# tvlearn/evo

Measured on AMD Instinct MI355X. Metric: E-step candidate-state evals/sec (NxS), full EM iteration, higher is better.
Workload: dtype f64; 1 GPU; ES3C D=256 H=512 S=200 N=100k f64 (north-star shape); algo=es3c, N_total=100000, N_rank0=100000, D=256, H=512, S=200, step=10 full EM iterations, world_size_rccl=1, ea=fit/randflip 10 parents x 1 child x 1 gen, states=p_init_Kn=1/H (init_states default), rng=device, mstep=device, parallelism=dp1

## Files before the change

evo_amd/csrc/evo_amd.hip:

```cpp
#include "../../include/evo_amd.h"

#include <dlfcn.h>
#include <math.h>
#include <stdarg.h>
#include <stdio.h>
#include <stdlib.h>
#include <string.h>

#include <chrono>
#include <memory>
#include <string>
#include <type_traits>
#include <vector>

#include "common.hpp"
#include "gemm_f64.hpp"
#include "kernels_bsc.hpp"
#include "kernels_common.hpp"
#include "kernels_evolve.hpp"
#include "kernels_mstep.hpp"
#include "kernels_sssc.hpp"
#include "kernels_sssc_quad.hpp"
#include "kernels_fused.hpp"
#include "kernels_patches.hpp"
#include "kernels_codes.hpp"
#include "kernels_init.hpp"
#include "kernels_generate.hpp"

static thread_local char g_err[512] = "";

static int fail(int code, const char *fmt, ...) {
  va_list ap;
  va_start(ap, fmt);
  vsnprintf(g_err, sizeof(g_err), fmt, ap);
  va_end(ap);
  return code;
}

#define HIP_TRY(expr)                                                                          \
  do {                                                                                         \
    hipError_t _e = (expr);                                                                    \
    if (_e != hipSuccess)                                                                      \
      return fail(EVOAMD_E_HIP, "%s failed: %s (%s:%d)", #expr, hipGetErrorString(_e), __FILE__, \
                  __LINE__);                                                                   \
  } while (0)

static const bool g_dbg_sync = getenv("EVOAMD_DEBUG_SYNC") != nullptr;
#define DBG_SYNC(c, what)                                                    \
  do {                                                                       \
    if (g_dbg_sync) {                                                        \
      fprintf(stderr, "[evoamd] %s ...", what);                              \
      fflush(stderr);                                                        \
      hipError_t _de = hipStreamSynchronize((c)->stream);                    \
      fprintf(stderr, " %s\n", hipGetErrorString(_de));                      \
      fflush(stderr);                                                        \
    }                                                                        \
  } while (0)

#define REQUIRE(cond, msg)                                   \
  do {                                                       \
    if (!(cond)) return fail(EVOAMD_E_INVALID, "%s", msg);   \
  } while (0)
#define REQUIRE_KN(c) \
  REQUIRE(!(c)->kn_lost, "K^n is not on the device: evoamd_init_states stopped at its round cap (upload or initialise K^n first)")

struct RcclId {
  char internal[128];
};
struct RcclApi {
  void *handle = nullptr;
  int (*GetUniqueId)(RcclId *) = nullptr;
  int (*CommInitRank)(void **, int, RcclId, int) = nullptr;
  int (*AllReduce)(const void *, void *, size_t, int, int, void *, hipStream_t) = nullptr;
  int (*CommDestroy)(void *) = nullptr;
  const char *(*GetErrorString)(int) = nullptr;
};
static RcclApi g_rccl;

static int rccl_load() {
  if (g_rccl.handle) return 0;
  const char *names[] = {"librccl.so.1", "librccl.so", "/opt/rocm/lib/librccl.so.1"};
  void *h = nullptr;
  for (const char *nm : names) {
    h = dlopen(nm, RTLD_NOW | RTLD_LOCAL);
    if (h) break;
  }
  if (!h) return fail(EVOAMD_E_RCCL, "cannot dlopen librccl: %s", dlerror());
  g_rccl.GetUniqueId = (int (*)(RcclId *))dlsym(h, "ncclGetUniqueId");
  g_rccl.CommInitRank = (int (*)(void **, int, RcclId, int))dlsym(h, "ncclCommInitRank");
  g_rccl.AllReduce =
      (int (*)(const void *, void *, size_t, int, int, void *, hipStream_t))dlsym(h, "ncclAllReduce");
  g_rccl.CommDestroy = (int (*)(void *))dlsym(h, "ncclCommDestroy");
  g_rccl.GetErrorString = (const char *(*)(int))dlsym(h, "ncclGetErrorString");
  if (!g_rccl.GetUniqueId || !g_rccl.CommInitRank || !g_rccl.AllReduce || !g_rccl.CommDestroy)
    return fail(EVOAMD_E_RCCL, "librccl is missing a required symbol");
  g_rccl.handle = h;
  return 0;
}
#define RCCL_TRY(expr)                                                                         \
  do {                                                                                         \
    int _r = (expr);                                                                           \
    if (_r != 0)                                                                               \
      return fail(EVOAMD_E_RCCL, "%s failed: %s", #expr,                                       \
                  g_rccl.GetErrorString ? g_rccl.GetErrorString(_r) : "?");                    \
  } while (0)

enum {
  KID_LPJ_RES = 0,
  KID_LPJ_CAND,
  KID_LPJ_OVF,
  KID_ROW_LSE,
  KID_VARY_KN,
  KID_STATS,
  KID_STATS_OVF,
  KID_GEMM,
  KID_EVOLVE,
  KID_MISC,
  KID_MSTEP,
  KID_LPJ_PASS,
  KID_STATS_PASS,
  KID_LPJ_K34,
  KID_LPJ_K58,
  KID_LPJ_K9P,
  KID_STATS_K34,
  KID_STATS_K58,
  KID_STATS_K9P,
  KID_ALLREDUCE,
  KID_ESTEP_FUSED,
  KID_PATCHES,
  KID_INIT_STATES,
  KID_COUNT
};

struct TimedSpan {
  hipEvent_t a, b;
  int kid;
};

struct evoamd_ctx {
  int device = 0;
  hipStream_t stream = nullptr;
  hipStream_t stream2 = nullptr;
  hipEvent_t ev_fork = nullptr, ev_join = nullptr;
  bool gemm_forked = false;
  hipStream_t stream_copy = nullptr;
  hipEvent_t ev_theta = nullptr, ev_theta_done = nullptr;
  hipEvent_t ev_mbox = nullptr, ev_bak = nullptr;
  int mbox_side = 1;
  int theta_copy_engine = 0;
  double rel_frac = -1.0;
  bool ar_gemm_pending = false;
  int overlap_gemm = 1;
  int early_fork = -1;
  int bg_unit = 0;
  int fold_clear = 1;
  bool acc_clean = false, clist_clean = false;
  bool wq_copy_valid = false;
  int stats_chunks = 1;
  int n_cu = 256;
  int stats_stage = 1;
  int stats_waves = 0;
  PairBins pbins = {};
  int bins_min = 256;
 int bins_scale = 3;
  int bins_scale_cur = 0;
  int bins_auto = 1;
  bool bins_dirty = false;
  int bins_nwg = 2048;
  int bsc_wave_opt = 1;
  int gemm_ws_opt = 1;
  double *gemm_ws = nullptr;
  size_t gemm_ws_n = 0;
  int pair_bins = 1;
  int gemm_streamk = 1;
  int sk_spare = -1;
  int sssc_prec32 = 0;
  int main_unstaged = 1;
  int sing_screen = 1;
  double *huge = nullptr;
  int *huge_ctl = nullptr;
  int huge_slots = 0, huge_kc = 0;
  int *sing_gen = nullptr;
  int theta_gen = 0;
  int gemm_grouped = 1;
  int gemm_per_xcd = 0;
  double *census = nullptr;
  i64 pre_n = 4;
  hipEvent_t ev_chunk[16] = {};
  bool configured = false, have_data = false, have_params = false, have_cand = false, B_valid = false;
  bool need_known = false;
  bool res_need[3] = {true, true, true};
  double res_cnt[3] = {0, 0, 0};
  bool cand_from_device = false;
  bool lists_clean = false;
  int pending_skip = 0;
  int pays_agreed = -1;
  int k8_mode = -1;
  bool bsc_direct = false;
  bool f32_opt = false, f32 = false;
  float *Yf = nullptr, *Ytf = nullptr, *Wf = nullptr, *Bf = nullptr, *Esf = nullptr;
  i64 ldYt = 0;
  double *Yt = nullptr;
  int b_tn_opt = 1;
  uint8_t *mask_infr = nullptr, *mask_x = nullptr;
  double *Yrec = nullptr;
  bool yrec_valid = false, rec_in_stats = false;
  double *yhat = nullptr, *tmpWt = nullptr;
  size_t yhat_n = 0;
  bool yhat_valid = false;
  bool stats_rows_valid = false;
  bool rec_resident = false, yrec_from_pass = false;
  uint8_t *keep_x = nullptr;
  bool keep_x_valid = false, rec_uses_keep = false;
  uint8_t *row_any = nullptr;
  int merge_select_fused = 0;
  unsigned long long gen = 0, prefetch_gen = ~0ull;
  bool prefetch_lpj = true;
  int spd_block = 0;
  bool use_digest = true;
  bool spd_inverse = true;
  long spd_fallbacks = 0;
  bool rows_fresh = false;
  int model = 0;
  i64 N = 0;
  int D = 0, H = 0, S = 0, S_perm = 0, Cmax = 0, HW = 0, L = 0;
  double *Y = nullptr, *yy = nullptr, *y2sum = nullptr;
  int ldY = 0;
  double *h_acc = nullptr, *h_par = nullptr;
  size_t h_par_n = 0;
  double *h_theta = nullptr;
  double *h_theta_dev = nullptr;
  bool h_theta_fresh = false;
  double *theta_bak = nullptr;
  size_t theta_bak_n = 0;
  bool theta_bak_valid = false;
  unsigned long long mbox_seq = 0;
  unsigned *mbox_counter = nullptr;
  int *h_err = nullptr;
  u64 *states = nullptr, *cand = nullptr;
  u64 *dig = nullptr, *cand_dig = nullptr;
  double *lpj = nullptr, *cand_lpj = nullptr;
  double *lpj_alt = nullptr;
  int *cand_counts = nullptr;
  u64 *cand_raw = nullptr, *dupold = nullptr;
  int *gen_start = nullptr;
  unsigned *flags = nullptr;
  double *rowmax = nullptr, *rowsum = nullptr, *partial = nullptr, *partial2 = nullptr, *diag = nullptr;
  i64 n_partial = 0;
  uint8_t *stage = nullptr;
  size_t stage_bytes = 0;
  double *W = nullptr, *Wt = nullptr, *G = nullptr, *Psi = nullptr, *Bm = nullptr, *mus = nullptr,
         *pilbar_v = nullptr;
  double2 *GP = nullptr;
  double4 *DG = nullptr;
  double4 *D1 = nullptr;
  PairEntry *PT = nullptr;
  double *pies = nullptr;
  double *dpar = nullptr;
  double *h_dpar = nullptr;
  double *colpart = nullptr;
  size_t colpart_n = 0;
  double *gjwork = nullptr;
  double *tmpA = nullptr, *tmpB = nullptr, *tmpC = nullptr;
  double ljc = 0;
  double *acc = nullptr;
  i64 acc_n = 0;
  double *acc_base = nullptr;
  i64 ovf_n = 0;
  double *Es = nullptr;
  int *list1 = nullptr, *list2 = nullptr, *list3 = nullptr, *list_n = nullptr, *err = nullptr;
  int *clist = nullptr, *clist_n = nullptr;
  size_t clist_words = 0;
  OvfRec *ovf_rec = nullptr;
  size_t ovf_rec_n = 0;
  unsigned long long kn_gen = 1, census_gen = 0;
  int census_opt = 1;
  int merge_small = 1;
  int stats_flat = 0;
  int fused_opt = 0;
  double *rowF = nullptr;
  int *rowcnt = nullptr, *defer = nullptr;
  double *fpart = nullptr;
  unsigned long long *fprof = nullptr;
  bool last_estep_fused = false;
  bool reduce_pending = false;
  long fused_calls = 0, unfused_calls = 0;
  int debug_poison_list = 0;
  int debug_fail_stats = 0;
  int census_skip = 0;
  size_t list_words = 0;
  double *tmp_y = nullptr, *tmp_lpj = nullptr;
  u64 *tmp_states = nullptr;
  size_t tmp_states_words = 0, tmp_lpj_n = 0;
  double *patch_img = nullptr, *patch_Y = nullptr;
  size_t patch_img_n = 0, patch_Y_n = 0;
  uint8_t *codes_buf = nullptr;
  size_t codes_bytes = 0;
  unsigned long long rows_kn_gen = 0;
  int codes_path = -1;
  int init_home = -1;
  u64 *init_scratch = nullptr;
  size_t init_scratch_words = 0;
  bool kn_lost = false;
  i64 kn_refill = 0;
  double *gen_par = nullptr, *gen_y = nullptr, *gen_z = nullptr, *gen_ymean = nullptr;
  u64 *gen_sin = nullptr, *gen_s = nullptr;
  size_t gen_par_n = 0, gen_y_n = 0, gen_z_n = 0, gen_ymean_n = 0, gen_sin_n = 0, gen_s_n = 0;
  i64 gen_N = 0;
  int gen_D = 0, gen_H = 0, gen_keep = -1;
  void *comm = nullptr;
  int rank = 0, world = 1;
  bool timing = false;
  unsigned timing_mask = 0xFFFFFFFFu;
  std::vector<TimedSpan> spans;
  std::vector<hipEvent_t> pool;
  double t_ms[KID_COUNT] = {0};
  i64 t_n[KID_COUNT] = {0};
};

struct SpanGuard {
  evoamd_ctx *c;
  int kid;
  hipStream_t stream;
  hipEvent_t a = nullptr, b = nullptr;
  SpanGuard(evoamd_ctx *ctx, int k, hipStream_t s = nullptr) : c(ctx), kid(k), stream(s ? s : ctx->stream) {
    if (!c->timing || !((c->timing_mask >> k) & 1u)) return;
    auto get = [&]() {
      hipEvent_t e;
      if (!c->pool.empty()) {
        e = c->pool.back();
        c->pool.pop_back();
      } else {
        (void)hipEventCreate(&e);
      }
      return e;
    };
    a = get();
    b = get();
    (void)hipEventRecord(a, stream);
  }
  ~SpanGuard() {
    if (!c->timing || !a) return;
    (void)hipEventRecord(b, stream);
    c->spans.push_back({a, b, kid});
  }
};

static int resolve_spans(evoamd_ctx *c) {
  for (auto &s : c->spans) {
    float ms = 0.f;
    HIP_TRY(hipEventSynchronize(s.b));
    HIP_TRY(hipEventElapsedTime(&ms, s.a, s.b));
    c->t_ms[s.kid] += ms;
    c->t_n[s.kid] += 1;
    c->pool.push_back(s.a);
    c->pool.push_back(s.b);
  }
  c->spans.clear();
  return 0;
}

template <typename T>
static int dev_alloc(T **p, size_t n) {
  if (*p) {
    (void)hipFree(*p);
    *p = nullptr;
  }
  if (n == 0) n = 1;
  HIP_TRY(hipMalloc((void **)p, n * sizeof(T)));
  return 0;
}
#define ALLOC(p, n)                 \
  do {                              \
    int _r = dev_alloc(&(p), (n));  \
    if (_r) return _r;              \
  } while (0)

static inline unsigned cdiv(i64 a, i64 b) { return (unsigned)((a + b - 1) / b); }
static inline size_t list_cap(i64 total) { return (size_t)(256 * (((total + 255) / 256 + LIST_SHARDS - 1) / LIST_SHARDS) + 1024); }

template <bool SQUARE>
static void launch_colsum(evoamd_ctx *c, const double *X, int ldx, i64 R, int Cn, double *out) {
  const i64 rpb = 256;
  dim3 grid(cdiv(Cn, 64), cdiv(R, rpb));
  colsum_f64<SQUARE><<<grid, 256, 0, c->stream>>>(X, ldx, R, Cn, rpb, out);
}


static int ensure_colpart(evoamd_ctx *c, size_t n) {
  if (n <= c->colpart_n) return 0;
  HIP_TRY(hipStreamSynchronize(c->stream));
  ALLOC(c->colpart, n);
  c->colpart_n = n;
  return 0;
}

static int ensure_lists(evoamd_ctx *c, i64 total) {
  const size_t need = list_cap(total) * LIST_SHARDS;
  if (need <= c->list_words) return 0;
  HIP_TRY(hipStreamSynchronize(c->stream));
  ALLOC(c->list1, need);
  ALLOC(c->list2, need);
  ALLOC(c->list3, need);
  c->list_words = need;
  return 0;
}

extern "C" int evoamd_abi_version(void) { return EVOAMD_ABI_VERSION; }
extern "C" const char *evoamd_last_error(void) { return g_err; }

extern "C" int evoamd_device_count(int *count) {
  REQUIRE(count, "count is NULL");
  int n = 0;
  hipError_t e = hipGetDeviceCount(&n);
  if (e != hipSuccess) {
    *count = 0;
    return fail(EVOAMD_E_NODEVICE, "hipGetDeviceCount: %s", hipGetErrorString(e));
  }
  *count = n;
  return 0;
}

extern "C" int evoamd_ctx_create(int device, evoamd_ctx **out) {
  REQUIRE(out, "out is NULL");
  int n = 0;
  if (hipGetDeviceCount(&n) != hipSuccess || n <= 0)
    return fail(EVOAMD_E_NODEVICE, "no HIP device visible (libevo_amd needs an MI355X / gfx950 GPU)");
  REQUIRE(device >= 0 && device < n, "device index out of range");
  HIP_TRY(hipSetDevice(device));
  hipDeviceProp_t prop;
  HIP_TRY(hipGetDeviceProperties(&prop, device));
  if (strncmp(prop.gcnArchName, "gfx950", 6) != 0)
    return fail(EVOAMD_E_NODEVICE, "device %d is %s; libevo_amd is built for gfx950 only", device,
                prop.gcnArchName);
  evoamd_ctx *c = new evoamd_ctx();
  c->device = device;
  c->n_cu = prop.multiProcessorCount > 0 ? prop.multiProcessorCount : 256;
  {
    int prio_lo = 0, prio_hi = 0;
    HIP_TRY(hipDeviceGetStreamPriorityRange(&prio_lo, &prio_hi));
    HIP_TRY(hipStreamCreateWithPriority(&c->stream, hipStreamNonBlocking, prio_hi));
    HIP_TRY(hipStreamCreateWithPriority(&c->stream2, hipStreamNonBlocking, prio_lo));
  }
  HIP_TRY(hipEventCreateWithFlags(&c->ev_fork, hipEventDisableTiming));
  HIP_TRY(hipEventCreateWithFlags(&c->ev_join, hipEventDisableTiming));
  HIP_TRY(hipStreamCreateWithFlags(&c->stream_copy, hipStreamNonBlocking));
  HIP_TRY(hipEventCreateWithFlags(&c->ev_theta, hipEventDisableTiming));
  HIP_TRY(hipEventCreateWithFlags(&c->ev_theta_done, hipEventDisableTiming));
  HIP_TRY(hipEventCreateWithFlags(&c->ev_mbox, hipEventDisableTiming));
  HIP_TRY(hipEventCreateWithFlags(&c->ev_bak, hipEventDisableTiming));
  for (int i = 0; i < 16; i++) HIP_TRY(hipEventCreateWithFlags(&c->ev_chunk[i], hipEventDisableTiming));

  HIP_TRY(hipFuncSetAttribute((const void *)sssc_stats_flat_kernel, hipFuncAttributeMaxDynamicSharedMemorySize, 150 * 1024));
  HIP_TRY(hipFuncSetAttribute((const void *)sssc_big_kernel<0>, hipFuncAttributeMaxDynamicSharedMemorySize,
                              136 * 1024));
  HIP_TRY(hipFuncSetAttribute((const void *)sssc_big_kernel<0, 0>, hipFuncAttributeMaxDynamicSharedMemorySize,
                              136 * 1024));
  HIP_TRY(hipFuncSetAttribute((const void *)sssc_big_kernel<0, 1>, hipFuncAttributeMaxDynamicSharedMemorySize,
                              136 * 1024));
  HIP_TRY(hipFuncSetAttribute((const void *)sssc_big_kernel<1>, hipFuncAttributeMaxDynamicSharedMemorySize,
                              136 * 1024));
  HIP_TRY(hipFuncSetAttribute((const void *)posterior_codes_kernel<CODES_LDS>, hipFuncAttributeMaxDynamicSharedMemorySize,
                              CODES_WAVES * CODES_LDS_H * (int)sizeof(double)));
  HIP_TRY(hipFuncSetAttribute((const void *)gemm_tn128_f64, hipFuncAttributeMaxDynamicSharedMemorySize,
                              (int)GEMM128_LDS_BYTES));
  HIP_TRY(hipFuncSetAttribute((const void *)gemm_tn128_rows_f64, hipFuncAttributeMaxDynamicSharedMemorySize,
                              (int)GEMM128_LDS_BYTES));
  HIP_TRY(hipFuncSetAttribute((const void *)gemm_tn128_sk_f64, hipFuncAttributeMaxDynamicSharedMemorySize,
                              (int)GEMM128_LDS_BYTES));
  HIP_TRY(hipFuncSetAttribute((const void *)gemm_tn128_sk_f32, hipFuncAttributeMaxDynamicSharedMemorySize,
                              (int)GEMM128_LDS_BYTES));
  HIP_TRY(hipFuncSetAttribute((const void *)gemm_tn128_store_f32, hipFuncAttributeMaxDynamicSharedMemorySize,
                              (int)GEMM128_LDS_BYTES));
  {
    const void *wk[] = {(const void *)sssc_stats_wave_kernel<0, 4>,  (const void *)sssc_stats_wave_kernel<1, 4>,
                        (const void *)sssc_stats_wave_kernel<2, 4>,  (const void *)sssc_stats_wave_kernel<4, 4>,
                        (const void *)sssc_stats_wave_kernel<8, 4>,  (const void *)sssc_stats_wave_kernel<16, 4>,
                        (const void *)sssc_stats_wave_kernel<0, 1>,  (const void *)sssc_stats_wave_kernel<0, 8>,
                        (const void *)sssc_stats_wave_kernel<0, 16>};
    for (const void *f : wk) HIP_TRY(hipFuncSetAttribute(f, hipFuncAttributeMaxDynamicSharedMemorySize, 150 * 1024));
    HIP_TRY(hipFuncSetAttribute((const void *)pair_bins_reduce_kernel, hipFuncAttributeMaxDynamicSharedMemorySize, 3 * PB_TILE * 8));
    HIP_TRY(hipFuncSetAttribute((const void *)sssc_small_kernel<4, 1, 2, 256>, hipFuncAttributeMaxDynamicSharedMemorySize, 120 * 1024));
    HIP_TRY(hipFuncSetAttribute((const void *)sssc_small_kernel<8, 1, 2, 256>, hipFuncAttributeMaxDynamicSharedMemorySize, 120 * 1024));
  }
  {
    const void *fk[] = {(const void *)sssc_estep_fused_kernel<1, false>,  (const void *)sssc_estep_fused_kernel<1, true>,
                        (const void *)sssc_estep_fused_kernel<2, false>,  (const void *)sssc_estep_fused_kernel<2, true>,
                        (const void *)sssc_estep_fused_kernel<4, false>,  (const void *)sssc_estep_fused_kernel<4, true>,
                        (const void *)sssc_estep_fused_kernel<8, false>,  (const void *)sssc_estep_fused_kernel<8, true>,
                        (const void *)sssc_estep_fused_kernel<16, false>, (const void *)sssc_estep_fused_kernel<16, true>};
    for (const void *fp : fk) HIP_TRY(hipFuncSetAttribute(fp, hipFuncAttributeMaxDynamicSharedMemorySize, 160 * 1024));
  }
  *out = c;
  return 0;
}

static void free_all(evoamd_ctx *c) {
  void *ptrs[] = {c->Y,      c->yy,     c->y2sum,   c->states,  c->cand,     c->lpj,       c->cand_lpj,
                  c->cand_counts, c->flags, c->rowmax, c->rowsum, c->partial, c->partial2, c->diag, c->stage,    c->W,
                  c->Wt,     c->G,      c->Psi,     c->Bm,      c->mus,      c->pilbar_v,  c->GP,      c->DG,    c->D1,    c->PT,   c->yhat,  c->tmpWt,  c->mask_infr,  c->mask_x,  c->Yrec,
                  c->pies,   c->tmpA,    c->tmpB,    c->tmpC,    c->gjwork,  c->colpart,
                  c->acc_base, c->Es,     c->list1,   c->list2,    c->list3,    c->list_n,    c->err,
                  c->tmp_y,  c->tmp_lpj, c->tmp_states, c->dig, c->cand_dig, c->lpj_alt, c->cand_raw, c->dupold, c->gen_start,
                  c->pbins.ent, c->pbins.part, c->pbins.gcnt, c->gemm_ws, c->Yt, c->Yf, c->Ytf, c->Wf, c->Bf, c->Esf,
                  c->clist, c->clist_n, c->ovf_rec, c->theta_bak, c->rowF, c->rowcnt, c->defer, c->fpart, c->huge, c->huge_ctl,
                  c->patch_img, c->patch_Y, c->keep_x, c->row_any, c->codes_buf, c->init_scratch,
                  c->gen_par, c->gen_y, c->gen_z, c->gen_ymean, c->gen_sin, c->gen_s};
  for (void *p : ptrs)
    if (p) (void)hipFree(p);
  if (c->h_acc) (void)hipHostFree(c->h_acc);
  if (c->h_par) (void)hipHostFree(c->h_par);
  if (c->h_theta) (void)hipHostFree(c->h_theta);
  c->h_theta = nullptr;
  if (c->h_err) (void)hipHostFree(c->h_err);
  if (c->h_dpar) (void)hipHostFree(c->h_dpar);
}

extern "C" void evoamd_ctx_destroy(evoamd_ctx *c) {
  if (!c) return;
  (void)hipSetDevice(c->device);
  (void)hipStreamSynchronize(c->stream);
  if (c->comm && g_rccl.CommDestroy) g_rccl.CommDestroy(c->comm);
  for (auto &s : c->spans) {
    (void)hipEventDestroy(s.a);
    (void)hipEventDestroy(s.b);
  }
  for (auto e : c->pool) (void)hipEventDestroy(e);
  free_all(c);
  (void)hipStreamDestroy(c->stream);
  if (c->stream2) (void)hipStreamDestroy(c->stream2);
  if (c->stream_copy) (void)hipStreamDestroy(c->stream_copy);
  if (c->ev_theta) (void)hipEventDestroy(c->ev_theta);
  if (c->ev_theta_done) (void)hipEventDestroy(c->ev_theta_done);
  if (c->ev_mbox) (void)hipEventDestroy(c->ev_mbox);
  if (c->ev_bak) (void)hipEventDestroy(c->ev_bak);
  if (c->ev_fork) (void)hipEventDestroy(c->ev_fork);
  if (c->ev_join) (void)hipEventDestroy(c->ev_join);
  for (int i = 0; i < 16; i++)
    if (c->ev_chunk[i]) (void)hipEventDestroy(c->ev_chunk[i]);

  delete c;
}

extern "C" int evoamd_set_option(evoamd_ctx *c, const char *name, int value) {
  REQUIRE(c && name, "bad arguments");
  c->gen++;
  if (strcmp(name, "sssc_k8") == 0) {
    c->k8_mode = value < 0 ? -1 : (value != 0);
    return 0;
  }
  if (strcmp(name, "ebsc_f32") == 0) {
    c->f32_opt = value != 0;
    return 0;
  }
  if (strcmp(name, "bsc_direct") == 0) {
    c->bsc_direct = value != 0;
    c->have_params = false;
    return 0;
  }
  if (strcmp(name, "reconstruct_in_stats") == 0) {
    c->rec_in_stats = value != 0;
    return 0;
  }
  if (strcmp(name, "codes_path") == 0) {
    if (value < -1 || value > CODES_GMEM) return fail(EVOAMD_E_INVALID, "codes_path: -1 (auto), 0 registers, 1 LDS, 2 global memory");
    c->codes_path = value;
    return 0;
  }
  if (strcmp(name, "merge_select_fused") == 0) {
    c->merge_select_fused = value != 0;
    return 0;
  }
  if (strcmp(name, "prefetch_lpj") == 0) {
    c->prefetch_lpj = value != 0;
    return 0;
  }
  if (strcmp(name, "inverse_block") == 0) {
    if (value != 0 && value != 16 && value != 32) return fail(EVOAMD_E_INVALID, "inverse_block: 0 (auto), 16 or 32");
    c->spd_block = value;
    return 0;
  }
  if (strcmp(name, "overlap_gemm") == 0) {
    c->overlap_gemm = value;
    return 0;
  }
  if (strcmp(name, "stats_stage") == 0) {
    c->stats_stage = value;
    return 0;
  }
  if (strcmp(name, "stats_waves") == 0) {
    c->stats_waves = value;
    return 0;
  }
  if (strcmp(name, "pair_bins") == 0) {
    c->pair_bins = value;
    return 0;
  }
  if (strcmp(name, "gemm_streamk") == 0) {
    c->gemm_streamk = value;
    return 0;
  }
  if (strcmp(name, "b_transposed") == 0) {
    c->b_tn_opt = value;
    return 0;
  }
  if (strcmp(name, "pair_bins_scale") == 0) {
    if (value < 1 || value > 64) return fail(EVOAMD_E_INVALID, "pair_bins_scale: 1 .. 64");
    c->bins_scale = value;
    return 0;
  }
  if (strcmp(name, "pair_bins_nwg") == 0) {
    if (value < 256 || value > 2048 || (value % 256) != 0) return fail(EVOAMD_E_INVALID, "pair_bins_nwg: 256 .. 2048, multiple of 256");
    c->bins_nwg = value;
    return 0;
  }
  if (strcmp(name, "pair_bins_auto") == 0) {
    c->bins_auto = value != 0;
    return 0;
  }
  if (strcmp(name, "pair_bins_min") == 0) {
    c->bins_min = value;
    return 0;
  }
  if (strcmp(name, "bsc_stats_wave") == 0) {
    c->bsc_wave_opt = value;
    return 0;
  }
  if (strcmp(name, "gemm_workspace") == 0) {
    c->gemm_ws_opt = value;
    return 0;
  }
  if (strcmp(name, "sssc_precision") == 0) {
    if (value != 64 && value != 32) return fail(EVOAMD_E_INVALID, "sssc_precision: 64 or 32");
    c->sssc_prec32 = value == 32;
    return 0;
  }
  if (strcmp(name, "lpj_main_unstaged") == 0) {
    c->main_unstaged = value != 0;
    return 0;
  }
  if (strcmp(name, "lpj_singular_screen") == 0) {
    if (value < 0 || value > 2) return fail(EVOAMD_E_INVALID, "lpj_singular_screen: 0 (never), 1 (automatic) or 2 (always)");
    c->sing_screen = (int)value;
    return 0;
  }
  if (strcmp(name, "gemm_grouped") == 0) {
    c->gemm_grouped = value != 0;
    return 0;
  }
  if (strcmp(name, "gemm_per_xcd") == 0) {
    c->gemm_per_xcd = value;
    return 0;
  }
  if (strcmp(name, "init_states_home") == 0) {
    if (value < -1 || value > 1) return fail(EVOAMD_E_INVALID, "init_states_home: -1 (auto), 0 LDS, 1 global memory");
    c->init_home = value;
    return 0;
  }
  if (strcmp(name, "background_unit") == 0) {
    c->bg_unit = value != 0;
    return 0;
  }
  if (strcmp(name, "fold_clear") == 0) {
    c->fold_clear = value != 0;
    return 0;
  }
  if (strcmp(name, "early_fork") == 0) {
    c->early_fork = value;
    return 0;
  }
  if (strcmp(name, "merge_small_levels") == 0) {
    c->merge_small = value != 0;
    return 0;
  }
  if (strcmp(name, "stats_flat") == 0) {
    c->stats_flat = value != 0;
    return 0;
  }
  if (strcmp(name, "theta_copy_engine") == 0) {
    c->theta_copy_engine = value != 0;
    return 0;
  }
  if (strcmp(name, "census_lists") == 0) {
    c->census_opt = value != 0;
    return 0;
  }
  if (strcmp(name, "sk_spare") == 0) {
    if (value < -1 || value > 32) return fail(EVOAMD_E_INVALID, "sk_spare: -1 (automatic) or 0 .. 32 workgroups per XCD");
    c->sk_spare = value;
    return 0;
  }
  if (strcmp(name, "stats_chunks") == 0) {
    if (value < 1 || value > 16) return fail(EVOAMD_E_INVALID, "stats_chunks: 1 .. 16");
    c->stats_chunks = value;
    return 0;
  }
  if (strcmp(name, "mailbox_side_stream") == 0) {
    c->mbox_side = value != 0;
    return 0;
  }
  if (strcmp(name, "fused_estep") == 0) {
    if (value < 0 || value > 2) return fail(EVOAMD_E_INVALID, "fused_estep: 0 (never), 1 (automatic) or 2 (whenever the shape allows it)");
    c->fused_opt = value;
    return 0;
  }
  if (strcmp(name, "debug_poison_list") == 0) {
    c->debug_poison_list = value != 0;
    return 0;
  }
  if (strcmp(name, "debug_fail_stats") == 0) {
    c->debug_fail_stats = value != 0;
    return 0;
  }
  if (strcmp(name, "state_digest") == 0) {
    c->use_digest = value != 0;
    return 0;
  }
  if (strcmp(name, "inverse_spd") == 0) {
    c->spd_inverse = value != 0;
    return 0;
  }
  return fail(EVOAMD_E_INVALID, "unknown option '%s'", name);
}

static int join_fork(evoamd_ctx *c);

extern "C" int evoamd_synchronize(evoamd_ctx *c) {
  REQUIRE(c, "ctx is NULL");
  int rj = join_fork(c);
  if (rj) return rj;
  HIP_TRY(hipStreamSynchronize(c->stream));
  return 0;
}

static i64 acc_len(const evoamd_ctx *c) {
  const i64 H = c->H, D = c->D;
  return (c->model == EVOAMD_MODEL_BSC) ? H * D + H * H + H + 1 + 8 : 2 * H + 4 * H * H + D * H + D + 8;
}
struct AccLayout {
  i64 Wp, Wq, pies, sigma;
  i64 xs, xss, xsz, xszsz, s_sz, sz_sz, sWp, y2;
  i64 tail;
};
static AccLayout acc_layout(const evoamd_ctx *c) {
  AccLayout a = {};
  const i64 H = c->H, D = c->D;
  if (c->model == EVOAMD_MODEL_BSC) {
    a.Wp = 0;
    a.Wq = H * D;
    a.pies = a.Wq + H * H;
    a.sigma = a.pies + H;
    a.tail = a.sigma + 1;
  } else {
    a.xs = 0;
    a.xss = H;
    a.xsz = a.xss + H * H;
    a.xszsz = a.xsz + H;
    a.sWp = a.xszsz + H * H;
    a.s_sz = a.sWp + D * H;
    a.sz_sz = a.s_sz + H * H;
    a.y2 = a.sz_sz + H * H;
    a.tail = a.y2 + D;
  }
  return a;
}

static int alloc_pair_bins(evoamd_ctx *c, int scale) {
  const i64 N = c->N;
  const int H = c->H, S = c->S;
  if (c->pbins.ent) (void)hipFree(c->pbins.ent);
  if (c->pbins.gcnt) (void)hipFree(c->pbins.gcnt);
  if (c->pbins.part) (void)hipFree(c->pbins.part);
  c->pbins = PairBins{};
  c->bins_scale_cur = 0;
  if (H >= 2 && H <= 1024) {
    PairBins pb = {};
    pb.rf = std::max(1, PB_TILE / (2 * H));
    const int nfold = (H - 1 + 1) / 2;
    pb.nb = (int)cdiv(nfold, pb.rf);
    pb.nwg = c->bins_nwg;
    pb.nsh = std::max((i64)N * S >= (i64)8 << 20 ? 8 : 4, std::min(PB_NSH_MAX, 256 / std::max(1, pb.nb)));
    pb.cap = (int)std::max<i64>(64, (i64)scale * cdiv((i64)N * S, (i64)pb.nb * pb.nwg));
    const size_t ne = (size_t)pb.nb * pb.nwg * pb.cap;
    const bool got = hipMalloc((void **)&pb.ent, ne * sizeof(double4)) == hipSuccess &&
                     hipMalloc((void **)&pb.part, (size_t)pb.nb * pb.nsh * 3 * 2 * pb.rf * H * sizeof(double)) == hipSuccess &&
                     hipMalloc((void **)&pb.gcnt, (size_t)pb.nb * pb.nwg * sizeof(int)) == hipSuccess;
    if (got) {
      HIP_TRY(hipMemsetAsync(pb.gcnt, 0, (size_t)pb.nb * pb.nwg * sizeof(int), c->stream));
      c->pbins = pb;
      c->bins_scale_cur = scale;
      c->bins_dirty = false;
    } else {
      (void)hipGetLastError();
      if (pb.ent) (void)hipFree(pb.ent);
      if (pb.part) (void)hipFree(pb.part);
      if (pb.gcnt) (void)hipFree(pb.gcnt);
    }
  }
  return 0;
}

static int ensure_bins_capacity(evoamd_ctx *c) {
  if (c->model != EVOAMD_MODEL_SSSC || !c->need_known || !c->pbins.ent || c->bins_auto == 0) return 0;
  const double NS = (double)c->N * c->S;
  const double n34 = c->res_cnt[0] - c->res_cnt[1], n58 = c->res_cnt[1] - c->res_cnt[2];
  const double entries = (NS - c->res_cnt[0]) + 6.0 * n34 + 28.0 * n58;
  int want = (int)std::ceil(3.0 * 1.25 * entries / NS);
  if (want > 64) want = 64;
  if (want <= c->bins_scale_cur) return 0;
  HIP_TRY(hipStreamSynchronize(c->stream));
  if (c->stream2) HIP_TRY(hipStreamSynchronize(c->stream2));
  const int before = c->bins_scale_cur;
  int r = alloc_pair_bins(c, want);
  if (r) return r;
  if (!c->pbins.ent) {
    r = alloc_pair_bins(c, before);
    if (r) return r;
    c->bins_auto = 0;
  }
  return 0;
}

extern "C" int evoamd_configure(evoamd_ctx *c, int model, int64_t N, int D, int H, int S, int S_perm,
                                int Cmax) {
  REQUIRE(c, "ctx is NULL");
  REQUIRE(model == EVOAMD_MODEL_BSC || model == EVOAMD_MODEL_SSSC, "unknown model");
  REQUIRE(N > 0 && D > 0 && H > 0 && S > 0, "N, D, H, S must be positive");
  REQUIRE(S_perm == 0 || S_perm == 1, "S_perm must be 0 or 1");
  REQUIRE(Cmax >= 1 && Cmax <= 64 * VK_MAX_C_PER_LANE, "Cmax must be in [1, 256]");
  REQUIRE(S <= 64 * VK_MAX_S_PER_LANE, "S must be <= 1024");
  REQUIRE((i64)N * (S > Cmax ? S : Cmax) < 2147483647LL, "N * max(S, Cmax) must fit in int32");
  HIP_TRY(hipSetDevice(c->device));
  c->model = model;
  c->N = N;
  c->D = D;
  c->H = H;
  c->S = S;
  c->S_perm = S_perm;
  c->Cmax = Cmax;
  c->HW = (H + 63) / 64;
  c->L = S + S_perm;
  const i64 HW = c->HW;
  c->ldY = (model == EVOAMD_MODEL_SSSC) ? D + 3 * H : D;
  ALLOC(c->Y, (size_t)N * c->ldY);
  ALLOC(c->yy, (size_t)N);
  ALLOC(c->y2sum, (size_t)D);
  ALLOC(c->states, (size_t)N * S * HW);
  ALLOC(c->cand, (size_t)N * Cmax * HW);
  if (H <= DIG_MAX_H) {
    ALLOC(c->dig, (size_t)N * S);
    ALLOC(c->cand_dig, (size_t)N * Cmax);
  } else {
    if (c->dig) (void)hipFree(c->dig);
    if (c->cand_dig) (void)hipFree(c->cand_dig);
    c->dig = c->cand_dig = nullptr;
  }
  ALLOC(c->lpj, (size_t)N * c->L);
  ALLOC(c->lpj_alt, (size_t)N * c->L);
  ALLOC(c->cand_lpj, (size_t)N * Cmax);
  ALLOC(c->cand_counts, (size_t)N);
  ALLOC(c->flags, (size_t)3 * N);
  ALLOC(c->rowmax, (size_t)N);
  ALLOC(c->rowsum, (size_t)N);
  c->n_partial = cdiv(N, 4);
  ALLOC(c->partial, (size_t)3 * c->n_partial);
  ALLOC(c->partial2, (size_t)c->n_partial);
  ALLOC(c->diag, (size_t)H);
  const int SC = S > Cmax ? S : Cmax;
  ALLOC(c->W, (size_t)D * H);
  ALLOC(c->tmpA, (size_t)H * H);
  ALLOC(c->tmpB, (size_t)H * H);
  ALLOC(c->tmpC, (size_t)H * H);
  ALLOC(c->gjwork, (size_t)2 * H * H + (size_t)132 * H + 1040 + 4 * GJS32 * GJS32);
  if (model == EVOAMD_MODEL_BSC) {
    ALLOC(c->Es, (model == EVOAMD_MODEL_BSC && c->f32_opt) ? 1 : (size_t)N * H);
  } else {
    if (c->Es) { (void)hipFree(c->Es); }
    c->Es = nullptr;
// ... 311 lines not shown
  REQUIRE(!(c->bg_unit && c->S_perm), "evoamd_init_states: no permanent all-zero state with the background unit (variational/utils.py:42-47)");
  REQUIRE(c->H - c->bg_unit >= 1, "evoamd_init_states: no latent varies");
  HIP_TRY(hipSetDevice(c->device));
  const int S = c->S, HW = c->HW;
  if (table_packed) {
    const int Hv = c->H - c->bg_unit;
    REQUIRE(Hv < 12 && S + c->S_perm == (1 << Hv),
            "evoamd_init_states: a state table means exact E-steps, S + S_perm == 2^Hv with Hv < 12 (variational/utils.py:55)");
  }
  if (table_packed) {
    const int PB = (c->H + 7) / 8;
    const size_t off = (((size_t)S * PB + 7) / 8) * 8;
    {
      int rs = ensure_stage(c, off + (size_t)S * HW * sizeof(u64));
      if (rs) return rs;
    }
    u64 *table = (u64 *)(c->stage + off);
    HIP_TRY(hipMemcpyAsync(c->stage, table_packed, (size_t)S * PB, hipMemcpyHostToDevice, c->stream));
    SpanGuard g(c, KID_INIT_STATES);
    words_from_packbits_kernel<<<cdiv((i64)S * HW, 256), 256, 0, c->stream>>>(c->stage, table, S, PB, HW, c->H);
    init_states_tile_kernel<<<cdiv(c->N * (i64)S, 256), 256, 0, c->stream>>>(table, c->states, c->dig, c->N, S, HW);
  } else {
    InitArgs a;
    a.states = c->states;
    a.dig = c->dig;
    a.scratch = nullptr;
    a.err = c->err + INIT_ERR_WORD;
    a.N = c->N;
    a.S = S;
    a.S_perm = c->S_perm;
    a.H = c->H;
    a.Hv = c->H - c->bg_unit;
    a.HW = HW;
    a.max_rounds = max_rounds;
    a.seed = seed;
    a.p0 = p_init > 0.0 ? p_init : 1.0 / (double)c->H;
    const size_t wave_words = 2 * (size_t)(HW + 1) * S;
    int W = 4;
    while (W > 1 && W * wave_words * sizeof(u64) > 150 * 1024) W >>= 1;
    const bool lds_fits = W * wave_words * sizeof(u64) <= 150 * 1024;
    REQUIRE(c->init_home != 0 || lds_fits, "init_states_home 0 (LDS): the round state of one wavefront does not fit");
    const bool lds_home = c->init_home < 0 ? lds_fits : c->init_home == 0;
    c->kn_lost = true;
    c->kn_refill = 0;
    c->gen++;
    c->kn_gen++;
    c->need_known = false;
    HIP_TRY(hipMemsetAsync(a.err, 0, sizeof(int), c->stream));
    if (lds_home) {
      const unsigned grid = (unsigned)std::min<i64>(cdiv(c->N, W), (i64)c->n_cu * 64);
      SpanGuard g(c, KID_INIT_STATES);
      init_states_kernel<true><<<grid, 64 * W, (size_t)W * wave_words * sizeof(u64), c->stream>>>(a);
    } else {
      W = 4;
      i64 grid = std::min<i64>(cdiv(c->N, W), (i64)c->n_cu * 2);
      while (grid > 1 && (size_t)grid * W * wave_words * sizeof(u64) > ((size_t)256 << 20)) grid >>= 1;
      const size_t need = (size_t)grid * W * wave_words;
      if (need > c->init_scratch_words) {
        HIP_TRY(hipStreamSynchronize(c->stream));
        ALLOC(c->init_scratch, need);
        c->init_scratch_words = need;
      }
      a.scratch = c->init_scratch;
      SpanGuard g(c, KID_INIT_STATES);
      init_states_kernel<false><<<(unsigned)grid, 64 * W, 0, c->stream>>>(a);
    }
    HIP_TRY(hipGetLastError());
    DBG_SYNC(c, "init_states");
    HIP_TRY(hipMemcpyAsync(c->h_err, a.err, sizeof(int), hipMemcpyDeviceToHost, c->stream));
    HIP_TRY(hipStreamSynchronize(c->stream));
    if (c->h_err[0] & INIT_ERR_CAP) {
      HIP_TRY(hipMemsetAsync(a.err, 0, sizeof(int), c->stream));
      return fail(EVOAMD_E_INVALID,
                  "evoamd_init_states: a datapoint holds fewer than S = %d distinct states after max_rounds = %d rounds (the "
                  "round cap); K^n is not initialised -- shapes with S close to 2^H belong to the host function",
                  S, max_rounds);
    }
    c->kn_lost = false;
    return 0;
  }
  HIP_TRY(hipGetLastError());
  HIP_TRY(hipStreamSynchronize(c->stream));
  c->gen++;
  c->kn_gen++;
  c->need_known = false;
  c->kn_lost = false;
  return 0;
}

extern "C" int evoamd_download_states_packed(evoamd_ctx *c, uint8_t *packed, int64_t n0, int64_t n) {
  REQUIRE(c && c->configured, "configure first");
  REQUIRE(packed && n0 >= 0 && n > 0 && n0 + n <= c->N, "bad row range");
  REQUIRE_KN(c);
  HIP_TRY(hipSetDevice(c->device));
  const int PB = (c->H + 7) / 8;
  const i64 ns = n * (i64)c->S;
  const size_t bytes = (size_t)ns * PB;
  {
    int rs = ensure_stage(c, bytes);
    if (rs) return rs;
  }
  packbits_from_words_kernel<<<cdiv(ns * PB, 256), 256, 0, c->stream>>>(c->states + (size_t)n0 * c->S * c->HW, c->stage, ns,
                                                                         PB, c->HW);
  HIP_TRY(hipGetLastError());
  HIP_TRY(hipMemcpyAsync(packed, c->stage, bytes, hipMemcpyDeviceToHost, c->stream));
  HIP_TRY(hipStreamSynchronize(c->stream));
  return 0;
}

extern "C" int evoamd_upload_lpj(evoamd_ctx *c, const double *lpj) {
  REQUIRE(c && c->configured, "configure first");
  HIP_TRY(hipSetDevice(c->device));
  HIP_TRY(hipMemcpyAsync(c->lpj, lpj, (size_t)c->N * c->L * sizeof(double), hipMemcpyHostToDevice, c->stream));
  HIP_TRY(hipStreamSynchronize(c->stream));
  c->rows_fresh = false;
  return 0;
}

extern "C" int evoamd_download_lpj(evoamd_ctx *c, double *lpj) {
  REQUIRE(c && c->configured, "configure first");
  HIP_TRY(hipSetDevice(c->device));
  HIP_TRY(hipMemcpyAsync(lpj, c->lpj, (size_t)c->N * c->L * sizeof(double), hipMemcpyDeviceToHost, c->stream));
  HIP_TRY(hipStreamSynchronize(c->stream));
  return 0;
}

static bool gemm_vec_ok(const double *p, int ld) { return (ld % 2) == 0 && ((uintptr_t)p % 16) == 0; }

static bool launch_gemm_nn_raw(evoamd_ctx *c, const double *A, int lda, const double *B, int ldb, double *C, int ldc,
                               i64 M, int Nc, int K, double *Ct = nullptr, int ldct = 0) {
  if (M <= 1024 && Nc <= 1024 && K <= 1024) {
    gemm_nn_small_kernel<<<dim3(cdiv(Nc, 16), cdiv(M, 16)), 256, 0, c->stream>>>(A, lda, B, ldb, C, ldc, (int)M, Nc, K, Ct, ldct);
    return Ct != nullptr;
  }
  const int gx = (int)cdiv(Nc, GEMM_BN), gy = (int)cdiv(M, GEMM_BM);
  const int rows_per_xcd = (gy + 7) / 8;
  const unsigned grid = (unsigned)(8 * rows_per_xcd * gx);
  if (gemm_vec_ok(A, lda) && gemm_vec_ok(B, ldb) && (K % 2) == 0 && (Nc % 2) == 0 && K >= 2 && Nc >= 2 && M >= 1)
    gemm_nn_f64<true><<<grid, 256, 0, c->stream>>>(A, lda, B, ldb, C, ldc, M, Nc, K, gx, gy, rows_per_xcd);
  else
    gemm_nn_f64<false><<<grid, 256, 0, c->stream>>>(A, lda, B, ldb, C, ldc, M, Nc, K, gx, gy, rows_per_xcd);
  return false;
}

struct GemmTnOpts {
  bool deterministic = false;
  int sym_row0 = -1;
  bool c_is_zero = false;
  bool accumulate = false;
  bool mirror = true;
  hipStream_t stream = nullptr;
  int spare = 0;
  double *diag = nullptr;
};

static bool gram_is_small(int M, i64 K) { return M <= 512 && K <= 4096; }

static double *streamk_workspace(evoamd_ctx *c, unsigned wpx, i64 n_real, int *segmax) {
  *segmax = (int)(n_real / wpx) + 2;
  const size_t need = (size_t)8 * wpx * (size_t)*segmax * GEMM_T * GEMM_T;
  if (need > c->gemm_ws_n) {
    if (c->gemm_ws) (void)hipFree(c->gemm_ws);
    c->gemm_ws = nullptr;
    c->gemm_ws_n = 0;
    if (hipMalloc((void **)&c->gemm_ws, need * sizeof(double)) != hipSuccess) {
      (void)hipGetLastError();
      c->gemm_ws = nullptr;
      return nullptr;
    }
    c->gemm_ws_n = need;
  }
  return c->gemm_ws;
}

static int launch_gemm_tn(evoamd_ctx *c, const double *A, int lda, const double *B, int ldb, double *C, int ldc,
                          int M, int Nc, i64 K, const GemmTnOpts &o = GemmTnOpts()) {
  const bool deterministic = o.deterministic, c_is_zero = o.c_is_zero, accumulate = o.accumulate, mirror = o.mirror;
  int sym_row0 = o.sym_row0;
  const hipStream_t stream = o.stream ? o.stream : c->stream;
  if (deterministic && A == B && lda == ldb && M == Nc && sym_row0 < 0 && gram_is_small(M, K)) {
    SpanGuard g(c, KID_GEMM, stream);
    const int nb16 = (int)cdiv(M, 16);
    gram_small_kernel<<<dim3(nb16, nb16), 256, 0, stream>>>(A, lda, (int)K, M, C, ldc, o.diag);
    HIP_TRY(hipGetLastError());
    return 0;
  }
  const bool vec = gemm_vec_ok(A, lda) && gemm_vec_ok(B, ldb) && (M % 2) == 0 && (Nc % 2) == 0 && M >= 2 && Nc >= 2;
  const bool big = vec && !deterministic && K >= 8192 && M >= 256 && Nc >= 256 &&
                   (sym_row0 < 0 || (sym_row0 % GEMM_T) == 0);
  const int T = big ? GEMM_T : GEMM_BM;
  if (sym_row0 >= 0 && (sym_row0 % T) != 0) sym_row0 = -1;
  const int gx = (int)cdiv(Nc, T), gy = (int)cdiv(M, T);
  const i64 tiles = (i64)gx * gy;
  i64 splits = 1;
  if (K >= 128 && !deterministic) {
    if (big) {
      i64 real = tiles;
      if (sym_row0 >= 0) {
        const i64 ts = cdiv(Nc, T);
        real -= ts * (ts - 1) / 2;
      }
      i64 per_xcd = 1;
      double best = 0.0;
      for (i64 pc = 1; pc <= 16; pc++) {
        if (pc > 1 && K / (8 * pc) < 512) break;
        const double eff = (double)(real * pc) / (64.0 * (double)cdiv(real * pc, 64));
        if (eff > best + 0.01) {
          best = eff;
          per_xcd = pc;
        }
      }
      if (real > 24 && K / 64 >= 384) per_xcd = 8;
      if (c->gemm_per_xcd > 0) per_xcd = c->gemm_per_xcd;
      splits = 8 * per_xcd;
    } else {
      splits = (512 + tiles - 1) / tiles;
    }
    const i64 maxs = (K + 63) / 64;
    if (splits > maxs) splits = maxs;
    if (splits > 1) splits = ((splits + 7) / 8) * 8;
  }
  if (accumulate && splits < 8) splits = 8;
  const int split = splits > 1;
  i64 kps = K;
  if (split) {
    kps = (K + splits - 1) / splits;
    kps = ((kps + GEMM_BK - 1) / GEMM_BK) * GEMM_BK;
    if (!c_is_zero && !accumulate) HIP_TRY(hipMemsetAsync(C, 0, (size_t)M * ldc * sizeof(double), stream));
  }
  const unsigned grid = (unsigned)(tiles * (split ? splits : 1));
  SpanGuard g(c, KID_GEMM, stream);
  if (big && split && c->gemm_streamk) {
    i64 real = tiles;
    if (sym_row0 >= 0) {
      const i64 ts = cdiv(Nc, T);
      real -= ts * (ts - 1) / 2;
    }
    const i64 Kx = ((cdiv(K, 8) + GEMM_BK - 1) / GEMM_BK) * GEMM_BK;
    const unsigned wpx = (unsigned)std::max(1, 2 * c->n_cu / 8 - o.spare);
    int segmax = 0;
    double *ws = c->gemm_ws_opt ? streamk_workspace(c, wpx, real, &segmax) : nullptr;
    const i64 J = (i64)8 * wpx / real;
    if (ws && c->gemm_grouped && J >= 2 && real * J * 100 >= (i64)8 * wpx * 93 && K / J >= 256) {
      const i64 Kc = ((cdiv(K, J) + 2 * GEMM_BK - 1) / (2 * GEMM_BK)) * (2 * GEMM_BK);
      gemm_tn128_gk<double><<<8 * wpx, 256, GEMM128_LDS_BYTES, stream>>>(A, lda, B, ldb, C, ldc, M, Nc, K, Kc, gx, gy,
                                                                            sym_row0, (int)real, (int)J, ws);
      gemm_gk_reduce_kernel<<<dim3((unsigned)real, GEMM_T * GEMM_T / 256), 256, 0, stream>>>(ws, C, ldc, M, Nc, gx, gy,
                                                                                               sym_row0, (int)real, (int)J);
    } else {
    gemm_tn128_sk_f64<<<8 * wpx, 256, GEMM128_LDS_BYTES, stream>>>(A, lda, B, ldb, C, ldc, M, Nc, K, Kx, gx, gy, sym_row0,
                                                                       (int)real, ws, segmax);
    if (ws)
      gemm_sk_reduce_kernel<<<dim3((unsigned)real, GEMM_T * GEMM_T / 256), 256, 0, stream>>>(
          ws, segmax, C, ldc, M, Nc, K, Kx, gx, gy, sym_row0, (int)real, (int)wpx);
    }
  } else if (big)
    gemm_tn128_f64<<<grid, 256, GEMM128_LDS_BYTES, stream>>>(A, lda, B, ldb, C, ldc, M, Nc, K, kps, gx, gy, split, sym_row0);
  else if (vec)
    gemm_tn_f64<true><<<grid, 256, 0, stream>>>(A, lda, B, ldb, C, ldc, M, Nc, K, kps, gx, gy, split, sym_row0);
  else
    gemm_tn_f64<false><<<grid, 256, 0, stream>>>(A, lda, B, ldb, C, ldc, M, Nc, K, kps, gx, gy, split, sym_row0);
  if (sym_row0 >= 0 && mirror)
    mirror_lower_kernel<<<cdiv((i64)Nc * Nc, 256), 256, 0, stream>>>(C + (size_t)sym_row0 * ldc, Nc, ldc, T);
  HIP_TRY(hipGetLastError());
  return 0;
}

static int launch_gemm_nn(evoamd_ctx *c, const double *A, int lda, const double *B, int ldb, double *C, int ldc,
                          i64 M, int Nc, int K) {
  SpanGuard g(c, KID_GEMM);
  launch_gemm_nn_raw(c, A, lda, B, ldb, C, ldc, M, Nc, K);
  HIP_TRY(hipGetLastError());
  return 0;
}

static int launch_B_f32(evoamd_ctx *c);

static int launch_B(evoamd_ctx *c) {
  if (c->f32) return launch_B_f32(c);
  if (!c->Yt) return launch_gemm_nn(c, c->Y, c->ldY, c->W, c->H, c->Bm, c->H, c->N, c->H, c->D);
  SpanGuard g(c, KID_GEMM);
  const int gx = (int)cdiv(c->H, GEMM_T), gy = (int)cdiv(c->N, GEMM_T);
  gemm_tn128_rows_f64<<<(unsigned)(8 * cdiv(gy, 8) * gx), 256, GEMM128_LDS_BYTES, c->stream>>>(
      c->Yt, (int)c->ldYt, c->W, c->H, c->Bm, c->H, (int)c->N, c->H, c->D, gx, gy);
  HIP_TRY(hipGetLastError());
  return 0;
}

static int derive_from_theta(evoamd_ctx *c, bool updated) {
  const int H = c->H, D = c->D;
  int r = 0;
  c->B_valid = false;
  if (c->model == EVOAMD_MODEL_BSC && c->bsc_direct) return 0;
  GemmTnOpts gram;
  gram.deterministic = true;
  if (c->model == EVOAMD_MODEL_SSSC) {
    if (!updated) {
      r = launch_gemm_tn(c, c->W, H, c->W, H, c->G, H, H, H, D, gram);
      if (r) return r;
      DBG_SYNC(c, "derive_from_theta: G = W^T W");
    }
    if (c->mask_infr) {
      if (!c->Wt) ALLOC(c->Wt, (size_t)H * D);
      transpose_kernel<<<cdiv((i64)H * D, 256), 256, 0, c->stream>>>(c->W, D, H, c->Wt);
    }
    sssc_tables_kernel<<<cdiv((i64)H * H, 256), 256, 0, c->stream>>>(c->G, c->Psi, c->mus, c->pilbar_v, c->dpar, H, c->D1,
                                                                     c->PT, c->GP, c->DG, c->sing_gen, ++c->theta_gen);
    DBG_SYNC(c, "derive_from_theta: tables");
  } else {
    const bool diag_rides = updated && gram_is_small(H, D);
    if (diag_rides) gram.diag = c->diag;
    r = launch_gemm_tn(c, c->W, H, c->W, H, c->G, H, H, H, D, gram);
    if (r) return r;
    if (!diag_rides) extract_diag_kernel<<<cdiv(H, 256), 256, 0, c->stream>>>(c->G, H, c->diag);
  }
  HIP_TRY(hipGetLastError());
  if (c->have_data) {
    r = launch_B(c);
    if (r) return r;
    c->B_valid = true;
  }
  return 0;
}

extern "C" int evoamd_set_params_bsc(evoamd_ctx *c, const double *W, double pi, double sigma, double *ljc) {
  REQUIRE(c && c->configured && c->model == EVOAMD_MODEL_BSC, "context is not configured for BSC");
  REQUIRE(W, "W is NULL");
  REQUIRE(!(c->f32 && c->bsc_direct), "the direct residual kernel is not available in the float32 mode");
  HIP_TRY(hipSetDevice(c->device));
  c->ljc = c->H * log(1.0 - pi) - (c->rel_frac >= 0.0 ? c->rel_frac : (double)c->D) / 2.0 * log(2 * M_PI * sigma * sigma);
  if (ljc) *ljc = c->ljc;
  HIP_TRY(hipStreamSynchronize(c->stream));
  memset(c->h_dpar, 0, DP_COUNT * sizeof(double));
  c->h_dpar[DP_PRE1] = -1.0 / 2.0 / sigma / sigma;
  c->h_dpar[DP_PILBAR] = log(pi / (1.0 - pi));
  c->h_dpar[DP_LJC] = c->ljc;
  c->h_dpar[DP_PI] = pi;
  c->h_dpar[DP_SIGMA] = sigma;
  HIP_TRY(hipMemcpyAsync(c->dpar, c->h_dpar, DP_COUNT * sizeof(double), hipMemcpyHostToDevice, c->stream));
  HIP_TRY(hipStreamSynchronize(c->stream));
  double *wt = c->h_par;
  for (int d = 0; d < c->D; d++)
    for (int h = 0; h < c->H; h++) wt[(size_t)h * c->D + d] = W[(size_t)d * c->H + h];
  HIP_TRY(hipMemcpyAsync(c->Wt, wt, (size_t)c->H * c->D * sizeof(double), hipMemcpyHostToDevice, c->stream));
  HIP_TRY(hipStreamSynchronize(c->stream));
  memcpy(wt, W, (size_t)c->D * c->H * sizeof(double));
  HIP_TRY(hipMemcpyAsync(c->W, wt, (size_t)c->D * c->H * sizeof(double), hipMemcpyHostToDevice, c->stream));
  int r = derive_from_theta(c, false);
  if (r) return r;
  c->have_params = true;
  c->gen++;
  c->h_theta_fresh = false;
  c->yhat_valid = c->stats_rows_valid = c->rec_resident = c->yrec_from_pass = false;
  return 0;
}

extern "C" int evoamd_set_params_sssc(evoamd_ctx *c, const double *W, const double *pies, const double *mus,
                                      const double *Psi, double sigma2, double *ljc) {
  REQUIRE(c && c->configured && c->model == EVOAMD_MODEL_SSSC, "context is not configured for SSSC");
  REQUIRE(W && pies && mus && Psi, "NULL parameter array");
  HIP_TRY(hipSetDevice(c->device));
  const int H = c->H, D = c->D;
  const long double s2 = (long double)sigma2;
  const double s2inv = c->sssc_prec32 ? (double)(float)(1.0L / s2) : (double)(1.0L / s2);
  double l = 0.0;
  std::vector<double> pb(H);
  {
    long double acc = 0.0L;
    for (int h = 0; h < H; h++) {
      acc += (long double)log(1.0 - pies[h]);
      pb[h] = log(pies[h] / (1.0 - pies[h]));
    }
    l = (double)acc;
  }
  if (c->rel_frac >= 0.0) {
    l += (-log(2 * M_PI) - log(sigma2)) * c->rel_frac / 2.0;
  } else {
    l -= D / 2.0 * log(2 * M_PI);
    if (c->sssc_prec32) {
      const float ld = (float)D * (float)logl(s2);
      l -= (double)(0.5f * ld);
    } else {
      l -= 0.5 * (D * (double)logl(s2));
    }
  }
  c->ljc = l;
  if (ljc) *ljc = l;
  HIP_TRY(hipStreamSynchronize(c->stream));
  {
    double *hw = c->h_par, *hpsi = hw + (size_t)D * H, *hmu = hpsi + (size_t)H * H, *hpb = hmu + H, *hpi = hpb + H;
    memcpy(hw, W, (size_t)D * H * sizeof(double));
    memcpy(hpsi, Psi, (size_t)H * H * sizeof(double));
    memcpy(hmu, mus, (size_t)H * sizeof(double));
    memcpy(hpb, pb.data(), (size_t)H * sizeof(double));
    memcpy(hpi, pies, (size_t)H * sizeof(double));
    memset(c->h_dpar, 0, DP_COUNT * sizeof(double));
    c->h_dpar[DP_S2INV] = s2inv;
    c->h_dpar[DP_SIGMA2] = sigma2;
    c->h_dpar[DP_LJC] = l;
    HIP_TRY(hipMemcpyAsync(c->dpar, c->h_dpar, DP_COUNT * sizeof(double), hipMemcpyHostToDevice, c->stream));
    HIP_TRY(hipMemcpyAsync(c->pies, hpi, (size_t)H * sizeof(double), hipMemcpyHostToDevice, c->stream));
    HIP_TRY(hipMemcpyAsync(c->W, hw, (size_t)D * H * sizeof(double), hipMemcpyHostToDevice, c->stream));
    HIP_TRY(hipMemcpyAsync(c->Psi, hpsi, (size_t)H * H * sizeof(double), hipMemcpyHostToDevice, c->stream));
    HIP_TRY(hipMemcpyAsync(c->mus, hmu, (size_t)H * sizeof(double), hipMemcpyHostToDevice, c->stream));
    HIP_TRY(hipMemcpyAsync(c->pilbar_v, hpb, (size_t)H * sizeof(double), hipMemcpyHostToDevice, c->stream));
  }
  int r = derive_from_theta(c, false);
  if (r) return r;
  c->have_params = true;
  c->gen++;
  c->h_theta_fresh = false;
  c->yhat_valid = c->stats_rows_valid = c->rec_resident = c->yrec_from_pass = false;
  return 0;
}

static int launch_gemm_tn_f32(evoamd_ctx *c, const float *A, int lda, const float *B, int ldb, double *C, int ldc, int M, int Nc,
                              i64 K, const GemmTnOpts &o = GemmTnOpts()) {
  const hipStream_t stream = o.stream ? o.stream : c->stream;
  SpanGuard g(c, KID_GEMM, stream);
  if (M >= 128 && Nc >= 128 && K >= 2048 && (M % 4) == 0 && (Nc % 4) == 0) {
    const int gx = (int)cdiv(Nc, GEMM_T), gy = (int)cdiv(M, GEMM_T);
    const i64 Kx = ((cdiv(K, 8) + GEMM_BK - 1) / GEMM_BK) * GEMM_BK;
    const unsigned wpx = (unsigned)std::max(1, 2 * c->n_cu / 8 - o.spare);
    int segmax = 0;
    double *ws = c->gemm_ws_opt ? streamk_workspace(c, wpx, (i64)gx * gy, &segmax) : nullptr;
    const i64 real = (i64)gx * gy, J = (i64)8 * wpx / real;
    if (ws && c->gemm_grouped && J >= 2 && real * J * 100 >= (i64)8 * wpx * 93 && K / J >= 256) {
      const i64 Kc = ((cdiv(K, J) + 2 * GEMM_BK - 1) / (2 * GEMM_BK)) * (2 * GEMM_BK);
      gemm_tn128_gk<float><<<8 * wpx, 256, GEMM128_LDS_BYTES, stream>>>(A, lda, B, ldb, C, ldc, M, Nc, K, Kc, gx, gy, -1,
                                                                           (int)real, (int)J, ws);
      gemm_gk_reduce_kernel<<<dim3((unsigned)real, GEMM_T * GEMM_T / 256), 256, 0, stream>>>(ws, C, ldc, M, Nc, gx, gy, -1,
                                                                                               (int)real, (int)J);
    } else {
      gemm_tn128_sk_f32<<<8 * wpx, 256, GEMM128_LDS_BYTES, stream>>>(A, lda, B, ldb, C, ldc, M, Nc, K, Kx, gx, gy, gx * gy,
                                                                         ws, segmax);
      if (ws)
        gemm_sk_reduce_kernel<<<dim3((unsigned)(gx * gy), GEMM_T * GEMM_T / 256), 256, 0, stream>>>(
            ws, segmax, C, ldc, M, Nc, K, Kx, gx, gy, -1, gx * gy, (int)wpx);
    }
  } else {
    gemm_tn_naive_f32<<<cdiv((i64)M * Nc, 256), 256, 0, stream>>>(A, lda, B, ldb, C, ldc, M, Nc, K);
  }
  HIP_TRY(hipGetLastError());
  return 0;
}

static int launch_B_f32(evoamd_ctx *c) {
  SpanGuard g(c, KID_GEMM);
  to_f32_kernel<<<cdiv((i64)c->D * c->H, 256), 256, 0, c->stream>>>(c->W, c->H, c->D, c->H, c->Wf, c->H);
  if (c->H >= 128 && c->N >= 128) {
    const int gx = (int)cdiv(c->H, GEMM_T), gy = (int)cdiv(c->N, GEMM_T);
    gemm_tn128_store_f32<<<(unsigned)gx * gy, 256, GEMM128_LDS_BYTES, c->stream>>>(c->Ytf, (int)c->ldYt, c->Wf, c->H, c->Bf,
                                                                                  c->H, (int)c->N, c->H, c->D, gx);
  } else {
    gemm_nn_naive_f32<<<cdiv(c->N * (i64)c->H, 256), 256, 0, c->stream>>>(c->Yf, c->D, c->Wf, c->H, c->Bf, c->H, c->N, c->H,
                                                                           c->D);
  }
  HIP_TRY(hipGetLastError());
  return 0;
}

static int ensure_B(evoamd_ctx *c) {
  if (c->B_valid || (c->model == EVOAMD_MODEL_BSC && c->bsc_direct)) return 0;
  int r = launch_B(c);
  if (r) return r;
  DBG_SYNC(c, "B = Y W");
  c->B_valid = true;
  return 0;
}

struct Batch {
  const u64 *states;
  const int *counts;
  const double *Y;
  const double *Bm;
  const double *yy;
  i64 N;
  int C, shared;
  double *out;
  int ldo, col0;
  unsigned *flags;
  int kid;
  int tag;
  const uint8_t *mask = nullptr;
};

static const u64 *dig_for(const evoamd_ctx *c, const u64 *states) {
  if (!c->use_digest) return nullptr;
  return states == c->states ? c->dig : states == c->cand ? c->cand_dig : nullptr;
}

static int launch_bsc_lpj(evoamd_ctx *c, const Batch &b) {
  if (!c->bsc_direct && b.tag != 2 && !b.mask) {
    const i64 total = b.N * (i64)b.C;
    unsigned grid = cdiv(total, 256);
    const int bf32 = (c->f32 && b.Bm == c->Bm) ? 1 : 0;
    const void *bmat = bf32 ? (const void *)c->Bf : (const void *)b.Bm;
    SpanGuard g(c, b.kid);
    const int rows_cap = 512 / b.C + 2;
    const size_t lds = (size_t)rows_cap * c->H * sizeof(double);
    const bool hw_ok = c->HW == 1 || c->HW == 2 || c->HW == 4 || c->HW == 8 || c->HW == 16;
    const u64 *dg = b.shared ? nullptr : dig_for(c, b.states);
    if (!b.shared && (hw_ok || dg) && (c->H % 2) == 0 && lds <= 40 * 1024) {
      const unsigned g2 = cdiv(total, 512);
#define GRAM2(TAG, HWT)                                                                                      \
  bsc_lpj_gram2_kernel<TAG, HWT><<<g2, 512, lds, c->stream>>>(b.states, b.counts, bmat, b.yy, c->G, b.N, b.C, c->H, \
                                                              c->HW, c->dpar, b.out, b.ldo, b.col0, b.flags, c->err, dg, bf32, c->diag)
#define GRAM2_HW(TAG)                    \
  switch (c->HW) {                       \
    case 1: GRAM2(TAG, 1); break;        \
    case 2: GRAM2(TAG, 2); break;        \
    case 4: GRAM2(TAG, 4); break;        \
    case 8: GRAM2(TAG, 8); break;        \
    default: GRAM2(TAG, 16); break;      \
  }
      if (b.tag == 0) {
        GRAM2_HW(0)
      } else {
        GRAM2_HW(1)
      }
#undef GRAM2_HW
#undef GRAM2
      HIP_TRY(hipGetLastError());
      return 0;
    }
#define GRAM_LAUNCH(TAG)                                                                                       \
  bsc_lpj_gram_kernel<TAG><<<grid, 256, 0, c->stream>>>(b.states, b.counts, bmat, b.yy, c->G, b.N, b.C, b.shared, \
                                                        c->H, c->HW, c->dpar, b.out, b.ldo, b.col0, b.flags, c->err, dg, bf32, c->diag)
    if (b.tag == 0)
      GRAM_LAUNCH(0);
    else
      GRAM_LAUNCH(1);
#undef GRAM_LAUNCH
    HIP_TRY(hipGetLastError());
    return 0;
  }
  const int nchunk = (b.C + BSC_CHUNK - 1) / BSC_CHUNK;
  const unsigned grid = cdiv(b.N * nchunk, 4);
  SpanGuard g(c, b.kid);
#define BSC_LAUNCH(R)                                                                                     \
  bsc_lpj_kernel<R><<<grid, 256, 0, c->stream>>>(b.Y, c->Wt, b.states, b.counts, b.N, b.C, b.C, b.shared, \
                                                  c->D, c->HW, c->dpar, b.out, b.ldo, b.col0, b.flags, c->err, b.mask)
  if (c->D <= 64)
    BSC_LAUNCH(1);
  else if (c->D <= 128)
    BSC_LAUNCH(2);
  else
    BSC_LAUNCH(4);
#undef BSC_LAUNCH
  HIP_TRY(hipGetLastError());
  return 0;
}

static SsscArgs sssc_args(evoamd_ctx *c, const Batch &b) {
  SsscArgs a = {};
  a.states = b.states;
  a.dig = b.shared ? nullptr : dig_for(c, b.states);
  a.counts = b.counts;
  a.Bm = b.Bm;
  a.yy = b.yy;
  a.GP = c->GP;
  a.DG = c->DG;
  a.D1 = c->D1;
  a.PT = c->PT;
  a.mus = c->mus;
  a.pil_bar = c->pilbar_v;
  a.s2inv = 0.0;
  a.dpar = c->dpar;
  a.N = b.N;
  a.C = b.C;
  a.shared = b.shared;
  a.H = c->H;
  a.HW = c->HW;
  a.lpj_out = b.out;
  a.ldo = b.ldo;
  a.col0 = b.col0;
  a.flags = b.flags;
  a.err = c->err;
  a.sing_gen = c->sing_gen;
  a.gen = c->theta_gen;
  a.screen = c->sing_screen;
  a.huge = c->huge;
  a.huge_ctl = c->huge_ctl;
  a.huge_slots = c->huge_slots;
  a.huge_kc = c->huge_kc;
  a.mask = b.mask;
  a.Wt = c->Wt;
  a.D = c->D;
  return a;
}

// ... 810 lines not shown
  HIP_TRY(hipGetLastError());
  DBG_SYNC(c, "fused E-step (reduce)");
  return 0;
}

extern "C" int evoamd_estep(evoamd_ctx *c, int n_parents, int n_children, uint64_t seed, int fit_parents, int Mprime, int *fused_out) {
  REQUIRE(c && c->configured && c->have_data && c->have_params, "configure, upload_data and set_params first");
  REQUIRE(n_parents >= 1 && n_parents <= c->S && n_parents <= 64, "n_parents must be in [1, min(S, 64)]");
  REQUIRE(n_children >= 1 && n_children <= EV_MAX_CHILDREN && n_children <= c->H, "n_children must be in [1, min(8, H)]");
  REQUIRE(n_parents * n_children <= c->Cmax, "n_parents * n_children exceeds the configured Cmax");
  REQUIRE(Mprime >= 1 && Mprime <= c->S, "Mprime must be in [1, S]");
  REQUIRE_KN(c);
  HIP_TRY(hipSetDevice(c->device));
  bool fused = c->fused_opt != 0 && fused_shape_ok(c, n_parents, n_children);
  if (fused && c->fused_opt == 1) fused = c->need_known && c->res_cnt[1] <= 0.25 * (double)c->N;
  if (fused_out) *fused_out = fused ? 1 : 0;
  if (!fused) {
    c->unfused_calls++;
    c->last_estep_fused = false;
    int r = evoamd_lpj_resident(c);
    if (r) return r;
    r = evoamd_evolve_randflip(c, n_parents, n_children, seed, fit_parents);
    if (r) return r;
    return evoamd_vary_kn(c, Mprime, nullptr);
  }
  c->fused_calls++;
  c->prefetch_gen = ~0ull;
  c->rows_fresh = false;
  int r = launch_estep_fused(c, n_parents, n_children, seed, fit_parents, Mprime);
  if (r) return r;
  c->gen++;
  c->kn_gen++;
  if (c->N * (i64)c->S < ((i64)4 << 20)) c->census_gen = c->kn_gen;
  c->rows_fresh = true;
  c->have_cand = false;
  c->cand_from_device = true;
  c->last_estep_fused = true;
  return 0;
}

extern "C" int evoamd_estep_counters(evoamd_ctx *c, int64_t out[4]) {
  REQUIRE(c && c->configured && out, "bad arguments");
  HIP_TRY(hipSetDevice(c->device));
  out[0] = c->fused_calls;
  out[1] = c->unfused_calls;
  out[2] = out[3] = 0;
  if (c->defer) {
    int h[2] = {0, 0};
    HIP_TRY(hipStreamSynchronize(c->stream));
    HIP_TRY(hipMemcpy(&h[0], c->defer + c->N, sizeof(int), hipMemcpyDeviceToHost));
    out[2] = h[0];
  }
  return 0;
}

extern "C" int evoamd_evolve_states(evoamd_ctx *c, int mutation, int fit_parents, int n_parents, int n_children,
                                    int n_generations, uint64_t seed, double sparseness, double bitflip_prob) {
  REQUIRE(c && c->configured && c->have_data && c->have_params, "configure, upload_data and set_params first");
  REQUIRE(mutation >= EV_RANDFLIP && mutation <= EV_CROSS_SPARSEFLIP, "unknown mutation operator");
  REQUIRE_KN(c);
  REQUIRE(n_parents >= 1 && n_parents <= c->S && n_parents <= 64, "n_parents must be in [1, min(S, 64)]");
  REQUIRE(n_generations >= 1, "n_generations must be positive");
  const bool crossing = mutation >= EV_CROSS;
  const int per_gen = crossing ? n_parents * (n_parents - 1) : n_parents * n_children;
  REQUIRE(crossing || (n_children >= 1 && n_children <= c->H), "n_children must be in [1, H]");
  REQUIRE(mutation != EV_RANDFLIP || n_children <= EV_MAX_CHILDREN, "randflip: n_children must be <= 8");
  REQUIRE((i64)per_gen * n_generations <= c->Cmax, "children per generation x generations exceeds the configured Cmax");
  REQUIRE(c->S <= EVG_MAX_S && c->Cmax <= EVG_MAX_C, "S <= 1024 and Cmax <= 256");
  const bool sparse = mutation == EV_SPARSEFLIP || mutation == EV_CROSS_SPARSEFLIP;
  REQUIRE(!sparse || bitflip_prob == bitflip_prob, "sparseflip needs bitflip_prob (eas.py:69)");
  REQUIRE(!crossing || c->H >= 2, "crossover needs H >= 2");
  HIP_TRY(hipSetDevice(c->device));
  if (!c->cand_raw) {
    ALLOC(c->cand_raw, (size_t)c->N * c->Cmax * c->HW);
    ALLOC(c->dupold, (size_t)c->N * EVG_FLAGW);
    ALLOC(c->gen_start, (size_t)c->N);
  }
  EvolveArgs a = {};
  a.states = c->states;
  a.dig = c->use_digest ? c->dig : nullptr;
  a.lpj = c->lpj;
  a.cand = c->cand;
  a.cand_dig = c->cand_dig;
  a.cand_lpj = c->cand_lpj;
  a.raw = c->cand_raw;
  a.counts = c->cand_counts;
  a.gen_start = c->gen_start;
  a.dupold = c->dupold;
  a.N = c->N;
  a.S = c->S;
  a.S_perm = c->S_perm;
  a.H = c->H - c->bg_unit;
  a.HW = c->HW;
  a.Cmax = c->Cmax;
  a.n_parents = n_parents;
  a.n_children = n_children;
  a.kind = mutation;
  a.fit_parents = fit_parents;
  a.seed = seed;
  a.sparseness = sparseness;
  a.p_bf = bitflip_prob;
  for (int g = 0; g < n_generations; g++) {
    a.gen = g;
    {
      SpanGuard sg(c, KID_EVOLVE);
      evolve_general_kernel<<<(unsigned)c->N, 64, 0, c->stream>>>(a);
      HIP_TRY(hipGetLastError());
      DBG_SYNC(c, "evolve (general)");
    }
    c->cand_from_device = false;
    int r = eval_candidates(c);
    if (r) return r;
  }
  c->have_cand = true;
  return 0;
}

extern "C" int evoamd_download_candidates(evoamd_ctx *c, uint8_t *cand_bool, int32_t *counts, double *lpj) {
  REQUIRE(c && c->configured && c->have_cand, "no resident candidate batch");
  REQUIRE(cand_bool && counts && lpj, "NULL output");
  HIP_TRY(hipSetDevice(c->device));
  const i64 ns = c->N * (i64)c->Cmax;
  int r = ensure_stage(c, (size_t)ns * c->H);
  if (r) return r;
  unpack_states_kernel<<<cdiv(ns * c->H, 256), 256, 0, c->stream>>>(c->cand, c->stage, ns, c->H, c->HW);
  HIP_TRY(hipGetLastError());
  HIP_TRY(hipMemcpyAsync(cand_bool, c->stage, (size_t)ns * c->H, hipMemcpyDeviceToHost, c->stream));
  HIP_TRY(hipMemcpyAsync(counts, c->cand_counts, (size_t)c->N * sizeof(int), hipMemcpyDeviceToHost, c->stream));
  HIP_TRY(hipMemcpyAsync(lpj, c->cand_lpj, (size_t)ns * sizeof(double), hipMemcpyDeviceToHost, c->stream));
  if (c->model == EVOAMD_MODEL_SSSC) return check_err(c);
  HIP_TRY(hipStreamSynchronize(c->stream));
  return 0;
}

extern "C" int64_t evoamd_acc_size(evoamd_ctx *c) { return (c && c->configured) ? c->acc_n : -1; }

static int row_lse(evoamd_ctx *c, const double *lpj, i64 N, int L, double *rowmax, double *rowsum, double *out_slot) {
  const unsigned nb = cdiv(N, 4);
  if ((i64)nb > c->n_partial) {
    ALLOC(c->partial, (size_t)3 * nb);
    ALLOC(c->partial2, (size_t)nb);
    c->n_partial = nb;
  }
  if (lpj != c->lpj) c->rows_fresh = false;
  SpanGuard g(c, KID_ROW_LSE);
  row_lse_kernel<<<nb, 256, 0, c->stream>>>(lpj, N, L, rowmax, rowsum, c->partial);
  reduce_partials_kernel<<<1, 256, 0, c->stream>>>(c->partial, nb, out_slot, 0);
  HIP_TRY(hipGetLastError());
  return 0;
}

static int compute_reconstruction(evoamd_ctx *c);

static int join_fork(evoamd_ctx *c) {
  if (c->gemm_forked) {
    HIP_TRY(hipStreamWaitEvent(c->stream, c->ev_join, 0));
    c->gemm_forked = false;
  }
  if (c->ar_gemm_pending) {
    c->ar_gemm_pending = false;
    const AccLayout a = acc_layout(c);
    SpanGuard g(c, KID_ALLREDUCE);
    RCCL_TRY(g_rccl.AllReduce(c->acc + a.sWp, c->acc + a.sWp, (size_t)(a.y2 - a.sWp),  8,  0,
                              c->comm, c->stream));
  }
  return 0;
}

static TailArgs make_tail_args(evoamd_ctx *c, const AccLayout &a, i64 N, bool census, int skipped) {
  TailArgs ta = {};
  ta.tail = c->acc + a.tail;
  ta.N = (double)N;
  ta.dpar = c->dpar;
  ta.flags = c->flags;
  ta.nflags3 = 3 * N;
  ta.nper = N;
  ta.err = c->err;
  ta.list_n = c->model == EVOAMD_MODEL_SSSC ? (census ? c->clist_n : c->list_n) : nullptr;
  ta.nshards = LIST_SHARDS;
  ta.skipped_mask = skipped;
  ta.census = c->census;
  ta.census_lists = census ? 1 : 0;
  ta.fly_n = (census && c->model == EVOAMD_MODEL_SSSC) ? c->list_n : nullptr;
  ta.fly_skip = c->pending_skip;
  return ta;
}

static double contraction_flops(const evoamd_ctx *c) {
  return c->model == EVOAMD_MODEL_SSSC ? 2.0 * (double)c->N * (c->D + 2.0 * c->H) * c->H : 2.0 * (double)c->N * c->D * c->H;
}

struct StatsPlan {
  AccLayout a;
  i64 N;
  int H, D;
  bool masked;
  LevelHints lv;
  bool gemm_timed;
  double gemm_flops;
  bool pays;
  bool early;
  bool fork_gemm;
  i64 rpb;
  int nblk;
  int nchunks;
  i64 rows_per_chunk;
  bool second_stream;
  int gemm_spare;
  int waves;
  bool census;
  bool bsc_wave;
};

struct StatsBlock {
  int ci;
  i64 n0, nc;
  int blk0, nblk_c;
};

struct StatsFlow {
  bool early_recorded = false;
  bool tail_done = false;
  bool served3 = false;
  int skipped = 0;
  int bsc_grid = 0;
  PairBins bsc_pb = {};
  PairBins pb = {};
};

struct Es3cPass {
  double *Es, *Ez, *Ed;
  SsscArgs sa = {};
  bool need[3] = {true, true, true};
  Es3cLists ls = {};
};

struct Es3cBlock {
  SsscArgs sc;
  i64 total;
  LevelHints lv;
  int flatG = 0;
  size_t flat_lds = 0;
  bool few4;
};

static bool stats_bins_pay(const evoamd_ctx *c) {
  return c->pbins.ent && (c->pair_bins == 2 || (c->pair_bins == 1 && c->N * (i64)c->S >= (i64)c->bins_min * 1024));
}

static int stats_per_cu(size_t lds_per_wg, int wave_lim) {
  int per_cu = (int)((160 * 1024) / lds_per_wg);
  if (per_cu > wave_lim) per_cu = wave_lim;
  if (per_cu > 8) per_cu = 8;
  if (per_cu < 1) per_cu = 1;
  return per_cu;
}

static int rows_written(evoamd_ctx *c, const StatsPlan &p, StatsFlow &fl) {
  if (p.second_stream && p.nchunks == 1 && p.early && !p.masked) {
    HIP_TRY(hipEventRecord(c->ev_chunk[0], c->stream));
    fl.early_recorded = true;
  }
  return 0;
}

static int reconstruct_rows(evoamd_ctx *c, const char *asked_msg = nullptr) {
  int r = compute_reconstruction(c);
  if (r) return r;
  if (asked_msg) REQUIRE(c->rec_in_stats, asked_msg);
  select_rec_kernel<<<cdiv(c->N, 4), 256, 0, c->stream>>>(c->Y, c->ldY, c->mask_x, c->mask_infr, c->yhat, c->N, c->D, c->Yrec);
  HIP_TRY(hipGetLastError());
  c->yrec_valid = c->yrec_from_pass = true;
  c->rec_in_stats = false;
  return 0;
}

static int stats_plan(evoamd_ctx *c, bool fork_gemm, StatsPlan &p) {
  p = StatsPlan{};
  p.a = acc_layout(c);
  p.N = c->N;
  p.H = c->H;
  p.D = c->D;
  p.masked = c->mask_infr != nullptr;
  p.lv.known_tag = c->cand_from_device ? 1 : 2;
  p.lv.one_bit = c->cand_from_device;
  p.gemm_timed = c->timing && (c->timing_mask & ((1u << KID_MSTEP) | (1u << KID_MISC) |
                                                 (1u << KID_STATS) | (1u << KID_STATS_OVF)));
  const double gemm_flops = p.gemm_flops = contraction_flops(c);
  bool pays = (c->model == EVOAMD_MODEL_SSSC && gemm_flops >= 8e9) || (c->model == EVOAMD_MODEL_BSC && !c->comm && gemm_flops >= 5e10);
  const bool early = p.early = c->early_fork == 1 || (c->early_fork < 0 && gemm_flops < 2e10);
  if (c->model == EVOAMD_MODEL_SSSC && !c->comm && early && gemm_flops >= 5e8 && !c->mask_infr) pays = true;
  if (c->model == EVOAMD_MODEL_BSC && !c->comm && early && gemm_flops >= 5e8 && !c->mask_infr && c->bsc_wave_opt &&
      dig_for(c, c->states) && cdiv(c->S, 64) <= 4 && (size_t)5 * c->H * sizeof(double) <= 150 * 1024 && !c->f32)
    pays = true;
  if (c->comm && c->model == EVOAMD_MODEL_SSSC) {
    if (c->pays_agreed < 0) {
      double v = pays ? 1.0 : 0.0;
      int ra = evoamd_comm_allreduce_host(c, &v, 1, 1);
      if (ra) return ra;
      c->pays_agreed = v > 0.0 ? 1 : 0;
    }
    pays = c->pays_agreed == 1;
  }
  p.pays = pays;
  p.fork_gemm = fork_gemm && (c->overlap_gemm == 2 || (c->overlap_gemm == 1 && pays)) &&
                (!c->comm || c->model == EVOAMD_MODEL_SSSC) && !p.gemm_timed && !c->mask_infr;
  p.rpb = ((std::max<i64>(256, cdiv(p.N, 128)) + 3) / 4) * 4;
  p.nblk = (int)cdiv(p.N, p.rpb);
  int nchunks = 1;
  if (!p.masked && !p.gemm_timed && c->overlap_gemm != 0 && c->stats_chunks > 1 && (gemm_flops >= 8e9 || c->overlap_gemm == 2))
    nchunks = std::min<int>(c->stats_chunks, p.nblk);
  p.waves = (c->stats_waves == 4 || c->stats_waves == 8 || c->stats_waves == 16)
                ? c->stats_waves
                : ((size_t)(4 * 2 + 3) * p.H * sizeof(double) <= 150 * 1024 ? 4 : 1);
  p.census = census_mode(c) && !p.masked && p.waves == 4;
  if (p.census) nchunks = 1;
  p.rows_per_chunk = (i64)cdiv(p.nblk, nchunks) * p.rpb;
  p.nchunks = nchunks = (int)cdiv(p.N, p.rows_per_chunk);
  p.second_stream = p.fork_gemm || nchunks > 1;
  {
    const double chain_us = c->H >= 256 ? 15.0 * cdiv(c->H, 32) : 8.5 * cdiv(c->H, 16);
    p.gemm_spare = !(p.fork_gemm && nchunks == 1) ? 0 : ((gemm_flops / 65e6 >= 3.0 * chain_us && c->H <= 512) ? 4 : 8);
  }
  const int SRb = (int)cdiv(c->S, 64);
  p.bsc_wave = c->model == EVOAMD_MODEL_BSC && c->bsc_wave_opt && dig_for(c, c->states) &&
               (SRb == 1 || SRb == 2 || SRb == 4 || SRb == 3) && nchunks == 1 && (size_t)5 * p.H * sizeof(double) <= 150 * 1024;
  return 0;
}

static int stats_bsc_wave(evoamd_ctx *c, const StatsPlan &p, const StatsBlock &blk, StatsFlow &fl) {
  const AccLayout &a = p.a;
  const i64 nc = blk.nc;
  const int H = p.H;
  const u64 *bdig = dig_for(c, c->states);
  const int SRb = (int)cdiv(c->S, 64);
  SpanGuard g(c, KID_STATS);
  const size_t ldsb = (size_t)5 * H * sizeof(double);
  const int per_cu = stats_per_cu(ldsb + 2048, 8);
  PairBins &bsc_pb = fl.bsc_pb;
  bsc_pb = PairBins{};
  if (stats_bins_pay(c)) bsc_pb = c->pbins;
  int sgrid = (int)std::min<i64>(cdiv(nc, 4), (i64)c->n_cu * per_cu * 2);
  if (sgrid > 2048) sgrid = 2048;
  if (bsc_pb.ent && sgrid > bsc_pb.nwg) sgrid = bsc_pb.nwg;
  PB_GRID_CHECK(bsc_pb, sgrid);
  if (bsc_pb.ent) c->bins_dirty = true;
  fl.bsc_grid = sgrid;
  void *EsP = c->f32 ? (void *)c->Esf : (void *)c->Es;
  double *csb = c->acc_base + 4;
#define BSC_WAVE(SR)                                                                                                      \
  bsc_stats_wave_kernel<SR><<<sgrid, 256, ldsb, c->stream>>>(c->states, c->lpj, c->rowmax, c->rowsum, c->yy, nc, c->S,     \
                                                            c->S_perm, H, c->HW, c->dpar, EsP, c->acc + a.Wq, c->partial2, \
                                                            bdig, c->f32 ? 1 : 0, bsc_pb, csb)
  if (SRb == 1) BSC_WAVE(1);
  else if (SRb == 2) BSC_WAVE(2);
  else BSC_WAVE(4);
#undef BSC_WAVE
  HIP_TRY(hipGetLastError());
  DBG_SYNC(c, "bsc stats (wave)");
  int r = rows_written(c, p, fl);
  if (r) return r;
  if (bsc_pb.ent) {
    pair_bins_reduce_kernel<<<bsc_pb.nb * bsc_pb.nsh, PB_RTHREADS, (size_t)3 * 2 * bsc_pb.rf * H * sizeof(double), c->stream>>>(
        bsc_pb, H, 0);
    HIP_TRY(hipGetLastError());
    c->bins_dirty = false;
  }
  return 0;
}

static int stats_bsc_classic(evoamd_ctx *c, const StatsPlan &p, const StatsBlock &blk) {
  const AccLayout &a = p.a;
  const i64 n0 = blk.n0, nc = blk.nc;
  const int H = p.H;
  {
    SpanGuard g(c, KID_STATS);
    with_hw(c->HW, [&](auto hw) {
      bsc_stats_kernel<decltype(hw)::value><<<cdiv(nc, 4), 256, (size_t)4 * H * sizeof(double), c->stream>>>(
          c->states + (size_t)n0 * c->S * c->HW, c->lpj + (size_t)n0 * c->L, c->rowmax + n0, c->rowsum + n0, c->yy + n0, nc,
          c->S, c->S_perm, H, c->HW, c->dpar,
          c->f32 ? (void *)(c->Esf + (size_t)n0 * H) : (void *)(c->Es + (size_t)n0 * H), c->acc + a.Wq, c->partial2 + n0 / 4,
          dig_for(c, c->states) ? dig_for(c, c->states) + (size_t)n0 * c->S : nullptr, c->f32 ? 1 : 0);
    });
    HIP_TRY(hipGetLastError());
    DBG_SYNC(c, "bsc stats");
  }
  {
    SpanGuard g(c, KID_MISC);
    if (c->f32)
      colsum_partial_f32_kernel<<<dim3(cdiv(H, 64), blk.nblk_c), 256, 0, c->stream>>>(c->Esf + (size_t)n0 * H, H, nc, H, p.rpb,
                                                                                      c->colpart + (size_t)blk.blk0 * H);
    else
      colsum_partial_kernel<<<dim3(cdiv(H, 64), blk.nblk_c), 256, 0, c->stream>>>(c->Es + (size_t)n0 * H, H, nc, H, p.rpb,
                                                                                  c->colpart + (size_t)blk.blk0 * H);
    HIP_TRY(hipGetLastError());
  }
  return 0;
}

static int stats_bsc_block(evoamd_ctx *c, const StatsPlan &p, const StatsBlock &blk, StatsFlow &fl, const double *&Ywp, int &ldwp) {
  int r = p.bsc_wave ? stats_bsc_wave(c, p, blk, fl) : stats_bsc_classic(c, p, blk);
  if (r) return r;
  if (p.masked) {
    if (c->rec_in_stats) {
      r = reconstruct_rows(c);
      if (r) return r;
    }
    REQUIRE(c->yrec_valid, "incomplete data: the M-step needs y_reconstructed (bsc.py:186); reconstruct or upload it");
    Ywp = c->Yrec;
    ldwp = p.D;
  }
  return 0;
}

static int stats_sssc_masked_block(evoamd_ctx *c, const StatsPlan &p, const Es3cPass &ep) {
  const i64 N = p.N;
  const int H = p.H;
  const i64 total = N * (i64)c->S;
  HIP_TRY(hipMemset2DAsync(ep.Es, (size_t)c->ldY * sizeof(double), 0, (size_t)3 * H * sizeof(double), (size_t)N, c->stream));
  {
    SpanGuard g(c, KID_STATS);
    sssc_big_kernel<1><<<(int)std::min<i64>(total, 65536), 64, big_lds(8), c->stream>>>(ep.sa, ep.ls.none_in, ep.ls.o3, 8);
    sssc_big_kernel<1><<<1024, 64, big_lds(SSSC_KCAP), c->stream>>>(ep.sa, ep.ls.i3, ep.ls.none_out, SSSC_KCAP);
    HIP_TRY(hipGetLastError());
  }
  SpanGuard g(c, KID_MISC);
  colsum_partial_kernel<<<dim3(cdiv(3 * H, 64), p.nblk), 256, 0, c->stream>>>(ep.Es, c->ldY, N, 3 * H, p.rpb, c->colpart);
  HIP_TRY(hipGetLastError());
  return 0;
}

static Es3cBlock sssc_block_setup(evoamd_ctx *c, const StatsPlan &p, const Es3cPass &ep, const StatsBlock &blk) {
  const SsscArgs &sa = ep.sa;
  const i64 n0 = blk.n0;
  const int H = p.H, D = p.D;
  Es3cBlock eb = {};
  SsscArgs &sc = eb.sc;
  sc = sa;
  sc.states = sa.states + (size_t)n0 * c->S * c->HW;
  if (sa.dig) sc.dig = sa.dig + (size_t)n0 * c->S;
  sc.Bm = sa.Bm + (size_t)n0 * H;
  sc.yy = sa.yy + n0;
  sc.lpj_in = sa.lpj_in + (size_t)n0 * sa.ldo;
  sc.rowmax = sa.rowmax + n0;
  sc.rowsum = sa.rowsum + n0;
  sc.Es = sa.Es + (size_t)n0 * sa.ldE;
  sc.Ez = sa.Ez + (size_t)n0 * sa.ldE;
  sc.Ed = sa.Ed + (size_t)n0 * sa.ldE;
  sc.N = blk.nc;
  eb.total = blk.nc * (i64)c->S;
  eb.lv = p.lv;
  eb.lv.scale = (double)blk.nc / (double)p.N;
  if (p.census && c->stats_flat && c->S <= FLAT_T && (H % 2) == 0 && (D % 2) == 0 && sc.Ez == sc.Es + H && c->stats_waves == 0) {
    int flatG = FLAT_T / c->S;
    const int gmax = (int)(((size_t)140 * 1024 / sizeof(double) - (size_t)7 * H) / ((size_t)4 * H + 4));
    if (flatG > gmax) flatG = gmax;
    if (flatG > 4 * FLAT_T / H) flatG = 4 * FLAT_T / H;
    if (flatG >= 1) eb.flat_lds = ((size_t)H * (4 * flatG + 7) + 4 * flatG) * sizeof(double);
    eb.flatG = flatG;
  }
  eb.few4 = p.census && eb.flatG < 1 && few_above4(c, eb.lv);
  return eb;
}

static int stats_sssc_census_quads(evoamd_ctx *c, const StatsPlan &p, const Es3cPass &ep, const Es3cBlock &eb, StatsFlow &fl) {
  const bool *need = ep.need;
  const PairBins &pb = fl.pb;
  int r = ensure_census(c);
  if (r) return r;
  if (need[0] || need[1]) {
    SpanGuard g(c, KID_STATS_OVF);
    const unsigned gcap = pb.ent ? (unsigned)std::min(2048, pb.nwg) : 2048u;
    const size_t dl = (size_t)p.H * sizeof(double);
    if (need[0]) {
      SpanGuard gl(c, KID_STATS_K34);
      const unsigned qg = quad_grid(c, eb.lv, 0, eb.total, gcap);
      PB_GRID_CHECK(pb, qg);
      sssc_quad_kernel<1, 1, 2><<<qg, 256, dl, c->stream>>>(eb.sc, ep.ls.cA, ep.ls.none_out, ep.ls.o3, pb, c->ovf_rec);
    }
// ... 62 lines not shown
  DBG_SYNC(c, "sssc stats main");
  return 0;
}

static int stats_sssc_census_levels(evoamd_ctx *c, const Es3cPass &ep, const Es3cBlock &eb) {
  const bool *need = ep.need;
  if (need[0] || need[1] || need[2]) {
    SpanGuard g(c, KID_STATS_OVF);
    SpanGuard gl(c, KID_STATS_K9P);
    const int served = census_wavefront_levels<1, 2>(c, eb.sc, ep.ls, need, eb.few4, eb.lv, eb.total);
    if (!(served & 2)) c->pending_skip |= 2;
    HIP_TRY(hipGetLastError());
    DBG_SYNC(c, "sssc stats wavefront level (census)");
  }
  return 0;
}

static int stats_sssc_chain_levels(evoamd_ctx *c, const StatsPlan &p, const Es3cPass &ep, const Es3cBlock &eb, StatsFlow &fl) {
  const bool *need = ep.need;
  const PairBins &pb = fl.pb;
  const SsscArgs &sc = eb.sc;
  const i64 total = eb.total;
  const LevelHints &lv = eb.lv;
  if (need[0] || need[1] || need[2]) {
    SpanGuard g(c, KID_STATS_OVF);
    const size_t cs_lds = sc.cs ? (size_t)3 * p.H * sizeof(double) : 0;
    bool merged23 = false;
    if (need[0]) {
      const unsigned g4 = pb_clamp(pb, level_grid(c, lv, 0, total, 1024, 256));
      PB_GRID_CHECK(pb, g4);
      sssc_small_kernel<4, 1, 2, 256><<<g4, 256, cs_lds, c->stream>>>(sc, ep.ls.i1, ep.ls.o2, pb, ep.ls.o3);
    }
    if (c->k8_mode == 1) {
      if (need[1]) {
        const unsigned g8 = pb_clamp(pb, level_grid(c, lv, 1, total, 256, 256));
        PB_GRID_CHECK(pb, g8);
        sssc_small_kernel<8, 1, 2, 256><<<g8, 256, cs_lds, c->stream>>>(sc, ep.ls.i2, ep.ls.o3, pb, ep.ls.o3);
      }
    } else if (need[1] && few_dense_states(c, lv)) {
      sssc_big_kernel<1><<<level_grid(c, lv, 1, total * 256, 1024, 1), 64, big_lds(SSSC_KCAP), c->stream>>>(
          sc, ep.ls.i2, ep.ls.none_out, SSSC_KCAP, ep.ls.i3);
      fl.served3 = true;
      merged23 = true;
    } else if (need[1]) {
      sssc_big_kernel<1><<<level_grid(c, lv, 1, total * 256, 4096, 1), 64, big_lds(8), c->stream>>>(sc, ep.ls.i2, ep.ls.o3, 8);
    }
    if ((need[2] || c->sing_screen) && !merged23) {
      sssc_big_kernel<1><<<level_grid(c, lv, 2, total * 256, 1024, 1), 64, big_lds(SSSC_KCAP), c->stream>>>(
          sc, ep.ls.i3, ep.ls.none_out, SSSC_KCAP);
      fl.served3 = true;
    }
    HIP_TRY(hipGetLastError());
    DBG_SYNC(c, "sssc stats overflow levels");
  }
  return 0;
}

static int stats_sssc_block(evoamd_ctx *c, const StatsPlan &p, const Es3cPass &ep, const StatsBlock &blk, StatsFlow &fl,
                            bool debug_fail) {
  PairBins &pb = fl.pb;
  const Es3cBlock eb = sssc_block_setup(c, p, ep, blk);
  int r;
  if (pb.ent) c->bins_dirty = true;
  if (blk.ci > 0) {
    census_lists_kernel<<<1, 256, 0, c->stream>>>(c->list_n, LIST_SHARDS, skip_mask(ep.need), c->err, c->census);
    HIP_TRY(hipGetLastError());
  }
  if (eb.flatG >= 1 && pb.ent) {
    const i64 per_bin = (i64)pb.nwg * pb.cap;
    pb.nwg = std::min(pb.nwg, c->n_cu);
    pb.cap = (int)std::min<i64>(per_bin / pb.nwg, 1 << 30);
  }
  if (p.census) {
    r = stats_sssc_census_quads(c, p, ep, eb, fl);
    if (r) return r;
  }
  r = stats_sssc_main(c, p, ep, eb, blk, fl);
  if (r) return r;
  if (debug_fail)
    return fail(EVOAMD_E_INVALID, "debug_fail_stats: statistics pass stopped after its main kernel");
  r = p.census ? stats_sssc_census_levels(c, ep, eb) : stats_sssc_chain_levels(c, p, ep, eb, fl);
  if (r) return r;
  r = rows_written(c, p, fl);
  if (r) return r;
  if (pb.ent) {
    SpanGuard g(c, KID_STATS);
    pair_bins_reduce_kernel<<<pb.nb * pb.nsh, PB_RTHREADS, (size_t)3 * 2 * pb.rf * p.H * sizeof(double), c->stream>>>(pb, p.H, blk.ci > 0);
    HIP_TRY(hipGetLastError());
    c->bins_dirty = false;
    DBG_SYNC(c, "pair bins reduce");
  }
  fl.skipped = skip_mask(ep.need) & ~(fl.served3 ? 4 : 0);
  return 0;
}

static int stats_finish(evoamd_ctx *c, const StatsPlan &p, const Es3cPass &ep, StatsFlow &fl) {
  const AccLayout &a = p.a;
  const i64 N = p.N;
  const int H = p.H, D = p.D;
  const bool masked = p.masked;
  SpanGuard g(c, KID_MISC);
  if (c->model == EVOAMD_MODEL_BSC) {
    TailArgs ta = {};
    if (p.nchunks == 1 && !masked && !c->reduce_pending) {
      ta = make_tail_args(c, a, N, false, fl.skipped);
      fl.tail_done = true;
    }
    double *wq_copy = (!c->comm && !masked && c->tmpA) ? c->tmpA : nullptr;
    c->wq_copy_valid = wq_copy != nullptr;
    const unsigned fgrid = cdiv((i64)H * H, 256) + (fl.tail_done ? 1 : 0);
    if (p.bsc_wave)
      bsc_finish_kernel<<<fgrid, 256, 0, c->stream>>>(c->acc + a.Wq, c->acc + a.pies, c->acc_base + 4, BSC_CS_SLICES, H,
                                                       c->partial2, fl.bsc_grid, c->acc + a.sigma, fl.bsc_pb, ta, wq_copy);
    else
      bsc_finish_kernel<<<fgrid, 256, 0, c->stream>>>(c->acc + a.Wq, c->acc + a.pies, c->colpart, p.nblk, H, c->partial2,
                                                       cdiv(N, 4), c->acc + a.sigma, PairBins{}, ta, wq_copy);
  } else {
    const SsscArgs &sa = ep.sa;
    const i64 nthr = (i64)H * H > D ? (i64)H * H : D;
    TailArgs ta = {};
    if (p.nchunks == 1 && !masked && !c->reduce_pending) {
      ta = make_tail_args(c, a, N, p.census, fl.skipped);
      fl.tail_done = true;
    }
    sssc_finish_kernel<<<cdiv(nthr, 256) + (fl.tail_done ? 1 : 0), 256, 0, c->stream>>>(
        c->acc + a.xss, c->acc + a.xszsz, c->acc + a.xs, c->acc + a.xsz, masked ? c->colpart : sa.cs,
        masked ? p.nblk : CS_SLICES, H, c->y2sum, c->acc + a.y2, D, sa.xss_o, sa.xszsz_o, masked ? nullptr : c->PT, fl.pb, ta);
  }
  HIP_TRY(hipGetLastError());
  DBG_SYNC(c, "colsum + finish");
  return 0;
}

static int stats_contract_block(evoamd_ctx *c, const StatsPlan &p, const Es3cPass &ep, const StatsBlock &blk, const StatsFlow &fl,
                                const double *Ywp, int ldwp) {
  const AccLayout &a = p.a;
  const i64 n0 = blk.n0, nc = blk.nc;
  const int H = p.H, D = p.D, ci = blk.ci;
  GemmTnOpts o;
  if (p.second_stream) {
    if (!fl.early_recorded) HIP_TRY(hipEventRecord(c->ev_chunk[ci], c->stream));
    HIP_TRY(hipStreamWaitEvent(c->stream2, c->ev_chunk[ci], 0));
    o.stream = c->stream2;
    o.spare = c->sk_spare >= 0 ? c->sk_spare : p.gemm_spare;
  }
  o.c_is_zero = true;
  o.accumulate = p.nchunks > 1;
  o.mirror = ci == p.nchunks - 1;
  if (c->model == EVOAMD_MODEL_BSC && c->f32)
    return launch_gemm_tn_f32(c, c->Esf + (size_t)n0 * H, H, c->Yf + (size_t)n0 * D, D, c->acc + a.Wp, D, H, D, nc, o);
  if (c->model == EVOAMD_MODEL_BSC)
    return launch_gemm_tn(c, c->Es + (size_t)n0 * H, H, Ywp + (size_t)n0 * ldwp, ldwp, c->acc + a.Wp, D, H, D, nc, o);
  o.sym_row0 = ((D + H) % GEMM_BM) == 0 ? D + H : -1;
  return launch_gemm_tn(c, c->Y + (size_t)n0 * c->ldY, c->ldY, ep.Ez + (size_t)n0 * c->ldY, c->ldY, c->acc + a.sWp, H,
                        D + 2 * H, H, nc, o);
}

static int stats_sssc_masked_products(evoamd_ctx *c, const StatsPlan &p, const Es3cPass &ep) {
  const AccLayout &a = p.a;
  const int H = p.H, D = p.D;
  int r = reconstruct_rows(c, "ES3C on incomplete data needs do_reconstruction in every step (sssc.py:630-633)");
  if (r) return r;
  GemmTnOpts o;
  o.c_is_zero = true;
  o.sym_row0 = (H % GEMM_BM) == 0 ? H : -1;
  r = launch_gemm_tn(c, ep.Es, c->ldY, ep.Ez, c->ldY, c->acc + a.sWp + (size_t)D * H, H, 2 * H, H, p.N, o);
  if (r) return r;
  o.sym_row0 = -1;
  return launch_gemm_tn(c, c->Yrec, D, ep.Ez, c->ldY, c->acc + a.sWp, H, D, H, p.N, o);
}

static int stats_epilogue(evoamd_ctx *c, const StatsPlan &p, const StatsFlow &fl) {
  const AccLayout &a = p.a;
  const i64 N = p.N;
  if (p.second_stream) {
    HIP_TRY(hipEventRecord(c->ev_join, c->stream2));
    if (p.fork_gemm)
      c->gemm_forked = true;
    else
      HIP_TRY(hipStreamWaitEvent(c->stream, c->ev_join, 0));
  }
  {
    int rfr = flush_reduce(c);
    if (rfr) return rfr;
  }
  {
    SpanGuard g(c, KID_MISC);
    if (!fl.tail_done) tail_kernel<<<1, 256, 0, c->stream>>>(make_tail_args(c, a, N, p.census, fl.skipped));
    HIP_TRY(hipGetLastError());
    DBG_SYNC(c, "stats contraction + tail");
    c->lists_clean = c->model == EVOAMD_MODEL_SSSC;
    if (c->lists_clean) c->pending_skip = 0;
    if (c->model == EVOAMD_MODEL_SSSC && c->mask_infr) {
      masked_sqsum_kernel<<<256, 256, 0, c->stream>>>(c->yhat, c->mask_infr, N * (i64)p.D, c->acc + a.tail + 7);
      HIP_TRY(hipGetLastError());
    }
  }
  if (c->comm && c->gemm_forked) {
    SpanGuard g(c, KID_ALLREDUCE);
    RCCL_TRY(g_rccl.AllReduce(c->acc, c->acc, (size_t)a.sWp,  8,  0, c->comm, c->stream));
    RCCL_TRY(g_rccl.AllReduce(c->acc + a.y2, c->acc + a.y2, (size_t)(c->acc_n - a.y2), 8, 0, c->comm, c->stream));
    c->ar_gemm_pending = true;
  } else if (c->comm) {
    SpanGuard g(c, KID_ALLREDUCE);
    RCCL_TRY(g_rccl.AllReduce(c->acc, c->acc, (size_t)c->acc_n,  8,  0, c->comm, c->stream));
  }
  return 0;
}

static int stats_sssc_pass(evoamd_ctx *c, const StatsPlan &p, Es3cPass &ep) {
  const AccLayout &a = p.a;
  const i64 N = p.N;
  const int H = p.H, D = p.D;
  ep.Es = c->model == EVOAMD_MODEL_SSSC ? c->Y + D : c->Es;
  ep.Ez = c->Y + D + H;
  ep.Ed = c->Y + D + 2 * H;
  if (c->model != EVOAMD_MODEL_SSSC) return 0;
  SsscArgs &sa = ep.sa;
  Batch b = {c->states, nullptr, c->Y, c->Bm, c->yy, N, c->S, 0, nullptr, c->L, c->S_perm, c->flags, KID_STATS, 0};
  b.mask = c->mask_infr;
  sa = sssc_args(c, b);
  sa.lpj_in = c->lpj;
  sa.rowmax = c->rowmax;
  sa.rowsum = c->rowsum;
  sa.Es = ep.Es;
  sa.Ez = ep.Ez;
  sa.Ed = ep.Ed;
  sa.ldE = c->ldY;
  sa.xss = c->acc + a.xss;
  sa.xszsz = c->acc + a.xszsz;
  sa.xss_o = c->acc_base + c->pre_n;
  sa.xszsz_o = c->acc_base + c->pre_n + (size_t)H * H;
  if (!p.masked) sa.cs = c->acc_base + 4;
  ep.ls = es3c_lists(c, (int)list_cap(N * (i64)c->S));
  levels_for(c, p.lv, ep.need);
  return zero_lists(c);
}

static int stats_compute(evoamd_ctx *c, bool fork_gemm = false) {
  REQUIRE(c && c->configured && c->have_data && c->have_params, "configure, upload_data and set_params first");
  REQUIRE_KN(c);
  StatsPlan p;
  int r = stats_plan(c, fork_gemm, p);
  if (r) return r;
  r = join_fork(c);
  if (r) return r;
  HIP_TRY(hipSetDevice(c->device));
  r = ensure_bins_capacity(c);
  if (r) return r;
  if (c->bins_dirty && c->pbins.gcnt)
    HIP_TRY(hipMemsetAsync(c->pbins.gcnt, 0, (size_t)c->pbins.nb * c->pbins.nwg * sizeof(int), c->stream));
  c->bins_dirty = false;
  const bool debug_fail = c->debug_fail_stats != 0;
  c->debug_fail_stats = 0;
  if (!c->acc_clean)
    HIP_TRY(hipMemsetAsync(c->acc_base, 0, (size_t)(c->ovf_n + c->acc_n) * sizeof(double), c->stream));
  c->acc_clean = false;
  c->yhat_valid = c->stats_rows_valid = c->rec_resident = c->yrec_from_pass = false;
  r = ensure_B(c);
  if (r) return r;
  if (!c->rows_fresh) {
    r = row_lse(c, c->lpj, p.N, c->L, c->rowmax, c->rowsum, c->dpar + DP_FS);
    if (r) return r;
  }
  StatsFlow fl;
  std::unique_ptr<SpanGuard> pass(new SpanGuard(c, KID_STATS_PASS));
  r = ensure_colpart(c, (size_t)p.nblk * (c->model == EVOAMD_MODEL_BSC ? p.H : 3 * p.H));
  if (r) return r;
  Es3cPass ep;
  r = stats_sssc_pass(c, p, ep);
  if (r) return r;
  const double *Ywp = c->Y;
  int ldwp = c->ldY;
  if (c->model == EVOAMD_MODEL_SSSC && !p.masked && stats_bins_pay(c)) fl.pb = c->pbins;
  for (int ci = 0; ci < p.nchunks; ci++) {
    const i64 n0 = (i64)ci * p.rows_per_chunk;
    const i64 nc = std::min<i64>(p.rows_per_chunk, p.N - n0);
    const StatsBlock blk = {ci, n0, nc, (int)(n0 / p.rpb), (int)cdiv(nc, p.rpb)};
    if (c->model == EVOAMD_MODEL_BSC)
      r = stats_bsc_block(c, p, blk, fl, Ywp, ldwp);
    else if (p.masked)
      r = stats_sssc_masked_block(c, p, ep);
    else
      r = stats_sssc_block(c, p, ep, blk, fl, debug_fail);
    if (r) return r;
    if (ci == p.nchunks - 1) {
      r = stats_finish(c, p, ep, fl);
      if (r) return r;
      pass.reset();
    }
    if (c->model == EVOAMD_MODEL_SSSC && p.masked) continue;
    r = stats_contract_block(c, p, ep, blk, fl, Ywp, ldwp);
    if (r) return r;
  }
  if (c->model == EVOAMD_MODEL_SSSC && p.masked) {
    r = stats_sssc_masked_products(c, p, ep);
    if (r) return r;
  }
  r = stats_epilogue(c, p, fl);
  if (r) return r;
  c->stats_rows_valid = true;
  c->rows_kn_gen = c->kn_gen;
  return 0;
}

static void note_levels(evoamd_ctx *c, const double *dpar_host) {
  if (c->model != EVOAMD_MODEL_SSSC) return;
  for (int j = 0; j < 3; j++) {
    c->res_cnt[j] = dpar_host[DP_NGT2 + j];
    c->res_need[j] = c->res_cnt[j] > 0.0;
  }
  c->need_known = true;
}

extern "C" int evoamd_stats(evoamd_ctx *c, double *acc_out) {
  REQUIRE(acc_out, "acc_out is NULL");
  int r = stats_compute(c);
  if (r) return r;
  HIP_TRY(hipMemcpyAsync(c->h_acc, c->acc, ((size_t)c->acc_n + DP_COUNT) * sizeof(double), hipMemcpyDeviceToHost,
                         c->stream));
  r = check_err(c);
  if (c->sssc_prec32 && c->model == EVOAMD_MODEL_SSSC) {
    const AccLayout a = acc_layout(c);
    for (i64 i = 0; i < a.sWp; i++) c->h_acc[i] = (double)(float)c->h_acc[i];
    for (i64 i = a.s_sz; i < a.y2; i++) c->h_acc[i] = (double)(float)c->h_acc[i];
  }
  memcpy(acc_out, c->h_acc, (size_t)c->acc_n * sizeof(double));
  if (!r) note_levels(c, c->h_acc + c->acc_n);
  return r;
}

static int launch_inverse_pivoted(evoamd_ctx *c, double *A, double *B, int n) {
  if (n <= GJR_N) {
    gj_inverse_reg_kernel<<<B ? 2 : 1, MS_T, 0, c->stream>>>(A, B, n, c->dpar + DP_STATUS);
    HIP_TRY(hipGetLastError());
    return 0;
  }
  double *mats[2] = {A, B};
  const dim3 ugrid(cdiv(n, 64), cdiv(n, 64));
  if (n <= 1024) {
    const int nmat = B ? 2 : 1;
    GjMats gm;
    gm.a[0] = A;
    gm.a[1] = B ? B : A;
    gm.w[0] = c->gjwork;
    gm.w[1] = c->gjwork + (size_t)n * n;
    double *Dp = c->gjwork + (size_t)2 * n * n;
    double *Pn = Dp + (size_t)64 * n;
    int *ipiv = (int *)(Pn + (size_t)64 * n);
    int *perm = ipiv + 2 * n;
    const int rpt = n <= 256 ? 1 : 2;
    const int pthreads = cdiv(cdiv(n, rpt), 64) * 64;
    const dim3 ug(cdiv(n, 64), cdiv(n, 64), nmat);
    int flip = 0;
    for (int p0 = 0; p0 < n; p0 += 16, flip ^= 1) {
      const int pf = flip | (p0 ? 0 : 4);
      if (rpt == 1)
        gjp_panel_kernel<16, 1><<<nmat, pthreads, 0, c->stream>>>(gm, n, p0, pf, ipiv, perm, Pn, Dp, c->dpar + DP_STATUS);
      else
        gjp_panel_kernel<16, 2><<<nmat, pthreads, 0, c->stream>>>(gm, n, p0, pf, ipiv, perm, Pn, Dp, c->dpar + DP_STATUS);
      gjp_update_kernel<16><<<ug, 256, 0, c->stream>>>(gm, n, p0, flip, ipiv, Dp, Pn);
    }
    gjp_unscramble_kernel<<<dim3(n, nmat), 256, 0, c->stream>>>(gm, n, flip, perm);
    HIP_TRY(hipGetLastError());
    return 0;
  }
  for (int m = 0; m < 2; m++) {
    if (!mats[m]) continue;
    for (int p = 0; p < n; p++) {
      gj_pivot_kernel<<<1, MS_T, 0, c->stream>>>(mats[m], n, p, c->gjwork, c->dpar + DP_STATUS);
      gj_update_kernel<<<ugrid, 256, 0, c->stream>>>(mats[m], n, p, c->gjwork);
    }
    gj_unscramble_kernel<<<n, 256, (size_t)n * (sizeof(double) + sizeof(int)), c->stream>>>(mats[m], n, c->gjwork);
    HIP_TRY(hipGetLastError());
  }
  return 0;
}

static int launch_inverse_spd(evoamd_ctx *c, double *A, double *B, int n) {
  const int nmat = B ? 2 : 1;
  GjMats gm;
  gm.a[0] = A;
  gm.a[1] = B ? B : A;
  gm.w[0] = c->gjwork;
  gm.w[1] = c->gjwork + (size_t)n * n;
  double *Pinv = c->gjwork + (size_t)2 * n * n + (size_t)130 * n + 8;
  double *d0 = Pinv + 2 * 2 * GJS_B * GJS_B;
  if (n <= GJR_MAXN && c->spd_block == 0) {
    gjs_resident_kernel<<<nmat, 1024, 0, c->stream>>>(gm, n, c->dpar + DP_STATUS);
    HIP_TRY(hipGetLastError());
    return 0;
  }
  if (n >= GJS32 && (c->spd_block == 32 || (c->spd_block == 0 && n >= 256))) {
    double *Pinv32 = c->gjwork + (size_t)2 * n * n + (size_t)132 * n + 1040;
    gjs32_first_kernel<<<nmat, 64, 0, c->stream>>>(gm, n, Pinv32, d0, c->dpar + DP_STATUS);
    const dim3 grid32(cdiv(n, 64), cdiv(n, 64), nmat);
    int flip32 = 0;
    for (int p0 = 0; p0 < n; p0 += GJS32, flip32 ^= 1)
      gjs32_step_kernel<<<grid32, 256, 0, c->stream>>>(gm, n, p0, flip32, Pinv32, d0, c->dpar + DP_STATUS);
    HIP_TRY(hipGetLastError());
    if (flip32) {
      for (int k = 0; k < nmat; k++)
        HIP_TRY(hipMemcpyAsync(gm.a[k], gm.w[k], (size_t)n * n * sizeof(double), hipMemcpyDeviceToDevice, c->stream));
    }
    return 0;
  }
  gjs_first_kernel<<<nmat, 64, 0, c->stream>>>(gm, n, Pinv, d0, c->dpar + DP_STATUS);
  const dim3 grid(cdiv(n, 64), cdiv(n, 64), nmat);
  int flip = 0;
  for (int p0 = 0; p0 < n; p0 += GJS_B, flip ^= 1)
    gjs_step_kernel<<<grid, 256, 0, c->stream>>>(gm, n, p0, flip, Pinv, d0, c->dpar + DP_STATUS);
  HIP_TRY(hipGetLastError());
  if (flip) {
    for (int k = 0; k < nmat; k++)
      HIP_TRY(hipMemcpyAsync(gm.a[k], gm.w[k], (size_t)n * n * sizeof(double), hipMemcpyDeviceToDevice, c->stream));
  }
  return 0;
}

static int launch_inverse(evoamd_ctx *c, double *A, double *B, int n, bool force_pivot = false) {
  if (c->spd_inverse && !force_pivot) return launch_inverse_spd(c, A, B, n);
  return launch_inverse_pivoted(c, A, B, n);
}

enum : int {
  MSTEP_LEARN_BITS = L_W | L_PIES | L_MUS | L_SIGMA2 | L_PSI,
  MSTEP_WANT_REC = 32,
  MSTEP_THETA_HOME = 64,
};

enum BackupRoute {
  BACKUP_NONE,
  BACKUP_IN_UPDATE,
  BACKUP_SIDE_KERNEL,
};

enum PublishRoute {
  PUBLISH_FOLDED,
  PUBLISH_MAIN,
  PUBLISH_SIDE,
  PUBLISH_COPY_ENGINE,
};

struct MstepPlan {
  int learn;
  bool want_rec;
  bool theta_home;
  bool force_pivot;
  BackupRoute backup;
  PublishRoute publish;
  bool theta_in_mailbox;
};

static bool backup_rides_in_update(const evoamd_ctx *c) {
  return c->model == EVOAMD_MODEL_SSSC && c->D <= 8 * c->H;
}

static MstepPlan mstep_plan(const evoamd_ctx *c, int learn_mask, bool spd_retry) {
  MstepPlan p = {};
  p.learn = learn_mask & MSTEP_LEARN_BITS;
  p.want_rec = (learn_mask & MSTEP_WANT_REC) != 0;
  p.theta_home = (learn_mask & MSTEP_THETA_HOME) != 0;
  p.force_pivot = spd_retry;
  p.backup = BACKUP_NONE;
  if (p.learn && p.theta_home && !spd_retry) p.backup = backup_rides_in_update(c) ? BACKUP_IN_UPDATE : BACKUP_SIDE_KERNEL;
  const bool theta_out = p.learn && !p.theta_home;
  if (theta_out && c->theta_copy_engine) {
    p.publish = PUBLISH_COPY_ENGINE;
    return p;
  }
  p.theta_in_mailbox = theta_out;
  if (c->mbox_side && contraction_flops(c) >= (theta_out ? 8e10 : 8e9))
    p.publish = PUBLISH_SIDE;
  else
    p.publish = (p.learn && p.theta_home && !spd_retry) ? PUBLISH_FOLDED : PUBLISH_MAIN;
  return p;
}

static int theta_update_sssc(evoamd_ctx *c, const MstepPlan &p, unsigned long long fold_seq) {
  const AccLayout a = acc_layout(c);
  const int H = c->H, D = c->D, learn = p.learn;
  const i64 HH = (i64)H * H;
  const double *Nptr = c->acc + a.tail + 3;
  double *bak = p.backup == BACKUP_IN_UPDATE ? c->theta_bak : nullptr;
  int r = 0;
  if (c->sssc_prec32)
    round_f32_kernel<<<cdiv(a.sWp, 256), 256, 0, c->stream>>>(c->acc, a.sWp);
  sssc_mstep_prepare_kernel<<<cdiv(HH, 256), 256, 0, c->stream>>>(c->acc + a.xs, c->acc + a.xsz, c->acc + a.xss,
                                                                  c->acc + a.xszsz, Nptr, H, learn,
                                                                  c->pies, c->mus, c->tmpA, c->tmpC, c->tmpB, bak, c->W,
                                                                  c->Psi, c->dpar, D, c->bg_unit);
  if ((learn & L_W) && (learn & L_PSI))
    r = launch_inverse(c, c->tmpA, c->tmpB, H, p.force_pivot);
  else if (learn & L_W)
    r = launch_inverse(c, c->tmpA, nullptr, H, p.force_pivot);
  else if (learn & L_PSI)
    r = launch_inverse(c, c->tmpB, nullptr, H, p.force_pivot);
  if (r) return r;
  r = join_fork(c);
  if (r) return r;
  if (c->sssc_prec32) round_f32_kernel<<<cdiv(a.y2 - a.s_sz, 256), 256, 0, c->stream>>>(c->acc + a.s_sz, a.y2 - a.s_sz);
  if (learn & L_W)
    launch_gemm_nn_raw(c, c->acc + a.sWp, H, c->tmpA, H, c->W, H, D, H, H);
  const bool masked = c->mask_infr != nullptr;
  const bool psi_with_trace = (learn & L_PSI) && (learn & L_SIGMA2) && !masked;
  if ((learn & L_PSI) && !psi_with_trace)
    sssc_psi_finish_kernel<<<cdiv(HH, 256), 256, 0, c->stream>>>(c->tmpC, c->tmpB, c->acc + a.s_sz, c->mus, H, c->Psi);
  else if (!(learn & L_PSI))
    psi_floor_kernel<<<cdiv(H, 256), 256, 0, c->stream>>>(c->Psi, H);
  HIP_TRY(hipGetLastError());
  GemmTnOpts gram;
  gram.deterministic = true;
  r = launch_gemm_tn(c, c->W, H, c->W, H, c->G, H, H, H, D, gram);
  if (r) return r;
  const int n_part = (int)std::min<i64>(1024, cdiv(HH, 1024));
  r = ensure_colpart(c, (size_t)n_part);
  if (r) return r;
  if (psi_with_trace)
    sssc_trace_partial_kernel<<<n_part, 256, 0, c->stream>>>(c->acc + a.sz_sz, c->G, H, cdiv(HH, n_part), c->colpart, c->tmpC,
                                                             c->tmpB, c->acc + a.s_sz, c->mus, c->Psi);
  else if ((learn & L_SIGMA2) && !masked)
    sssc_trace_partial_kernel<<<n_part, 256, 0, c->stream>>>(c->acc + a.sz_sz, c->G, H, cdiv(HH, n_part), c->colpart);
  sssc_sigma_precompute_kernel<<<1, MS_T, 0, c->stream>>>(c->acc + a.y2, D, c->colpart, masked ? 0 : n_part, H, Nptr, learn,
                                                          c->pies, c->pilbar_v, c->dpar, masked ? c->rel_frac : -1.0,
                                                          c->acc + a.tail + 7, c->sssc_prec32,
                                                          fold_seq ? c->h_theta_dev : nullptr, c->acc + a.tail, c->err, fold_seq);
  HIP_TRY(hipGetLastError());
  return 0;
}

static int theta_update_bsc(evoamd_ctx *c, const MstepPlan &p, unsigned long long fold_seq) {
  const AccLayout a = acc_layout(c);
  const int H = c->H, D = c->D, learn = p.learn;
  int r = 0;
  if (learn & L_W) {
    if (!c->wq_copy_valid || p.force_pivot)
      HIP_TRY(hipMemcpyAsync(c->tmpA, c->acc + a.Wq, (size_t)H * H * sizeof(double), hipMemcpyDeviceToDevice, c->stream));
    c->wq_copy_valid = false;
    r = launch_inverse(c, c->tmpA, nullptr, H, p.force_pivot);
    if (r) return r;
    r = join_fork(c);
    if (r) return r;
    if (!launch_gemm_nn_raw(c, c->tmpA, H, c->acc + a.Wp, D, c->Wt, D, H, D, H, c->W, H))
      transpose_kernel<<<cdiv((i64)H * D, 256), 256, 0, c->stream>>>(c->Wt, H, D, c->W);
  }
  bsc_scalars_kernel<<<1, MS_T, 0, c->stream>>>(c->acc + a.pies, c->acc + a.sigma, H, D, c->acc + a.tail + 3, learn, c->dpar,
                                                c->mask_infr ? c->rel_frac : -1.0, fold_seq ? c->h_theta_dev : nullptr,
                                                c->acc + a.tail, c->err, fold_seq, c->bg_unit);
  HIP_TRY(hipGetLastError());
  return 0;
}

static int theta_update(evoamd_ctx *c, const MstepPlan &p, unsigned long long fold_seq) {
  c->gen++;
  SpanGuard g(c, KID_MSTEP);
  int r = c->model == EVOAMD_MODEL_SSSC ? theta_update_sssc(c, p, fold_seq) : theta_update_bsc(c, p, fold_seq);
  if (r) return r;
  c->B_valid = false;
  return 0;
}

static int compute_reconstruction(evoamd_ctx *c) {
  REQUIRE(!c->f32, "reconstruction is not available in the float32 mode");
  const size_t need = (size_t)c->N * c->D;
  if (need > c->yhat_n) {
    ALLOC(c->yhat, need);
    c->yhat_n = need;
  }
  const double *Wt = c->Wt;
  const double *E = c->Es;
  int lde = c->H;
  if (c->model == EVOAMD_MODEL_SSSC) {
    if (!c->tmpWt) ALLOC(c->tmpWt, (size_t)c->H * c->D);
    transpose_kernel<<<cdiv((i64)c->H * c->D, 256), 256, 0, c->stream>>>(c->W, c->D, c->H, c->tmpWt);
    Wt = c->tmpWt;
    E = c->Y + c->D + c->H;
    lde = c->ldY;
  }
  SpanGuard g(c, KID_GEMM);
  launch_gemm_nn_raw(c, E, lde, Wt, c->D, c->yhat, c->D, c->N, c->D, c->H);
  HIP_TRY(hipGetLastError());
  c->yhat_valid = true;
  return 0;
}

extern "C" int evoamd_reconstruct(evoamd_ctx *c, double *y_hat) {
  REQUIRE(c && c->configured && c->have_data && c->have_params && y_hat, "bad arguments");
  HIP_TRY(hipSetDevice(c->device));
  if (!c->yhat_valid) {
    REQUIRE(c->stats_rows_valid, "evoamd_reconstruct: call evoamd_stats first (and before setting new parameters)");
    int r = compute_reconstruction(c);
    if (r) return r;
  }
  HIP_TRY(hipMemcpyAsync(y_hat, c->yhat, (size_t)c->N * c->D * sizeof(double), hipMemcpyDeviceToHost, c->stream));
  HIP_TRY(hipStreamSynchronize(c->stream));
  return 0;
}

struct MailboxTicket {
  unsigned long long seq;
  hipStream_t stream;
};

static int mailbox_publish(evoamd_ctx *c, const MstepPlan &p, unsigned long long fold_seq, MailboxTicket &t) {
  t.stream = c->stream;
  if (p.publish == PUBLISH_FOLDED) {
    t.seq = fold_seq;
    return 0;
  }
  const AccLayout a = acc_layout(c);
  const size_t DH = (size_t)c->D * c->H, HH = (size_t)c->H * c->H, H = c->H;
  const bool sssc = c->model == EVOAMD_MODEL_SSSC;
  if (p.publish == PUBLISH_COPY_ENGINE) {
    double *dst = c->h_theta + MAILBOX_HDR;
    HIP_TRY(hipEventRecord(c->ev_theta, c->stream));
    HIP_TRY(hipStreamWaitEvent(c->stream_copy, c->ev_theta, 0));
    HIP_TRY(hipMemcpyAsync(dst, c->W, DH * sizeof(double), hipMemcpyDeviceToHost, c->stream_copy));
    if (sssc) {
      HIP_TRY(hipMemcpyAsync(dst + DH, c->Psi, HH * sizeof(double), hipMemcpyDeviceToHost, c->stream_copy));
      HIP_TRY(hipMemcpyAsync(dst + DH + HH, c->mus, H * sizeof(double), hipMemcpyDeviceToHost, c->stream_copy));
      HIP_TRY(hipMemcpyAsync(dst + DH + HH + H, c->pies, H * sizeof(double), hipMemcpyDeviceToHost, c->stream_copy));
    }
    HIP_TRY(hipEventRecord(c->ev_theta_done, c->stream_copy));
  }
  MailboxSegs segs = {};
  if (p.theta_in_mailbox) {
    segs.src[0] = c->W;
    segs.n[0] = (long long)DH;
    if (sssc) {
      segs.src[1] = c->Psi;
      segs.n[1] = (long long)HH;
      segs.src[2] = c->mus;
      segs.n[2] = (long long)H;
      segs.src[3] = c->pies;
      segs.n[3] = (long long)H;
    }
  }
  t.seq = ++c->mbox_seq;
  const long long total = MAILBOX_HDR + (p.theta_in_mailbox ? (long long)(DH + HH + 2 * H) : 0);
  const int grid = (int)std::min<long long>(64, cdiv(total, 256 * 8));
  if (p.publish == PUBLISH_SIDE) {
    HIP_TRY(hipEventRecord(c->ev_mbox, c->stream));
    HIP_TRY(hipStreamWaitEvent(c->stream_copy, c->ev_mbox, 0));
    t.stream = c->stream_copy;
  }
  mailbox_kernel<<<grid < 1 ? 1 : grid, 256, 0, t.stream>>>(c->h_theta_dev, c->acc + a.tail, c->err, segs, c->mbox_counter, t.seq);
  HIP_TRY(hipGetLastError());
  return 0;
}

static void prefetch_next_pass(evoamd_ctx *c) {
  if (!c->prefetch_lpj || c->mask_infr || c->last_estep_fused) return;
  c->prefetch_gen = ~0ull;
  const int rp = lpj_resident_launch(c, c->lpj_alt, batch_hints(c, 0, true));
  if (rp == 0) c->prefetch_gen = c->gen;
}

static int mailbox_poll(evoamd_ctx *c, const MstepPlan &p, const MailboxTicket &t) {
  volatile unsigned long long *flag = (volatile unsigned long long *)c->h_theta;
  const auto t0 = std::chrono::steady_clock::now();
  unsigned spins = 0;
  while (*flag != t.seq) {
    __builtin_ia32_pause();
    if ((++spins & 0xFFFu) == 0 &&
        std::chrono::duration<double>(std::chrono::steady_clock::now() - t0).count() > 0.02) {
      HIP_TRY(hipStreamSynchronize(t.stream));
      if (*flag != t.seq) return fail(EVOAMD_E_HIP, "mailbox kernel finished without publishing its sequence number");
    }
  }
  __atomic_thread_fence(__ATOMIC_ACQUIRE);
  if (p.publish == PUBLISH_COPY_ENGINE) HIP_TRY(hipEventSynchronize(c->ev_theta_done));
  return 0;
}

static int mailbox_errors(evoamd_ctx *c) {
  const int *e = (const int *)(c->h_theta + 1);
  if (e[0]) {
    HIP_TRY(hipMemsetAsync(c->err, 0, sizeof(int), c->stream));
    if (e[0] & 4) return fail(EVOAMD_E_INVALID, "internal: an ES3C overflow level was skipped although its list was not empty");
    if (e[0] & EVO_ERR_LIST_FULL) return fail(EVOAMD_E_INVALID, "internal: an ES3C overflow list was full, states were dropped");
    if (e[0] & EVO_ERR_BAD_ENTRY) return fail(EVOAMD_E_INVALID, "internal: an ES3C list entry or latent index read back from LDS was out of range");
    if (e[0] & 1) return fail(EVOAMD_E_KLIMIT, "ES3C: a state has more than %d active latents", SSSC_KCAP);
    return fail(EVOAMD_E_SINGULAR, "ES3C: exactly singular k x k system (the reference takes pinv here)");
  }
  return 0;
}

static CopySegs theta_segs(evoamd_ctx *c) {
  CopySegs s = {};
  s.ptr[0] = c->W;
  s.n[0] = (long long)c->D * c->H;
  if (c->model == EVOAMD_MODEL_SSSC) {
    s.ptr[1] = c->Psi;
    s.n[1] = (long long)c->H * c->H;
    s.ptr[2] = c->mus;
    s.n[2] = c->H;
    s.ptr[3] = c->pies;
    s.n[3] = c->H;
  }
  s.ptr[4] = c->dpar;
  s.n[4] = DP_COUNT;
  return s;
}

static int mstep_backup(evoamd_ctx *c, const MstepPlan &p) {
  if (p.backup == BACKUP_NONE) return 0;
  const CopySegs s = theta_segs(c);
  size_t n = 0;
  for (int k = 0; k < 5; k++) n += (size_t)s.n[k];
  if (n > c->theta_bak_n) {
    ALLOC(c->theta_bak, n);
    c->theta_bak_n = n;
  }
  if (p.backup == BACKUP_IN_UPDATE) return 0;
  theta_backup_kernel<<<(unsigned)std::min<size_t>(256, cdiv((i64)n, 256 * 8)), 256, 0, c->stream_copy>>>(c->theta_bak, s, 0);
  HIP_TRY(hipGetLastError());
  HIP_TRY(hipEventRecord(c->ev_bak, c->stream_copy));
  c->theta_bak_valid = true;
  return 0;
}

extern "C" int evoamd_restore_theta_backup(evoamd_ctx *c) {
  REQUIRE(c && c->configured, "configure first");
  REQUIRE(c->theta_bak && c->theta_bak_valid, "no parameter backup (evoamd_mstep_device keeps one when Theta stays on the device)");
  HIP_TRY(hipSetDevice(c->device));
  int r = join_fork(c);
  if (r) return r;
  HIP_TRY(hipStreamSynchronize(c->stream_copy));
  theta_backup_kernel<<<256, 256, 0, c->stream>>>(c->theta_bak, theta_segs(c), 1);
  HIP_TRY(hipGetLastError());
  HIP_TRY(hipStreamSynchronize(c->stream));
  c->gen++;
  c->h_theta_fresh = false;
  c->B_valid = false;
  c->have_params = true;
  c->prefetch_gen = ~0ull;
  return 0;
}

static int mstep_attempt(evoamd_ctx *c, const MstepPlan &p) {
  unsigned long long fold_seq = 0;
  int r;
  if (p.learn) {
    if (p.publish == PUBLISH_FOLDED) fold_seq = ++c->mbox_seq;
    r = theta_update(c, p, fold_seq);
    if (r) return r;
    if (p.backup == BACKUP_IN_UPDATE) c->theta_bak_valid = true;
    c->stats_rows_valid = false;
  }
  r = join_fork(c);
  if (r) return r;
  MailboxTicket t;
  r = mailbox_publish(c, p, fold_seq, t);
  if (r) return r;
  if (p.learn) {
    SpanGuard g(c, KID_MSTEP);
    r = derive_from_theta(c, true);
    if (r) return r;
  }
  prefetch_next_pass(c);
  return mailbox_poll(c, p, t);
}

static int mstep_deliver(evoamd_ctx *c, const MstepPlan &p, double *tail_out, double *dpar_out) {
  const double *h = c->h_theta + 8;
  memcpy(tail_out, h, 8 * sizeof(double));
  memcpy(dpar_out, h + 8, DP_COUNT * sizeof(double));
  memcpy(c->h_dpar, h + 8, DP_COUNT * sizeof(double));
  int r = mailbox_errors(c);
  if (r) return r;
  note_levels(c, c->h_dpar);
  c->h_theta_fresh = p.learn != 0 && !p.theta_home && c->h_dpar[DP_STATUS] == 0.0;
  if (c->h_dpar[DP_STATUS] == 0.0) return 0;
  dpar_out[DP_STATUS] = c->h_dpar[DP_STATUS];
  HIP_TRY(hipMemsetAsync(c->dpar + DP_STATUS, 0, sizeof(double), c->stream));
  c->prefetch_gen = ~0ull;
  c->have_params = false;
  HIP_TRY(hipMemsetAsync(c->flags, 0, (size_t)3 * c->N * sizeof(unsigned), c->stream));
  HIP_TRY(hipMemsetAsync(c->err, 0, 2 * sizeof(int), c->stream));
  return fail(EVOAMD_E_SINGULAR, "device Theta update: %s",
              c->h_dpar[DP_STATUS] == 1.0 ? "singular H x H system (the reference falls back to pinv / lstsq here)"
                                          : "non-finite sigma / pi");
}

extern "C" int evoamd_mstep_device(evoamd_ctx *c, int learn_mask, double *tail_out, double *dpar_out) {
  REQUIRE(tail_out && dpar_out, "NULL output");
  REQUIRE(!(c && c->mask_infr && c->rel_frac < 0.0), "incomplete data: evoamd_set_reliable_fraction first (bsc.py:113-118)");
  const MstepPlan p = mstep_plan(c, learn_mask, false);
  c->theta_bak_valid = false;
  int r = mstep_backup(c, p);
  if (r) return r;
  r = stats_compute(c, true);
  if (r) return r;
  c->h_theta_fresh = false;
  if (p.want_rec && !c->yhat_valid) {
    r = compute_reconstruction(c);
    if (r) return r;
  }
  if (p.backup == BACKUP_SIDE_KERNEL) HIP_TRY(hipStreamWaitEvent(c->stream, c->ev_bak, 0));
  r = mstep_attempt(c, p);
  if (r) return r;
  if (p.learn && c->h_theta[8 + 8 + DP_STATUS] == 3.0) {
    c->spd_fallbacks++;
    HIP_TRY(hipMemsetAsync(c->dpar + DP_STATUS, 0, sizeof(double), c->stream));
    HIP_TRY(hipMemcpyAsync(c->dpar + DP_LJC, c->dpar + DP_LJC_PREV, sizeof(double), hipMemcpyDeviceToDevice, c->stream));
    r = mstep_attempt(c, mstep_plan(c, learn_mask, true));
    if (r) return r;
  }
  return mstep_deliver(c, p, tail_out, dpar_out);
}

extern "C" int evoamd_gemm_tn(evoamd_ctx *c, const double *A, const double *B, double *C, int64_t K, int M, int Nc,
                              int sym_row0) {
  REQUIRE(c && A && B && C && K > 0 && M > 0 && Nc > 0, "bad arguments");
  REQUIRE(sym_row0 < 0 || (sym_row0 + Nc == M), "sym_row0: the symmetric block must be the last Nc rows of C");
  HIP_TRY(hipSetDevice(c->device));
  double *dA = nullptr, *dB = nullptr, *dC = nullptr;
  hipError_t e = hipMalloc((void **)&dA, (size_t)K * M * sizeof(double));
  if (e == hipSuccess) e = hipMalloc((void **)&dB, (size_t)K * Nc * sizeof(double));
  if (e == hipSuccess) e = hipMalloc((void **)&dC, (size_t)M * Nc * sizeof(double));
  int r = 0;
  if (e == hipSuccess) e = hipMemcpyAsync(dA, A, (size_t)K * M * sizeof(double), hipMemcpyHostToDevice, c->stream);
  if (e == hipSuccess) e = hipMemcpyAsync(dB, B, (size_t)K * Nc * sizeof(double), hipMemcpyHostToDevice, c->stream);
  GemmTnOpts o;
  o.sym_row0 = sym_row0;
  if (e == hipSuccess) r = launch_gemm_tn(c, dA, M, dB, Nc, dC, Nc, M, Nc, K, o);
  if (e == hipSuccess && !r) e = hipMemcpyAsync(C, dC, (size_t)M * Nc * sizeof(double), hipMemcpyDeviceToHost, c->stream);
  if (e == hipSuccess) e = hipStreamSynchronize(c->stream);
  (void)hipFree(dA);
  (void)hipFree(dB);
  (void)hipFree(dC);
  if (e != hipSuccess) return fail(EVOAMD_E_HIP, "evoamd_gemm_tn: %s", hipGetErrorString(e));
  return r;
}

extern "C" int evoamd_inverse(evoamd_ctx *c, double *A, double *B, int n, double *timing_ms) {
  REQUIRE(c && c->configured, "configure first");
  REQUIRE(A && n == c->H, "A must be H x H of the configured context");
  HIP_TRY(hipSetDevice(c->device));
  const size_t bytes = (size_t)n * n * sizeof(double);
  hipEvent_t e0, e1;
  HIP_TRY(hipEventCreate(&e0));
  HIP_TRY(hipEventCreate(&e1));
  double st = 0.0;
  int r = 0;
  for (int attempt = 0; attempt < 2; attempt++) {
    HIP_TRY(hipMemcpyAsync(c->tmpA, A, bytes, hipMemcpyHostToDevice, c->stream));
    if (B) HIP_TRY(hipMemcpyAsync(c->tmpB, B, bytes, hipMemcpyHostToDevice, c->stream));
    HIP_TRY(hipMemsetAsync(c->dpar + DP_STATUS, 0, sizeof(double), c->stream));
    HIP_TRY(hipEventRecord(e0, c->stream));
    r = launch_inverse(c, c->tmpA, B ? c->tmpB : nullptr, n, attempt == 1);
    HIP_TRY(hipEventRecord(e1, c->stream));
    if (r) break;
    HIP_TRY(hipMemcpyAsync(c->h_dpar + DP_COUNT, c->dpar + DP_STATUS, sizeof(double), hipMemcpyDeviceToHost, c->stream));
    HIP_TRY(hipMemsetAsync(c->dpar + DP_STATUS, 0, sizeof(double), c->stream));
    HIP_TRY(hipStreamSynchronize(c->stream));
    st = c->h_dpar[DP_COUNT];
    if (st != 3.0) break;
    c->spd_fallbacks++;
  }
  float ms = 0.f;
  if (!r) {
    HIP_TRY(hipEventElapsedTime(&ms, e0, e1));
    if (st == 0.0) {
      HIP_TRY(hipMemcpyAsync(A, c->tmpA, bytes, hipMemcpyDeviceToHost, c->stream));
      if (B) HIP_TRY(hipMemcpyAsync(B, c->tmpB, bytes, hipMemcpyDeviceToHost, c->stream));
      HIP_TRY(hipStreamSynchronize(c->stream));
    }
  }
  (void)hipEventDestroy(e0);
  (void)hipEventDestroy(e1);
  if (timing_ms) *timing_ms = ms;
  if (r) return r;
  if (st != 0.0) return fail(EVOAMD_E_SINGULAR, "evoamd_inverse: singular %d x %d system", n, n);
  return 0;
}

extern "C" int evoamd_get_params_bsc(evoamd_ctx *c, double *W, double *pi, double *sigma) {
  REQUIRE(c && c->configured && c->model == EVOAMD_MODEL_BSC && c->have_params, "no BSC parameters on the device");
  REQUIRE(W && pi && sigma, "NULL output");
  if (c->h_theta_fresh) {
    memcpy(W, c->h_theta + MAILBOX_HDR, (size_t)c->D * c->H * sizeof(double));
    *pi = c->h_dpar[DP_PI];
    *sigma = c->h_dpar[DP_SIGMA];
    return 0;
  }
  HIP_TRY(hipSetDevice(c->device));
  HIP_TRY(hipStreamSynchronize(c->stream));
  HIP_TRY(hipMemcpyAsync(c->h_par, c->W, (size_t)c->D * c->H * sizeof(double), hipMemcpyDeviceToHost, c->stream));
  HIP_TRY(hipMemcpyAsync(c->h_dpar, c->dpar, DP_COUNT * sizeof(double), hipMemcpyDeviceToHost, c->stream));
  HIP_TRY(hipStreamSynchronize(c->stream));
  memcpy(W, c->h_par, (size_t)c->D * c->H * sizeof(double));
  *pi = c->h_dpar[DP_PI];
  *sigma = c->h_dpar[DP_SIGMA];
  return 0;
}

extern "C" int evoamd_get_params_sssc(evoamd_ctx *c, double *W, double *pies, double *mus, double *Psi, double *sigma2) {
  REQUIRE(c && c->configured && c->model == EVOAMD_MODEL_SSSC && c->have_params, "no SSSC parameters on the device");
  REQUIRE(W && pies && mus && Psi && sigma2, "NULL output");
  if (c->h_theta_fresh) {
    const size_t DH = (size_t)c->D * c->H, HH = (size_t)c->H * c->H, H = c->H;
    const double *th = c->h_theta + MAILBOX_HDR;
    memcpy(W, th, DH * sizeof(double));
    memcpy(Psi, th + DH, HH * sizeof(double));
    memcpy(mus, th + DH + HH, H * sizeof(double));
    memcpy(pies, th + DH + HH + H, H * sizeof(double));
    *sigma2 = c->h_dpar[DP_SIGMA2];
    return 0;
  }
  HIP_TRY(hipSetDevice(c->device));
  HIP_TRY(hipStreamSynchronize(c->stream));
  const size_t DH = (size_t)c->D * c->H, HH = (size_t)c->H * c->H, H = c->H;
  double *hw = c->h_par, *hpsi = hw + DH, *hmu = hpsi + HH, *hpi = hmu + 2 * H;
  HIP_TRY(hipMemcpyAsync(hw, c->W, DH * sizeof(double), hipMemcpyDeviceToHost, c->stream));
  HIP_TRY(hipMemcpyAsync(hpsi, c->Psi, HH * sizeof(double), hipMemcpyDeviceToHost, c->stream));
  HIP_TRY(hipMemcpyAsync(hmu, c->mus, H * sizeof(double), hipMemcpyDeviceToHost, c->stream));
  HIP_TRY(hipMemcpyAsync(hpi, c->pies, H * sizeof(double), hipMemcpyDeviceToHost, c->stream));
  HIP_TRY(hipMemcpyAsync(c->h_dpar, c->dpar, DP_COUNT * sizeof(double), hipMemcpyDeviceToHost, c->stream));
  HIP_TRY(hipStreamSynchronize(c->stream));
  memcpy(W, hw, DH * sizeof(double));
  memcpy(Psi, hpsi, HH * sizeof(double));
  memcpy(mus, hmu, H * sizeof(double));
  memcpy(pies, hpi, H * sizeof(double));
  *sigma2 = c->h_dpar[DP_SIGMA2];
  return 0;
}

extern "C" int evoamd_free_energy(evoamd_ctx *c, const double *lpj, int64_t N, int C, double *Fs_out) {
  REQUIRE(c && lpj && Fs_out && N > 0 && C > 0, "bad arguments");
  HIP_TRY(hipSetDevice(c->device));
  double *d = nullptr;
  HIP_TRY(hipMalloc((void **)&d, ((size_t)N * C + 1) * sizeof(double)));
  hipError_t e = hipMemcpyAsync(d, lpj, (size_t)N * C * sizeof(double), hipMemcpyHostToDevice, c->stream);
  int r = 0;
  if (e != hipSuccess) r = fail(EVOAMD_E_HIP, "free_energy upload: %s", hipGetErrorString(e));
  if (!r) r = row_lse(c, d, N, C, nullptr, nullptr, d + (size_t)N * C);
  if (!r) {
    e = hipMemcpyAsync(Fs_out, d + (size_t)N * C, sizeof(double), hipMemcpyDeviceToHost, c->stream);
    if (e == hipSuccess) e = hipStreamSynchronize(c->stream);
    if (e != hipSuccess) r = fail(EVOAMD_E_HIP, "free_energy copy back: %s", hipGetErrorString(e));
  }
  (void)hipFree(d);
  return r;
}

static int ensure_patch_scratch(evoamd_ctx *c, size_t img_n, size_t y_n) {
  if (img_n > c->patch_img_n) {
    ALLOC(c->patch_img, img_n);
    c->patch_img_n = img_n;
  }
  if (y_n > c->patch_Y_n) {
    ALLOC(c->patch_Y, y_n);
    c->patch_Y_n = y_n;
  }
  return 0;
}

extern "C" int evoamd_patches_extract(evoamd_ctx *c, const double *img, int H, int W, int C, int ph, int pw, int shift,
// ... 441 lines not shown
```

evo_amd/csrc/gemm_f64.hpp:

```cpp
#pragma once
#include "common.hpp"

typedef double v4f64 __attribute__((ext_vector_type(4)));

#define GEMM_BM 64
#define GEMM_BN 64
#define GEMM_BK 16
#define GEMM_LDS 80

template <bool VEC>
__global__ __launch_bounds__(256, 3) void gemm_tn_f64(const double *__restrict__ A, int lda,
                                                   const double *__restrict__ B, int ldb,
                                                   double *__restrict__ C, int ldc, int M, int Nc,
                                                   i64 K, i64 k_per_split, int gx, int gy, int split, int sym_row0) {
  __shared__ double As[2][GEMM_BK][GEMM_LDS];
  __shared__ double Bs[2][GEMM_BK][GEMM_LDS];
  const int tiles = gx * gy;
  const int xcd = blockIdx.x & 7, jj = blockIdx.x >> 3;
  const int zc = split ? xcd + 8 * (jj / tiles) : 0;
  const int tile = split ? jj % tiles : (int)blockIdx.x;
  const int m0 = (tile / gx) * GEMM_BM, n0 = (tile % gx) * GEMM_BN;
  if (sym_row0 >= 0 && m0 >= sym_row0 && m0 - sym_row0 > n0) return;
  const i64 kbeg = (i64)zc * k_per_split;
  const i64 kend = (kbeg + k_per_split < K) ? kbeg + k_per_split : K;
// ... 215 lines not shown
    const int kl = kk * 4 + (lane >> 4);
#pragma unroll
    for (int i = 0; i < 4; i++) a[i] = As[buf][kl][wm * 64 + i * 16 + (lane & 15)];
#pragma unroll
    for (int j = 0; j < 4; j++) b[j] = Bs[buf][kl][wn * 64 + j * 16 + (lane & 15)];
  };
  auto compute = [&](int buf) {
    T a[2][4], b[2][4];
    frags(buf, 0, a[0], b[0]);
#pragma unroll
    for (int kk = 0; kk < GEMM_BK / 4; kk++) {
      if (kk + 1 < GEMM_BK / 4) frags(buf, kk + 1, a[(kk + 1) & 1], b[(kk + 1) & 1]);
#pragma unroll
      for (int i = 0; i < 4; i++)
#pragma unroll
        for (int j = 0; j < 4; j++) acc[i][j] = MM::mma(a[kk & 1][i], b[kk & 1][j], acc[i][j]);
    }
  };
  i64 nslab = (kend > kbeg) ? (kend - kbeg + GEMM_BK - 1) / GEMM_BK : 0;
  nslab = (nslab + 1) & ~(i64)1;
  if (nslab > 0) {
    fetch(ra, rb, kbeg);
    stash(ra, rb, 0, kbeg);
    fetch(ra, rb, kbeg + GEMM_BK);
  }
  __syncthreads();
  i64 s0 = 0;
  if (m0 + GEMM_T <= M && n0 + GEMM_T <= Nc) {
    constexpr int RPP = 256 / PPR;
    const int pr = t / PPR, pc = (t % PPR) * EPP;
    const T *pa = A + (kbeg + 2 * GEMM_BK + pr) * (i64)lda + m0 + pc;
    const T *pb = B + (kbeg + 2 * GEMM_BK + pr) * (i64)ldb + n0 + pc;
    const i64 stepA = (i64)RPP * lda, stepB = (i64)RPP * ldb, slabA = (i64)GEMM_BK * lda, slabB = (i64)GEMM_BK * ldb;
    for (; kbeg + (s0 + 4) * GEMM_BK <= kend; s0 += 2) {
#pragma unroll
      for (int j = 0; j < 2; j++) {
        compute(j);
#pragma unroll
        for (int i = 0; i < NP; i++) {
          *(piece_t *)&As[j ^ 1][pr + RPP * i][pc] = ra[i];
          *(piece_t *)&Bs[j ^ 1][pr + RPP * i][pc] = rb[i];
        }
#pragma unroll
        for (int i = 0; i < NP; i++) {
          ra[i] = *(const piece_t *)(pa + i * stepA);
          rb[i] = *(const piece_t *)(pb + i * stepB);
        }
        pa += slabA;
        pb += slabB;
        __syncthreads();
      }
    }
    if (s0 + 2 == nslab && kbeg + nslab * GEMM_BK == kend) {
      compute(0);
#pragma unroll
      for (int i = 0; i < NP; i++) {
        *(piece_t *)&As[1][pr + RPP * i][pc] = ra[i];
        *(piece_t *)&Bs[1][pr + RPP * i][pc] = rb[i];
      }
      __syncthreads();
      compute(1);
      s0 = nslab;
    }
  }
  for (; s0 < nslab; s0 += 2) {
#pragma unroll
    for (int j = 0; j < 2; j++) {
      const i64 sl = s0 + j;
      compute(j);
      stash(ra, rb, j ^ 1, kbeg + (sl + 1) * GEMM_BK);
      fetch(ra, rb, kbeg + (sl + 2) * GEMM_BK);
      __syncthreads();
    }
  }
#pragma unroll
  for (int i = 0; i < 4; i++)
#pragma unroll
    for (int j = 0; j < 4; j++)
#pragma unroll
      for (int r = 0; r < 4; r++) {
        const int row = m0 + wm * 64 + i * 16 + MM::row(lane, r);
        const int col = n0 + wn * 64 + j * 16 + (lane & 15);
        if (slab) {
          slab[(row - m0) * GEMM_T + (col - n0)] = (TO)acc[i][j][r];
        } else if (row < M && col < Nc) {
          if (atomic)
            unsafeAtomicAdd((double *)&C[(i64)row * ldc + col], (double)acc[i][j][r]);
          else
            C[(i64)row * ldc + col] = (TO)acc[i][j][r];
        }
      }
}

__global__ __launch_bounds__(256) __attribute__((amdgpu_waves_per_eu(2, 2))) void gemm_tn128_f64(const double *__restrict__ A, int lda,
                                                      const double *__restrict__ B, int ldb,
                                                      double *__restrict__ C, int ldc, int M, int Nc, i64 K,
                                                      i64 k_per_split, int gx, int gy, int split, int sym_row0) {
  extern __shared__ double lds128[];
  double(*As)[GEMM_BK][GEMM_LDS2] = (double(*)[GEMM_BK][GEMM_LDS2])lds128;
  double(*Bs)[GEMM_BK][GEMM_LDS2] = (double(*)[GEMM_BK][GEMM_LDS2])(lds128 + 2 * GEMM_BK * GEMM_LDS2);
  const int tiles = gx * gy;
  const int xcd = blockIdx.x & 7, jj = blockIdx.x >> 3;
  const int zc = split ? xcd + 8 * (jj / tiles) : 0;
  const int tile = split ? jj % tiles : (int)blockIdx.x;
  const int m0 = (tile / gx) * GEMM_T, n0 = (tile % gx) * GEMM_T;
  if (sym_row0 >= 0 && m0 >= sym_row0 && m0 - sym_row0 > n0) return;
  const i64 kbeg = (i64)zc * k_per_split;
  const i64 kend = (kbeg + k_per_split < K) ? kbeg + k_per_split : K;
  gemm_tn128_segment(A, lda, B, ldb, C, ldc, M, Nc, m0, n0, kbeg, kend, split != 0, As, Bs);
}

__global__ __launch_bounds__(256) __attribute__((amdgpu_waves_per_eu(2, 2))) void gemm_tn128_sk_f64(
    const double *__restrict__ A, int lda, const double *__restrict__ B, int ldb, double *__restrict__ C, int ldc, int M,
    int Nc, i64 K, i64 Kx, int gx, int gy, int sym_row0, int n_real, double *__restrict__ ws, int segmax) {
  extern __shared__ double lds128[];
  double(*As)[GEMM_BK][GEMM_LDS2] = (double(*)[GEMM_BK][GEMM_LDS2])lds128;
  double(*Bs)[GEMM_BK][GEMM_LDS2] = (double(*)[GEMM_BK][GEMM_LDS2])(lds128 + 2 * GEMM_BK * GEMM_LDS2);
  const int xcd = blockIdx.x & 7, w = blockIdx.x >> 3, wpx = gridDim.x >> 3;
  const i64 kx0 = (i64)xcd * Kx;
  const i64 kx1 = (kx0 + Kx < K) ? kx0 + Kx : K;
  if (kx1 <= kx0) return;
  const i64 slabs = (kx1 - kx0 + GEMM_BK - 1) / GEMM_BK;
  const i64 U = (i64)n_real * slabs;
  i64 u = U * w / wpx;
  const i64 u1 = U * (w + 1) / wpx;
  int seg = 0;
  while (u < u1) {
    const int rt = (int)(u / slabs);
    const i64 sb = u - (i64)rt * slabs;
    i64 se = sb + (u1 - u);
    if (se > slabs) se = slabs;
    int tile = 0, seen = -1;
    for (int tt = 0; tt < gx * gy; tt++) {
      const int tm = (tt / gx) * GEMM_T, tn = (tt % gx) * GEMM_T;
      if (sym_row0 >= 0 && tm >= sym_row0 && tm - sym_row0 > tn) continue;
      if (++seen == rt) {
        tile = tt;
        break;
      }
    }
    const int m0 = (tile / gx) * GEMM_T, n0 = (tile % gx) * GEMM_T;
    const i64 kbeg = kx0 + sb * GEMM_BK;
    i64 kend = kx0 + se * GEMM_BK;
    if (kend > kx1) kend = kx1;
    double *slab = (ws && seg < segmax) ? ws + ((size_t)blockIdx.x * segmax + seg) * (GEMM_T * GEMM_T) : nullptr;
    gemm_tn128_segment(A, lda, B, ldb, C, ldc, M, Nc, m0, n0, kbeg, kend, true, As, Bs, slab);
    u += se - sb;
    seg++;
  }
}

__global__ __launch_bounds__(256) void gemm_sk_reduce_kernel(const double *__restrict__ ws, int segmax,
                                                             double *__restrict__ C, int ldc, int M, int Nc, i64 K, i64 Kx,
                                                             int gx, int gy, int sym_row0, int n_real, int wpx) {
  constexpr int MAXW = 72;
  __shared__ int slab_of[8][MAXW];
  __shared__ int slab_n[8];
  __shared__ int tile_sh;
  const int rt = blockIdx.x;
  const int e = blockIdx.y * 256 + threadIdx.x;
  if (threadIdx.x < 8) {
    const int xcd = threadIdx.x;
    int q = 0;
    const i64 kx0 = (i64)xcd * Kx;
    const i64 kx1 = (kx0 + Kx < K) ? kx0 + Kx : K;
    if (kx1 > kx0) {
      const i64 slabs = (kx1 - kx0 + GEMM_BK - 1) / GEMM_BK;
      const i64 U = (i64)n_real * slabs;
      const i64 a = (i64)rt * slabs, b = a + slabs;
      i64 w = a * wpx / U;
      while (w > 0 && U * w / wpx > a) w--;
      while (w < wpx && U * (w + 1) / wpx <= a) w++;
      for (; w < wpx && q < MAXW; w++) {
        const i64 u0 = U * w / wpx, u1 = U * (w + 1) / wpx;
        if (u0 >= b) break;
        if (u1 <= u0) continue;
        const int seg = rt - (int)(u0 / slabs);
        if (seg < segmax) slab_of[xcd][q++] = (int)((xcd + 8 * w) * segmax + seg);
      }
    }
    slab_n[xcd] = q;
  } else if (threadIdx.x == 64) {
    int tile = 0, seen = -1;
    for (int tt = 0; tt < gx * gy; tt++) {
      const int tm = (tt / gx) * GEMM_T, tn = (tt % gx) * GEMM_T;
      if (sym_row0 >= 0 && tm >= sym_row0 && tm - sym_row0 > tn) continue;
      if (++seen == rt) {
        tile = tt;
        break;
      }
    }
    tile_sh = tile;
  }
  __syncthreads();
  const int tile = tile_sh;
  const int row = (tile / gx) * GEMM_T + e / GEMM_T, col = (tile % gx) * GEMM_T + e % GEMM_T;
  double sum = 0.0;
  for (int xcd = 0; xcd < 8; xcd++)
    for (int q = 0; q < slab_n[xcd]; q++) sum += ws[(size_t)slab_of[xcd][q] * (GEMM_T * GEMM_T) + e];
  if (row < M && col < Nc) C[(i64)row * ldc + col] += sum;
}

template <typename T>
__global__ __launch_bounds__(256) __attribute__((amdgpu_waves_per_eu(2, 2))) void gemm_tn128_gk(
    const T *__restrict__ A, int lda, const T *__restrict__ B, int ldb, double *__restrict__ C, int ldc, int M, int Nc,
    i64 K, i64 Kc, int gx, int gy, int sym_row0, int n_real, int J, double *__restrict__ ws) {
  extern __shared__ double lds128[];
  T(*As)[GEMM_BK][GEMM_LDS2] = (T(*)[GEMM_BK][GEMM_LDS2])lds128;
  T(*Bs)[GEMM_BK][GEMM_LDS2] = (T(*)[GEMM_BK][GEMM_LDS2])((T *)lds128 + 2 * GEMM_BK * GEMM_LDS2);
  const int xcd = blockIdx.x & 7, l = blockIdx.x >> 3, wpx = gridDim.x >> 3;
  const int g = xcd * wpx + l;
  if (g >= n_real * J) return;
  const int j = g / n_real, rt = g - j * n_real;
  int tile = 0, seen = -1;
  for (int tt = 0; tt < gx * gy; tt++) {
    const int tm = (tt / gx) * GEMM_T, tn = (tt % gx) * GEMM_T;
    if (sym_row0 >= 0 && tm >= sym_row0 && tm - sym_row0 > tn) continue;
    if (++seen == rt) {
      tile = tt;
      break;
    }
  }
  const int m0 = (tile / gx) * GEMM_T, n0 = (tile % gx) * GEMM_T;
  const i64 kbeg = (i64)j * Kc;
  const i64 kend = (kbeg + Kc < K) ? kbeg + Kc : K;
  gemm_tn128_segment<T, double>(A, lda, B, ldb, C, ldc, M, Nc, m0, n0, kbeg, kend, true, As, Bs,
                                ws + (size_t)g * (GEMM_T * GEMM_T));
}

__global__ __launch_bounds__(256) void gemm_gk_reduce_kernel(const double *__restrict__ ws, double *__restrict__ C, int ldc,
                                                             int M, int Nc, int gx, int gy, int sym_row0, int n_real, int J) {
  __shared__ int tile_sh;
  const int rt = blockIdx.x;
  const int e = blockIdx.y * 256 + threadIdx.x;
  if (threadIdx.x == 0) {
    int tile = 0, seen = -1;
    for (int tt = 0; tt < gx * gy; tt++) {
      const int tm = (tt / gx) * GEMM_T, tn = (tt % gx) * GEMM_T;
      if (sym_row0 >= 0 && tm >= sym_row0 && tm - sym_row0 > tn) continue;
      if (++seen == rt) {
        tile = tt;
        break;
      }
    }
    tile_sh = tile;
  }
  __syncthreads();
  const int tile = tile_sh;
  const int row = (tile / gx) * GEMM_T + e / GEMM_T, col = (tile % gx) * GEMM_T + e % GEMM_T;
  double sum = 0.0;
  for (int j = 0; j < J; j++) sum += ws[((size_t)j * n_real + rt) * (GEMM_T * GEMM_T) + e];
  if (row < M && col < Nc) C[(i64)row * ldc + col] += sum;
}

__global__ __launch_bounds__(256) __attribute__((amdgpu_waves_per_eu(2, 2))) void gemm_tn128_rows_f64(
    const double *__restrict__ A, int lda, const double *__restrict__ B, int ldb, double *__restrict__ C, int ldc, int M,
    int Nc, i64 K, int gx, int gy) {
  extern __shared__ double lds128[];
  double(*As)[GEMM_BK][GEMM_LDS2] = (double(*)[GEMM_BK][GEMM_LDS2])lds128;
  double(*Bs)[GEMM_BK][GEMM_LDS2] = (double(*)[GEMM_BK][GEMM_LDS2])(lds128 + 2 * GEMM_BK * GEMM_LDS2);
  const int xcd = blockIdx.x & 7, j = blockIdx.x >> 3;
  const int ty = xcd + 8 * (j / gx), tx = j % gx;
  if (ty >= gy) return;
  gemm_tn128_segment(A, lda, B, ldb, C, ldc, M, Nc, ty * GEMM_T, tx * GEMM_T, 0, K, false, As, Bs);
}

__global__ __launch_bounds__(256) __attribute__((amdgpu_waves_per_eu(2, 2))) void gemm_tn128_sk_f32(
    const float *__restrict__ A, int lda, const float *__restrict__ B, int ldb, double *__restrict__ C, int ldc, int M,
    int Nc, i64 K, i64 Kx, int gx, int gy, int n_real, double *__restrict__ ws, int segmax) {
  extern __shared__ double lds128[];
  float(*As)[GEMM_BK][GEMM_LDS2] = (float(*)[GEMM_BK][GEMM_LDS2])lds128;
  float(*Bs)[GEMM_BK][GEMM_LDS2] = (float(*)[GEMM_BK][GEMM_LDS2])((float *)lds128 + 2 * GEMM_BK * GEMM_LDS2);
  const int xcd = blockIdx.x & 7, w = blockIdx.x >> 3, wpx = gridDim.x >> 3;
  const i64 kx0 = (i64)xcd * Kx;
  const i64 kx1 = (kx0 + Kx < K) ? kx0 + Kx : K;
  if (kx1 <= kx0) return;
  const i64 slabs = (kx1 - kx0 + GEMM_BK - 1) / GEMM_BK;
  const i64 U = (i64)n_real * slabs;
  i64 u = U * w / wpx;
  const i64 u1 = U * (w + 1) / wpx;
  int seg = 0;
  while (u < u1) {
    const int tile = (int)(u / slabs);
    const i64 sb = u - (i64)tile * slabs;
    i64 se = sb + (u1 - u);
    if (se > slabs) se = slabs;
    const int m0 = (tile / gx) * GEMM_T, n0 = (tile % gx) * GEMM_T;
    const i64 kbeg = kx0 + sb * GEMM_BK;
    i64 kend = kx0 + se * GEMM_BK;
    if (kend > kx1) kend = kx1;
    double *slab = (ws && seg < segmax) ? ws + ((size_t)blockIdx.x * segmax + seg) * (GEMM_T * GEMM_T) : nullptr;
    gemm_tn128_segment<float, double>(A, lda, B, ldb, C, ldc, M, Nc, m0, n0, kbeg, kend, true, As, Bs, slab);
    u += se - sb;
    seg++;
  }
}

__global__ __launch_bounds__(256) __attribute__((amdgpu_waves_per_eu(2, 2))) void gemm_tn128_store_f32(
    const float *__restrict__ A, int lda, const float *__restrict__ B, int ldb, float *__restrict__ C, int ldc, int M,
    int Nc, i64 K, int gx) {
  extern __shared__ double lds128[];
  float(*As)[GEMM_BK][GEMM_LDS2] = (float(*)[GEMM_BK][GEMM_LDS2])lds128;
  float(*Bs)[GEMM_BK][GEMM_LDS2] = (float(*)[GEMM_BK][GEMM_LDS2])((float *)lds128 + 2 * GEMM_BK * GEMM_LDS2);
  const int tile = blockIdx.x;
  const int m0 = (tile / gx) * GEMM_T, n0 = (tile % gx) * GEMM_T;
  gemm_tn128_segment<float, float>(A, lda, B, ldb, C, ldc, M, Nc, m0, n0, 0, K, false, As, Bs);
}

template <bool VEC>
__global__ __launch_bounds__(256, 4) void gemm_nn_f64(const double *__restrict__ A, int lda,
                                                   const double *__restrict__ B, int ldb,
                                                   double *__restrict__ C, int ldc, i64 M, int Nc,
                                                   int K, int gx, int gy, int rows_per_xcd) {
  __shared__ double As[2][GEMM_BK][GEMM_LDS];
  __shared__ double Bs[2][GEMM_BK][GEMM_LDS];
  const int xcd = blockIdx.x & 7, jj = blockIdx.x >> 3;
  const i64 ry = (i64)xcd * rows_per_xcd + jj / gx;
  if (jj / gx >= rows_per_xcd || ry >= gy) return;
  const i64 m0 = ry * GEMM_BM;
  const int n0 = (jj % gx) * GEMM_BN;
  const int t = threadIdx.x, lane = t & 63, wave = t >> 6;
  const int wm = wave >> 1, wn = wave & 1;
  v4f64 acc[2][2];
#pragma unroll
  for (int i = 0; i < 2; i++)
#pragma unroll
    for (int j = 0; j < 2; j++) acc[i][j] = (v4f64){0.0, 0.0, 0.0, 0.0};
  const int am = t >> 2, ak = (t & 3) * 4;
  const int br = t >> 4, bc = (t & 15) * 4;
  double ra[2][4], rb[2][4];
  auto fetch = [&](double(&qa)[4], double(&qb)[4], int k0) {
    const i64 m = m0 + am;
    if (VEC) {
#pragma unroll
      for (int i = 0; i < 2; i++) {
        const int k = k0 + ak + 2 * i;
        const i64 mc = m < M ? m : M - 1;
        const double2 va = *(const double2 *)(A + mc * lda + (k < K ? k : K - 2));
        qa[2 * i] = va.x;
        qa[2 * i + 1] = va.y;
        const int p = t + 256 * i, kb = k0 + (p >> 5), cc = (p & 31) * 2, nb = n0 + cc;
        const double2 vb = *(const double2 *)(B + (i64)(kb < K ? kb : K - 1) * ldb + (nb < Nc ? nb : Nc - 2));
        qb[2 * i] = vb.x;
        qb[2 * i + 1] = vb.y;
      }
    } else {
      const int kb = k0 + br;
#pragma unroll
      for (int q = 0; q < 4; q++) {
        const int k = k0 + ak + q, n = n0 + bc + q;
        qa[q] = (m < M && k < K) ? A[m * lda + k] : 0.0;
        qb[q] = (kb < K && n < Nc) ? B[(i64)kb * ldb + n] : 0.0;
      }
    }
  };
  auto stash = [&](const double(&qa)[4], const double(&qb)[4], int buf, int k0) {
    if (VEC) {
      const bool min = m0 + am < M;
#pragma unroll
      for (int q = 0; q < 4; q++) As[buf][ak + q][am] = (min && k0 + ak + (q & ~1) < K) ? qa[q] : 0.0;
#pragma unroll
      for (int i = 0; i < 2; i++) {
        const int p = t + 256 * i, r = p >> 5, cc = (p & 31) * 2;
        const bool inb = k0 + r < K && n0 + cc < Nc;
        *(double2 *)&Bs[buf][r][cc] = inb ? make_double2(qb[2 * i], qb[2 * i + 1]) : make_double2(0.0, 0.0);
      }
    } else {
#pragma unroll
      for (int q = 0; q < 4; q++) As[buf][ak + q][am] = qa[q];
#pragma unroll
      for (int q = 0; q < 4; q++) Bs[buf][br][bc + q] = qb[q];
    }
  };
  auto compute = [&](int buf) {
#pragma unroll
    for (int kk = 0; kk < GEMM_BK / 4; kk++) {
      const int kl = kk * 4 + (lane >> 4);
      double a[2], b[2];
#pragma unroll
      for (int i = 0; i < 2; i++) a[i] = As[buf][kl][wm * 32 + i * 16 + (lane & 15)];
#pragma unroll
      for (int j = 0; j < 2; j++) b[j] = Bs[buf][kl][wn * 32 + j * 16 + (lane & 15)];
#pragma unroll
      for (int i = 0; i < 2; i++)
#pragma unroll
        for (int j = 0; j < 2; j++)
// ... 237 lines not shown
```

Baseline: 5.083 billion state evals/s.

## Run M-step tail and Gram derivation on side stream beside B; split deferred GEMM reduce

Adds a DerivePlan that, for large SSSC problems, moves the post-W M-step tail (psi finish, Gram GEMM, trace, sigma, mailbox, tables) onto the secondary stream so it runs concurrently with launch_B on the main stream, joined by an event. It also defers the stream-K/grouped-K reduce of the sufficient-statistics GEMM: only the tiles feeding the W' rows are reduced before the W update, and the remaining tiles are reduced on the side stream. The reduce kernels gain a tile offset to allow partial launches. The cost is added cross-stream event bookkeeping and risk of ordering bugs around pending reduces.

```diff
diff --git a/evo_amd/csrc/evo_amd.hip b/evo_amd/csrc/evo_amd.hip
--- a/evo_amd/csrc/evo_amd.hip
+++ b/evo_amd/csrc/evo_amd.hip
@@ -152,6 +152,17 @@
   bool ar_gemm_pending = false;
   int overlap_gemm = 1;
   int early_fork = -1;
+  int tail_beside_b = -1;
+  hipEvent_t ev_w = nullptr, ev_tail = nullptr;
+  struct PendingReduce {
+    bool active = false;
+    bool grouped = false;
+    const double *ws = nullptr;
+    double *C = nullptr;
+    int ldc = 0, M = 0, Nc = 0, gx = 0, gy = 0, sym_row0 = -1, n_real = 0, J = 0, segmax = 0, wpx = 0, T = 0;
+    i64 K = 0, Kx = 0;
+    bool mirror = false;
+  } pend;
   int bg_unit = 0;
   int fold_clear = 1;
   bool acc_clean = false, clist_clean = false;
@@ -448,6 +459,8 @@
   HIP_TRY(hipEventCreateWithFlags(&c->ev_theta, hipEventDisableTiming));
   HIP_TRY(hipEventCreateWithFlags(&c->ev_theta_done, hipEventDisableTiming));
   HIP_TRY(hipEventCreateWithFlags(&c->ev_mbox, hipEventDisableTiming));
+  HIP_TRY(hipEventCreateWithFlags(&c->ev_w, hipEventDisableTiming));
+  HIP_TRY(hipEventCreateWithFlags(&c->ev_tail, hipEventDisableTiming));
   HIP_TRY(hipEventCreateWithFlags(&c->ev_bak, hipEventDisableTiming));
   for (int i = 0; i < 16; i++) HIP_TRY(hipEventCreateWithFlags(&c->ev_chunk[i], hipEventDisableTiming));
 
@@ -533,6 +546,8 @@
   if (c->ev_theta) (void)hipEventDestroy(c->ev_theta);
   if (c->ev_theta_done) (void)hipEventDestroy(c->ev_theta_done);
   if (c->ev_mbox) (void)hipEventDestroy(c->ev_mbox);
+  if (c->ev_w) (void)hipEventDestroy(c->ev_w);
+  if (c->ev_tail) (void)hipEventDestroy(c->ev_tail);
   if (c->ev_bak) (void)hipEventDestroy(c->ev_bak);
   if (c->ev_fork) (void)hipEventDestroy(c->ev_fork);
   if (c->ev_join) (void)hipEventDestroy(c->ev_join);
@@ -669,6 +684,11 @@
     c->early_fork = value;
     return 0;
   }
+  if (strcmp(name, "tail_beside_b") == 0) {
+    if (value < -1 || value > 1) return fail(EVOAMD_E_INVALID, "tail_beside_b: -1 (automatic), 0 (serial order) or 1");
+    c->tail_beside_b = value;
+    return 0;
+  }
   if (strcmp(name, "merge_small_levels") == 0) {
     c->merge_small = value != 0;
     return 0;
@@ -723,7 +743,7 @@
   return fail(EVOAMD_E_INVALID, "unknown option '%s'", name);
 }
 
-static int join_fork(evoamd_ctx *c);
+static int join_fork(evoamd_ctx *c, bool keep_reduce = false);
 
 extern "C" int evoamd_synchronize(evoamd_ctx *c) {
   REQUIRE(c, "ctx is NULL");
@@ -1341,6 +1361,7 @@
   hipStream_t stream = nullptr;
   int spare = 0;
   double *diag = nullptr;
+  bool defer_reduce = false;
 };
 
 static bool gram_is_small(int M, i64 K) { return M <= 512 && K <= 4096; }
@@ -1360,6 +1381,23 @@
     c->gemm_ws_n = need;
   }
   return c->gemm_ws;
+}
+
+static int reduce_tiles(const evoamd_ctx::PendingReduce &pr, int first, int last, hipStream_t stream) {
+  if (last > first) {
+    const dim3 grid((unsigned)(last - first), GEMM_T * GEMM_T / 256);
+    if (pr.grouped)
+      gemm_gk_reduce_kernel<<<grid, 256, 0, stream>>>(pr.ws, pr.C, pr.ldc, pr.M, pr.Nc, pr.gx, pr.gy, pr.sym_row0, pr.n_real,
+                                                      pr.J, first);
+    else
+      gemm_sk_reduce_kernel<<<grid, 256, 0, stream>>>(pr.ws, pr.segmax, pr.C, pr.ldc, pr.M, pr.Nc, pr.K, pr.Kx, pr.gx, pr.gy,
+                                                      pr.sym_row0, pr.n_real, pr.wpx, first);
+  }
+  if (pr.mirror && last == pr.n_real)
+    mirror_lower_kernel<<<cdiv((i64)pr.Nc * pr.Nc, 256), 256, 0, stream>>>(pr.C + (size_t)pr.sym_row0 * pr.ldc, pr.Nc, pr.ldc,
+                                                                         pr.T);
+  HIP_TRY(hipGetLastError());
+  return 0;
 }
 
 static int launch_gemm_tn(evoamd_ctx *c, const double *A, int lda, const double *B, int ldb, double *C, int ldc,
@@ -1427,6 +1465,7 @@
     }
     const i64 Kx = ((cdiv(K, 8) + GEMM_BK - 1) / GEMM_BK) * GEMM_BK;
     const unsigned wpx = (unsigned)std::max(1, 2 * c->n_cu / 8 - o.spare);
+    evoamd_ctx::PendingReduce pr;
     int segmax = 0;
     double *ws = c->gemm_ws_opt ? streamk_workspace(c, wpx, real, &segmax) : nullptr;
     const i64 J = (i64)8 * wpx / real;
@@ -1434,14 +1473,26 @@
       const i64 Kc = ((cdiv(K, J) + 2 * GEMM_BK - 1) / (2 * GEMM_BK)) * (2 * GEMM_BK);
       gemm_tn128_gk<double><<<8 * wpx, 256, GEMM128_LDS_BYTES, stream>>>(A, lda, B, ldb, C, ldc, M, Nc, K, Kc, gx, gy,
                                                                             sym_row0, (int)real, (int)J, ws);
-      gemm_gk_reduce_kernel<<<dim3((unsigned)real, GEMM_T * GEMM_T / 256), 256, 0, stream>>>(ws, C, ldc, M, Nc, gx, gy,
-                                                                                               sym_row0, (int)real, (int)J);
+      pr.grouped = true;
+      pr.J = (int)J;
     } else {
     gemm_tn128_sk_f64<<<8 * wpx, 256, GEMM128_LDS_BYTES, stream>>>(A, lda, B, ldb, C, ldc, M, Nc, K, Kx, gx, gy, sym_row0,
                                                                        (int)real, ws, segmax);
-    if (ws)
-      gemm_sk_reduce_kernel<<<dim3((unsigned)real, GEMM_T * GEMM_T / 256), 256, 0, stream>>>(
-          ws, segmax, C, ldc, M, Nc, K, Kx, gx, gy, sym_row0, (int)real, (int)wpx);
+    }
+    if (ws) {
+      pr.active = true;
+      pr.ws = ws;
+      pr.C = C;
+      pr.ldc = ldc, pr.M = M, pr.Nc = Nc, pr.gx = gx, pr.gy = gy, pr.sym_row0 = sym_row0, pr.n_real = (int)real;
+      pr.segmax = segmax, pr.wpx = (int)wpx, pr.T = T, pr.K = K, pr.Kx = Kx;
+      if (o.defer_reduce) {
+        pr.mirror = sym_row0 >= 0 && mirror;
+        HIP_TRY(hipGetLastError());
+        c->pend = pr;
+        return 0;
+      }
+      int rr = reduce_tiles(pr, 0, pr.n_real, stream);
+      if (rr) return rr;
     }
   } else if (big)
     gemm_tn128_f64<<<grid, 256, GEMM128_LDS_BYTES, stream>>>(A, lda, B, ldb, C, ldc, M, Nc, K, kps, gx, gy, split, sym_row0);
@@ -1476,13 +1527,36 @@
   return 0;
 }
 
-static int derive_from_theta(evoamd_ctx *c, bool updated) {
+struct DerivePlan {
+  bool tail_beside_b = false;
+  bool split_reduce = false;
+};
+
+static bool tail_beside_b_pays(const evoamd_ctx *c);
+static double contraction_flops(const evoamd_ctx *c);
+static double theta_chain_us(const evoamd_ctx *c);
+
+static DerivePlan derive_plan(const evoamd_ctx *c, int learn, bool copy_engine) {
+  DerivePlan d;
+  if (!learn || !c->have_data || copy_engine || !c->stream2 || c->tail_beside_b == 0) return d;
+  if (c->model == EVOAMD_MODEL_BSC && c->bsc_direct) return d;
+  if (c->timing && (c->timing_mask & ((1u << KID_MSTEP) | (1u << KID_GEMM) | (1u << KID_MISC)))) return d;
+  if (c->tail_beside_b < 0 && !tail_beside_b_pays(c)) return d;
+  d.tail_beside_b = true;
+  d.split_reduce = c->model == EVOAMD_MODEL_SSSC && !c->comm && !c->mask_infr && !c->sssc_prec32 &&
+                   contraction_flops(c) / 65e6 >= 2.0 * theta_chain_us(c);
+  return d;
+}
+
+static int derive_from_theta(evoamd_ctx *c, bool updated, const DerivePlan &dp = DerivePlan()) {
   const int H = c->H, D = c->D;
   int r = 0;
   c->B_valid = false;
   if (c->model == EVOAMD_MODEL_BSC && c->bsc_direct) return 0;
+  const hipStream_t side = dp.tail_beside_b ? c->stream2 : c->stream;
   GemmTnOpts gram;
   gram.deterministic = true;
+  gram.stream = side;
   if (c->model == EVOAMD_MODEL_SSSC) {
     if (!updated) {
       r = launch_gemm_tn(c, c->W, H, c->W, H, c->G, H, H, H, D, gram);
@@ -1491,9 +1565,9 @@
     }
     if (c->mask_infr) {
       if (!c->Wt) ALLOC(c->Wt, (size_t)H * D);
-      transpose_kernel<<<cdiv((i64)H * D, 256), 256, 0, c->stream>>>(c->W, D, H, c->Wt);
+      transpose_kernel<<<cdiv((i64)H * D, 256), 256, 0, side>>>(c->W, D, H, c->Wt);
     }
-    sssc_tables_kernel<<<cdiv((i64)H * H, 256), 256, 0, c->stream>>>(c->G, c->Psi, c->mus, c->pilbar_v, c->dpar, H, c->D1,
+    sssc_tables_kernel<<<cdiv((i64)H * H, 256), 256, 0, side>>>(c->G, c->Psi, c->mus, c->pilbar_v, c->dpar, H, c->D1,
                                                                      c->PT, c->GP, c->DG, c->sing_gen, ++c->theta_gen);
     DBG_SYNC(c, "derive_from_theta: tables");
   } else {
@@ -1501,15 +1575,16 @@
     if (diag_rides) gram.diag = c->diag;
     r = launch_gemm_tn(c, c->W, H, c->W, H, c->G, H, H, H, D, gram);
     if (r) return r;
-    if (!diag_rides) extract_diag_kernel<<<cdiv(H, 256), 256, 0, c->stream>>>(c->G, H, c->diag);
+    if (!diag_rides) extract_diag_kernel<<<cdiv(H, 256), 256, 0, side>>>(c->G, H, c->diag);
   }
   HIP_TRY(hipGetLastError());
+  if (dp.tail_beside_b) HIP_TRY(hipEventRecord(c->ev_tail, c->stream2));
   if (c->have_data) {
     r = launch_B(c);
-    if (r) return r;
-    c->B_valid = true;
-  }
-  return 0;
+    if (!r) c->B_valid = true;
+  }
+  if (dp.tail_beside_b) HIP_TRY(hipStreamWaitEvent(c->stream, c->ev_tail, 0));
+  return r;
 }
 
 extern "C" int evoamd_set_params_bsc(evoamd_ctx *c, const double *W, double pi, double sigma, double *ljc) {
@@ -1619,13 +1694,13 @@
       gemm_tn128_gk<float><<<8 * wpx, 256, GEMM128_LDS_BYTES, stream>>>(A, lda, B, ldb, C, ldc, M, Nc, K, Kc, gx, gy, -1,
                                                                            (int)real, (int)J, ws);
       gemm_gk_reduce_kernel<<<dim3((unsigned)real, GEMM_T * GEMM_T / 256), 256, 0, stream>>>(ws, C, ldc, M, Nc, gx, gy, -1,
-                                                                                               (int)real, (int)J);
+                                                                                               (int)real, (int)J, 0);
     } else {
       gemm_tn128_sk_f32<<<8 * wpx, 256, GEMM128_LDS_BYTES, stream>>>(A, lda, B, ldb, C, ldc, M, Nc, K, Kx, gx, gy, gx * gy,
                                                                          ws, segmax);
       if (ws)
         gemm_sk_reduce_kernel<<<dim3((unsigned)(gx * gy), GEMM_T * GEMM_T / 256), 256, 0, stream>>>(
-            ws, segmax, C, ldc, M, Nc, K, Kx, gx, gy, -1, gx * gy, (int)wpx);
+            ws, segmax, C, ldc, M, Nc, K, Kx, gx, gy, -1, gx * gy, (int)wpx, 0);
     }
   } else {
     gemm_tn_naive_f32<<<cdiv((i64)M * Nc, 256), 256, 0, stream>>>(A, lda, B, ldb, C, ldc, M, Nc, K);
@@ -2742,10 +2817,15 @@
 
 static int compute_reconstruction(evoamd_ctx *c);
 
-static int join_fork(evoamd_ctx *c) {
+static int join_fork(evoamd_ctx *c, bool keep_reduce) {
   if (c->gemm_forked) {
     HIP_TRY(hipStreamWaitEvent(c->stream, c->ev_join, 0));
     c->gemm_forked = false;
+  }
+  if (c->pend.active && !keep_reduce) {
+    c->pend.active = false;
+    int r = reduce_tiles(c->pend, 0, c->pend.n_real, c->stream);
+    if (r) return r;
   }
   if (c->ar_gemm_pending) {
     c->ar_gemm_pending = false;
@@ -2778,6 +2858,15 @@
 
 static double contraction_flops(const evoamd_ctx *c) {
   return c->model == EVOAMD_MODEL_SSSC ? 2.0 * (double)c->N * (c->D + 2.0 * c->H) * c->H : 2.0 * (double)c->N * c->D * c->H;
+}
+
+static double theta_chain_us(const evoamd_ctx *c) {
+  return c->H >= 256 ? 15.0 * cdiv(c->H, 32) : 8.5 * cdiv(c->H, 16);
+}
+
+static bool tail_beside_b_pays(const evoamd_ctx *c) {
+  if (c->comm || c->model != EVOAMD_MODEL_SSSC) return false;
+  return 2.0 * (double)c->N * c->H * c->D >= 2e10;
 }
 
 struct StatsPlan {
@@ -2800,6 +2889,7 @@
   int waves;
   bool census;
   bool bsc_wave;
+  bool defer_reduce;
 };
 
 struct StatsBlock {
@@ -2865,7 +2955,7 @@
   return 0;
 }
 
-static int stats_plan(evoamd_ctx *c, bool fork_gemm, StatsPlan &p) {
+static int stats_plan(evoamd_ctx *c, bool fork_gemm, bool defer_reduce, StatsPlan &p) {
   p = StatsPlan{};
   p.a = acc_layout(c);
   p.N = c->N;
@@ -2909,12 +2999,13 @@
   p.nchunks = nchunks = (int)cdiv(p.N, p.rows_per_chunk);
   p.second_stream = p.fork_gemm || nchunks > 1;
   {
-    const double chain_us = c->H >= 256 ? 15.0 * cdiv(c->H, 32) : 8.5 * cdiv(c->H, 16);
+    const double chain_us = theta_chain_us(c);
     p.gemm_spare = !(p.fork_gemm && nchunks == 1) ? 0 : ((gemm_flops / 65e6 >= 3.0 * chain_us && c->H <= 512) ? 4 : 8);
   }
   const int SRb = (int)cdiv(c->S, 64);
   p.bsc_wave = c->model == EVOAMD_MODEL_BSC && c->bsc_wave_opt && dig_for(c, c->states) &&
                (SRb == 1 || SRb == 2 || SRb == 4 || SRb == 3) && nchunks == 1 && (size_t)5 * p.H * sizeof(double) <= 150 * 1024;
+  p.defer_reduce = defer_reduce && c->model == EVOAMD_MODEL_SSSC && !p.masked && nchunks == 1 && !c->comm;
   return 0;
 }
 
@@ -3283,6 +3374,7 @@
   if (c->model == EVOAMD_MODEL_BSC)
     return launch_gemm_tn(c, c->Es + (size_t)n0 * H, H, Ywp + (size_t)n0 * ldwp, ldwp, c->acc + a.Wp, D, H, D, nc, o);
   o.sym_row0 = ((D + H) % GEMM_BM) == 0 ? D + H : -1;
+  o.defer_reduce = p.defer_reduce;
   return launch_gemm_tn(c, c->Y + (size_t)n0 * c->ldY, c->ldY, ep.Ez + (size_t)n0 * c->ldY, c->ldY, c->acc + a.sWp, H,
                         D + 2 * H, H, nc, o);
 }
@@ -3368,12 +3460,13 @@
   return zero_lists(c);
 }
 
-static int stats_compute(evoamd_ctx *c, bool fork_gemm = false) {
+static int stats_compute(evoamd_ctx *c, bool fork_gemm = false, bool defer_reduce = false) {
   REQUIRE(c && c->configured && c->have_data && c->have_params, "configure, upload_data and set_params first");
   REQUIRE_KN(c);
   StatsPlan p;
-  int r = stats_plan(c, fork_gemm, p);
-  if (r) return r;
+  int r = stats_plan(c, fork_gemm, defer_reduce, p);
+  if (r) return r;
+  c->pend.active = false;
   r = join_fork(c);
   if (r) return r;
   HIP_TRY(hipSetDevice(c->device));
@@ -3608,7 +3701,7 @@
   return p;
 }
 
-static int theta_update_sssc(evoamd_ctx *c, const MstepPlan &p, unsigned long long fold_seq) {
+static int theta_update_sssc(evoamd_ctx *c, const MstepPlan &p, const DerivePlan &dp, unsigned long long fold_seq) {
   const AccLayout a = acc_layout(c);
   const int H = c->H, D = c->D, learn = p.learn;
   const i64 HH = (i64)H * H;
@@ -3628,31 +3721,49 @@
   else if (learn & L_PSI)
     r = launch_inverse(c, c->tmpB, nullptr, H, p.force_pivot);
   if (r) return r;
-  r = join_fork(c);
-  if (r) return r;
+  r = join_fork(c, dp.split_reduce);
+  if (r) return r;
+  const bool split = dp.split_reduce && c->pend.active;
+  const int wp_tiles = split ? (int)std::min<i64>(c->pend.n_real, cdiv(D, c->pend.T) * c->pend.gx) : 0;
+  c->pend.active = false;
+  if (split && (learn & L_W)) {
+    r = reduce_tiles(c->pend, 0, wp_tiles, c->stream);
+    if (r) return r;
+  }
   if (c->sssc_prec32) round_f32_kernel<<<cdiv(a.y2 - a.s_sz, 256), 256, 0, c->stream>>>(c->acc + a.s_sz, a.y2 - a.s_sz);
   if (learn & L_W)
     launch_gemm_nn_raw(c, c->acc + a.sWp, H, c->tmpA, H, c->W, H, D, H, H);
+  hipStream_t side = c->stream;
+  if (dp.tail_beside_b) {
+    side = c->stream2;
+    HIP_TRY(hipEventRecord(c->ev_w, c->stream));
+    HIP_TRY(hipStreamWaitEvent(side, c->ev_w, 0));
+  }
+  if (split) {
+    r = reduce_tiles(c->pend, (learn & L_W) ? wp_tiles : 0, c->pend.n_real, side);
+    if (r) return r;
+  }
   const bool masked = c->mask_infr != nullptr;
   const bool psi_with_trace = (learn & L_PSI) && (learn & L_SIGMA2) && !masked;
   if ((learn & L_PSI) && !psi_with_trace)
-    sssc_psi_finish_kernel<<<cdiv(HH, 256), 256, 0, c->stream>>>(c->tmpC, c->tmpB, c->acc + a.s_sz, c->mus, H, c->Psi);
+    sssc_psi_finish_kernel<<<cdiv(HH, 256), 256, 0, side>>>(c->tmpC, c->tmpB, c->acc + a.s_sz, c->mus, H, c->Psi);
   else if (!(learn & L_PSI))
-    psi_floor_kernel<<<cdiv(H, 256), 256, 0, c->stream>>>(c->Psi, H);
+    psi_floor_kernel<<<cdiv(H, 256), 256, 0, side>>>(c->Psi, H);
   HIP_TRY(hipGetLastError());
   GemmTnOpts gram;
   gram.deterministic = true;
+  gram.stream = side;
   r = launch_gemm_tn(c, c->W, H, c->W, H, c->G, H, H, H, D, gram);
   if (r) return r;
   const int n_part = (int)std::min<i64>(1024, cdiv(HH, 1024));
   r = ensure_colpart(c, (size_t)n_part);
   if (r) return r;
   if (psi_with_trace)
-    sssc_trace_partial_kernel<<<n_part, 256, 0, c->stream>>>(c->acc + a.sz_sz, c->G, H, cdiv(HH, n_part), c->colpart, c->tmpC,
-                                                             c->tmpB, c->acc + a.s_sz, c->mus, c->Psi);
+    sssc_trace_partial_kernel<<<n_part, 256, 0, side>>>(c->acc + a.sz_sz, c->G, H, cdiv(HH, n_part), c->colpart, c->tmpC,
+                                                        c->tmpB, c->acc + a.s_sz, c->mus, c->Psi);
   else if ((learn & L_SIGMA2) && !masked)
-    sssc_trace_partial_kernel<<<n_part, 256, 0, c->stream>>>(c->acc + a.sz_sz, c->G, H, cdiv(HH, n_part), c->colpart);
-  sssc_sigma_precompute_kernel<<<1, MS_T, 0, c->stream>>>(c->acc + a.y2, D, c->colpart, masked ? 0 : n_part, H, Nptr, learn,
+    sssc_trace_partial_kernel<<<n_part, 256, 0, side>>>(c->acc + a.sz_sz, c->G, H, cdiv(HH, n_part), c->colpart);
+  sssc_sigma_precompute_kernel<<<1, MS_T, 0, side>>>(c->acc + a.y2, D, c->colpart, masked ? 0 : n_part, H, Nptr, learn,
                                                           c->pies, c->pilbar_v, c->dpar, masked ? c->rel_frac : -1.0,
                                                           c->acc + a.tail + 7, c->sssc_prec32,
                                                           fold_seq ? c->h_theta_dev : nullptr, c->acc + a.tail, c->err, fold_seq);
@@ -3660,7 +3771,7 @@
   return 0;
 }
 
-static int theta_update_bsc(evoamd_ctx *c, const MstepPlan &p, unsigned long long fold_seq) {
+static int theta_update_bsc(evoamd_ctx *c, const MstepPlan &p, const DerivePlan &dp, unsigned long long fold_seq) {
   const AccLayout a = acc_layout(c);
   const int H = c->H, D = c->D, learn = p.learn;
   int r = 0;
@@ -3675,17 +3786,25 @@
     if (!launch_gemm_nn_raw(c, c->tmpA, H, c->acc + a.Wp, D, c->Wt, D, H, D, H, c->W, H))
       transpose_kernel<<<cdiv((i64)H * D, 256), 256, 0, c->stream>>>(c->Wt, H, D, c->W);
   }
-  bsc_scalars_kernel<<<1, MS_T, 0, c->stream>>>(c->acc + a.pies, c->acc + a.sigma, H, D, c->acc + a.tail + 3, learn, c->dpar,
+  hipStream_t side = c->stream;
+  if (dp.tail_beside_b) {
+    r = join_fork(c);
+    if (r) return r;
+    side = c->stream2;
+    HIP_TRY(hipEventRecord(c->ev_w, c->stream));
+    HIP_TRY(hipStreamWaitEvent(side, c->ev_w, 0));
+  }
+  bsc_scalars_kernel<<<1, MS_T, 0, side>>>(c->acc + a.pies, c->acc + a.sigma, H, D, c->acc + a.tail + 3, learn, c->dpar,
                                                 c->mask_infr ? c->rel_frac : -1.0, fold_seq ? c->h_theta_dev : nullptr,
                                                 c->acc + a.tail, c->err, fold_seq, c->bg_unit);
   HIP_TRY(hipGetLastError());
   return 0;
 }
 
-static int theta_update(evoamd_ctx *c, const MstepPlan &p, unsigned long long fold_seq) {
+static int theta_update(evoamd_ctx *c, const MstepPlan &p, const DerivePlan &dp, unsigned long long fold_seq) {
   c->gen++;
   SpanGuard g(c, KID_MSTEP);
-  int r = c->model == EVOAMD_MODEL_SSSC ? theta_update_sssc(c, p, fold_seq) : theta_update_bsc(c, p, fold_seq);
+  int r = c->model == EVOAMD_MODEL_SSSC ? theta_update_sssc(c, p, dp, fold_seq) : theta_update_bsc(c, p, dp, fold_seq);
   if (r) return r;
   c->B_valid = false;
   return 0;
@@ -3733,10 +3852,12 @@
   hipStream_t stream;
 };
 
-static int mailbox_publish(evoamd_ctx *c, const MstepPlan &p, unsigned long long fold_seq, MailboxTicket &t) {
+static int mailbox_publish(evoamd_ctx *c, const MstepPlan &p, const DerivePlan &dp, unsigned long long fold_seq,
+                           MailboxTicket &t) {
   t.stream = c->stream;
   if (p.publish == PUBLISH_FOLDED) {
     t.seq = fold_seq;
+    if (dp.tail_beside_b) t.stream = c->stream2;
     return 0;
   }
   const AccLayout a = acc_layout(c);
@@ -3770,7 +3891,9 @@
   t.seq = ++c->mbox_seq;
   const long long total = MAILBOX_HDR + (p.theta_in_mailbox ? (long long)(DH + HH + 2 * H) : 0);
   const int grid = (int)std::min<long long>(64, cdiv(total, 256 * 8));
-  if (p.publish == PUBLISH_SIDE) {
+  if (dp.tail_beside_b) {
+    t.stream = c->stream2;
+  } else if (p.publish == PUBLISH_SIDE) {
     HIP_TRY(hipEventRecord(c->ev_mbox, c->stream));
     HIP_TRY(hipStreamWaitEvent(c->stream_copy, c->ev_mbox, 0));
     t.stream = c->stream_copy;
@@ -3869,12 +3992,12 @@
   return 0;
 }
 
-static int mstep_attempt(evoamd_ctx *c, const MstepPlan &p) {
+static int mstep_attempt(evoamd_ctx *c, const MstepPlan &p, const DerivePlan &dp) {
   unsigned long long fold_seq = 0;
   int r;
   if (p.learn) {
     if (p.publish == PUBLISH_FOLDED) fold_seq = ++c->mbox_seq;
-    r = theta_update(c, p, fold_seq);
+    r = theta_update(c, p, dp, fold_seq);
     if (r) return r;
     if (p.backup == BACKUP_IN_UPDATE) c->theta_bak_valid = true;
     c->stats_rows_valid = false;
@@ -3882,11 +4005,11 @@
   r = join_fork(c);
   if (r) return r;
   MailboxTicket t;
-  r = mailbox_publish(c, p, fold_seq, t);
+  r = mailbox_publish(c, p, dp, fold_seq, t);
   if (r) return r;
   if (p.learn) {
     SpanGuard g(c, KID_MSTEP);
-    r = derive_from_theta(c, true);
+    r = derive_from_theta(c, true, dp);
     if (r) return r;
   }
   prefetch_next_pass(c);
@@ -3918,10 +4041,11 @@
   REQUIRE(tail_out && dpar_out, "NULL output");
   REQUIRE(!(c && c->mask_infr && c->rel_frac < 0.0), "incomplete data: evoamd_set_reliable_fraction first (bsc.py:113-118)");
   const MstepPlan p = mstep_plan(c, learn_mask, false);
+  const DerivePlan dp = derive_plan(c, p.learn, p.publish == PUBLISH_COPY_ENGINE);
   c->theta_bak_valid = false;
   int r = mstep_backup(c, p);
   if (r) return r;
-  r = stats_compute(c, true);
+  r = stats_compute(c, true, dp.split_reduce);
   if (r) return r;
   c->h_theta_fresh = false;
   if (p.want_rec && !c->yhat_valid) {
@@ -3929,13 +4053,13 @@
     if (r) return r;
   }
   if (p.backup == BACKUP_SIDE_KERNEL) HIP_TRY(hipStreamWaitEvent(c->stream, c->ev_bak, 0));
-  r = mstep_attempt(c, p);
+  r = mstep_attempt(c, p, dp);
   if (r) return r;
   if (p.learn && c->h_theta[8 + 8 + DP_STATUS] == 3.0) {
     c->spd_fallbacks++;
     HIP_TRY(hipMemsetAsync(c->dpar + DP_STATUS, 0, sizeof(double), c->stream));
     HIP_TRY(hipMemcpyAsync(c->dpar + DP_LJC, c->dpar + DP_LJC_PREV, sizeof(double), hipMemcpyDeviceToDevice, c->stream));
-    r = mstep_attempt(c, mstep_plan(c, learn_mask, true));
+    r = mstep_attempt(c, mstep_plan(c, learn_mask, true), dp);
     if (r) return r;
   }
   return mstep_deliver(c, p, tail_out, dpar_out);
diff --git a/evo_amd/csrc/gemm_f64.hpp b/evo_amd/csrc/gemm_f64.hpp
--- a/evo_amd/csrc/gemm_f64.hpp
+++ b/evo_amd/csrc/gemm_f64.hpp
@@ -391,12 +391,13 @@
 
 __global__ __launch_bounds__(256) void gemm_sk_reduce_kernel(const double *__restrict__ ws, int segmax,
                                                              double *__restrict__ C, int ldc, int M, int Nc, i64 K, i64 Kx,
-                                                             int gx, int gy, int sym_row0, int n_real, int wpx) {
+                                                             int gx, int gy, int sym_row0, int n_real, int wpx,
+                                                             int rt0) {
   constexpr int MAXW = 72;
   __shared__ int slab_of[8][MAXW];
   __shared__ int slab_n[8];
   __shared__ int tile_sh;
-  const int rt = blockIdx.x;
+  const int rt = rt0 + blockIdx.x;
   const int e = blockIdx.y * 256 + threadIdx.x;
   if (threadIdx.x < 8) {
     const int xcd = threadIdx.x;
@@ -468,9 +469,10 @@
 }
 
 __global__ __launch_bounds__(256) void gemm_gk_reduce_kernel(const double *__restrict__ ws, double *__restrict__ C, int ldc,
-                                                             int M, int Nc, int gx, int gy, int sym_row0, int n_real, int J) {
+                                                             int M, int Nc, int gx, int gy, int sym_row0, int n_real, int J,
+                                                             int rt0) {
   __shared__ int tile_sh;
-  const int rt = blockIdx.x;
+  const int rt = rt0 + blockIdx.x;
   const int e = blockIdx.y * 256 + threadIdx.x;
   if (threadIdx.x == 0) {
     int tile = 0, seen = -1;
```

Result: no change. 5.121 billion state evals/s (median of 6 runs) (+0.8%).
